# lyndonchan/wsss-analysis

Hardware: AMD Instinct MI355X
Metric: images/sec CAM+CRF pseudo-labels, VOC2012 321x321 (higher is better)
Workload: dtype f16x3; 1 GPU; resnet50 CAM + dense-CRF (M=21, 10 mean-field iters), 321x321, batch 32 images (=64 samples) per GPU, image-sharded; batch_images=32, num_classes=20, parallelism=image-sharded x1, no collective, steps_per_rank=245

## Files before the change

### include/wsscam.h

```cpp
#ifndef WSSCAM_H
#define WSSCAM_H

#include <stddef.h>
#include <stdint.h>

#ifdef __cplusplus
extern "C" {
#endif

#define WSC_VERSION 100

typedef enum wsc_status {
    WSC_OK = 0,
    WSC_ERR_INVALID = -1,
    WSC_ERR_NO_DEVICE = -2,
    WSC_ERR_HIP = -3,
    WSC_ERR_MISSING_KEY = -4,
    WSC_ERR_SHAPE = -5,
    WSC_ERR_NOMEM = -6,
    WSC_ERR_KEY_RANGE = -7,
    WSC_ERR_CAPACITY = -8,
    WSC_ERR_RANGE = -9
} wsc_status;

typedef enum wsc_arch {
    WSC_ARCH_RESNET50_CAM = 0,
    WSC_ARCH_VGG16_CAM = 1,
    WSC_ARCH_M7_CAM = 2,
    WSC_ARCH_RESNET50_IRN = 3,
    WSC_ARCH_VGG16_IRN = 4,
    WSC_ARCH_M7_IRN = 5
} wsc_arch;

typedef enum wsc_precision {
    WSC_PREC_BF16 = 0,
    WSC_PREC_BF16X3 = 1,
    WSC_PREC_F16 = 2,
    WSC_PREC_F16X3 = 3
} wsc_precision;

typedef struct wsc_ctx wsc_ctx;
typedef struct wsc_net wsc_net;
typedef enum {
    WSC_OPT_CRF_GAUSS_ON_CHIP = 0,
    WSC_OPT_CRF_FUSED_BLUR = 1,
    WSC_OPT_CRF_BLUR_ON_CHIP = 2,
    WSC_OPT_CRF_RANK_BALLOT = 3,
    WSC_OPT_CRF_EMBED_FULL = 4,
    WSC_OPT_RW_TILED = 5,
    WSC_OPT_STEM_POOL_FUSED = 6,
    WSC_OPT_CONV_WINDOW = 7,
    WSC_OPT_CAM_HEAD_STREAM = 8,
    WSC_OPT_CRF_MSG_IN_UPDATE = 9,
    WSC_OPT_COUNT = 10
} wsc_option;

typedef struct wsc_crf wsc_crf;
typedef struct wsc_crf_v wsc_crf_v;

typedef struct wsc_tensor_desc {
    const char *name;
    const float *data;
    int32_t ndim;
    int64_t shape[4];
} wsc_tensor_desc;


int wsc_version(void);
const char *wsc_last_error(void);

int wsc_ctx_create(int device, void *stream, wsc_ctx **out);
void wsc_ctx_destroy(wsc_ctx *ctx);
int wsc_ctx_set_option(wsc_ctx *ctx, int option, int value);
int wsc_sync(wsc_ctx *ctx);
int wsc_ctx_range_status(wsc_ctx *ctx, int *flag_out, int clear);
int wsc_ctx_wait(wsc_ctx *ctx, wsc_ctx *other);
int wsc_ctx_mark(wsc_ctx *ctx, int slot);
int wsc_ctx_wait_mark(wsc_ctx *ctx, int slot);
int wsc_ctx_wait_for_mark(wsc_ctx *ctx, wsc_ctx *other, int slot);
int wsc_device_info(wsc_ctx *ctx, char *arch_name, size_t arch_name_len, int *num_cus);

int wsc_malloc(wsc_ctx *ctx, size_t bytes, void **dptr_out);
int wsc_free(wsc_ctx *ctx, void *dptr);
int wsc_memcpy_h2d(wsc_ctx *ctx, void *dst_dev, const void *src_host, size_t bytes);
int wsc_memcpy_d2h(wsc_ctx *ctx, void *dst_host, const void *src_dev, size_t bytes);
int wsc_memset(wsc_ctx *ctx, void *dst_dev, int value, size_t bytes);
int wsc_host_alloc(wsc_ctx *ctx, size_t bytes, void **host_out);
int wsc_host_free(wsc_ctx *ctx, void *host);
int wsc_host_write_segments(const char *path, int n, const void *const *ptrs, const size_t *sizes);
int wsc_memcpy_h2d_async(wsc_ctx *ctx, void *dst_dev, const void *src_pinned_host, size_t bytes);
int wsc_memcpy_d2h_async(wsc_ctx *ctx, void *dst_pinned_host, const void *src_dev, size_t bytes);

int wsc_timer_begin(wsc_ctx *ctx);
int wsc_timer_end(wsc_ctx *ctx, float *ms_out);

int wsc_profile_begin(wsc_ctx *ctx);
int wsc_profile_end(wsc_ctx *ctx, int max_classes, int32_t *calls_out, float *total_ms_out, double *work_out,
                    int *n_classes_out);
const char *wsc_profile_class_name(int cls);


int wsc_net_create(wsc_ctx *ctx, int arch, const wsc_tensor_desc *weights, int n_weights,
                   int num_classes, int precision, wsc_net **out);
void wsc_net_destroy(wsc_net *net);
int wsc_net_cam_size(const wsc_net *net, int S, int *h_out);
int wsc_net_feat_channels(const wsc_net *net, int *f_out);

int wsc_net_forward_cam(wsc_ctx *ctx, const wsc_net *net, const float *x_dev, int B, int S,
                        float *cam_dev, float *score_dev);
int wsc_net_cam_size_hw(const wsc_net *net, int H, int W, int *h_out, int *w_out);
int wsc_net_forward_cam_hw(wsc_ctx *ctx, const wsc_net *net, const float *x_dev, int B, int H, int W, float *cam_dev,
                           float *score_dev);

int wsc_net_forward_features(wsc_ctx *ctx, const wsc_net *net, const float *x_dev ,
                             int N, int S, float *feat_dev);

int wsc_net_forward_edge(wsc_ctx *ctx, const wsc_net *net, const float *x_dev, int B, int S, int feat_h, int feat_w,
                         float *edge_dev, float *dp_dev);

int wsc_rw_propagate(wsc_ctx *ctx, const float *x_dev, const float *edge_dev, int K, int h, int w,
                     const int32_t *dirs_host, const int32_t *path_start_host, const int32_t *path_yx_host, int D,
                     float beta, int n_steps, float *rw_dev);
int wsc_rw_propagate_batch(wsc_ctx *ctx, int n_img, const int32_t *K_host, const int32_t *h_host,
                           const int32_t *w_host, const float *x_dev, const float *edge_dev,
                           const int32_t *dirs_host, const int32_t *path_start_host, const int32_t *path_yx_host,
                           int D, float beta, int n_steps, float *rw_dev);

int wsc_net_forward_gradcam(wsc_ctx *ctx, const wsc_net *net, const float *x_dev, int N, int S, int relu,
                            float *cams_dev, float *score_dev);

#define WSC_CONV_GENERIC 0x100
int wsc_conv2d_nchw(wsc_ctx *ctx, const float *x_dev, int N, int Cin, int H, int W, const float *w_host,
                    int Cout, int kh, int kw, int stride, int pad, const float *scale_host,
                    const float *shift_host, const float *residual_dev, int relu, int precision,
                    float *y_dev);


int wsc_cam_postprocess(wsc_ctx *ctx, const float *cam_dev, int B, int C, int h, int w,
                        const int32_t *size_hw_host , const int32_t *keys_host,
                        const int32_t *key_off_host , const int64_t *strided_off_host ,
                        const int64_t *highres_off_host , float *strided_dev, float *highres_dev);

int wsc_cam_eval_confusion(wsc_ctx *ctx, const float *highres_dev, int B, const int32_t *size_hw_host,
                           const int32_t *keys_host, const int32_t *key_off_host,
                           const int64_t *highres_off_host, float bg_thres, const uint8_t *gt_dev, int n_class,
                           int ignore_label, uint8_t *pred_dev, int64_t *confusion_dev);

int wsc_unary_from_maps(wsc_ctx *ctx, const float *maps_dev, int B, int C, int N, float bg_value,
                        float *unary_dev);

int wsc_cam_eval_confusion_nn(wsc_ctx *ctx, const float *maps_dev, int B, const int32_t *src_hw_host ,
                              const int32_t *out_hw_host , const int32_t *keys_host, const int32_t *key_off_host ,
                              const int64_t *maps_off_host , const uint8_t *gt_dev, int n_class, int ignore_label,
                              uint8_t *pred_dev, int64_t *confusion_dev);

int wsc_label_confusion_nn(wsc_ctx *ctx, const int32_t *labels_dev, int B, const int32_t *src_hw_host ,
                           const int32_t *out_hw_host , const int64_t *labels_off_host , const uint8_t *gt_dev,
                           int n_class, int ignore_label, uint8_t *pred_dev, int64_t *confusion_dev);

int wsc_sem_seg_finish(wsc_ctx *ctx, const float *rw_dev, int B, const int64_t *rw_off_host , const int32_t *khw_host ,
                       const int32_t *up_hw_host , const int32_t *out_hw_host , const int32_t *keys_host,
                       const int32_t *key_off_host , int has_bg, float bg_thres, uint8_t *label_dev);

int wsc_cam_unary(wsc_ctx *ctx, const float *cam_dev, int B, int C, int h, int w, int H0, int W0, float bg_value,
                  float *unary_dev);
int wsc_cam_unary_pm(wsc_ctx *ctx, const float *cam_dev, int B, int C, int h, int w, int H0, int W0, float bg_value,
                     float *unary_pm_dev);

int wsc_cam_sum_scales(wsc_ctx *ctx, const float *cam_dev, int n_images, int n_scales, long long map_elems, float *out_dev);

int wsc_msf_input_u8(wsc_ctx *ctx, const uint8_t *images_dev, int B, const int32_t *size_hw_host,
                     const int64_t *offset_host, int S, const float *mean3_host, const float *std3_host,
                     int pre_div255, int pair, float *x_dev);

int wsc_resize_u8(wsc_ctx *ctx, const uint8_t *images_dev, int B, const int32_t *size_hw_host, const int64_t *offset_host,
                  int OH, int OW, uint8_t *out_dev);

int wsc_bilinear_resize(wsc_ctx *ctx, const float *src_dev, int C, int h, int w, float *dst_dev, int H,
                        int W);


int wsc_label_unary_from_cam(wsc_ctx *ctx, const float *highres_dev, int B, int K, int N, float thres, float gt_prob,
                             float *unary_dev, int32_t *labels_dev);
int wsc_ir_label_combine(wsc_ctx *ctx, const int32_t *fg_pred_dev, const int32_t *bg_pred_dev, const int32_t *keys_host,
                         int B, int M, int N, uint8_t *conf_dev);


int wsc_hsn_gradcam_post(wsc_ctx *ctx, const float *cams_nhwc_dev, int B, int h, int w, int C, int S,
                         const float *gate_dev, float *out_dev, int out_channels, int out_first);
int wsc_hsn_voc_background(wsc_ctx *ctx, const float *Hbg_dev, int B, int Cb, int N, float *y_dev, int Ctot);
int wsc_hsn_class_mass(wsc_ctx *ctx, const float *maps_dev, int n_maps, int N, uint32_t *mass_dev);
int wsc_hsn_background(wsc_ctx *ctx, const uint8_t *rgb_dev, int B, int H, int W, int Ho, int Wo, double *bg_dev);
int wsc_cam_adp_modify(wsc_ctx *ctx, const float *cam_dev, int B, int n_sc, int C, int hw, const double *bg_dev, int mode,
                       const int32_t *use_host, int n_use, const int32_t *adipose_host, int n_adip, const int32_t *exc_host,
                       int n_exc, float *out_dev);
int wsc_hsn_cs_gradcam(wsc_ctx *ctx, const float *H_dev, int B, int C_all, int N, const double *bg_dev,
                       const int32_t *src_of_valid_host, int Cv, int bg_ind, int other_ind,
                       const int32_t *exception_inds_host, int n_exc, const int32_t *adipose_src_host, int n_adip,
                       float *cs_dev, float *y_dev, uint32_t *mass_dev);
int wsc_hsn_gather_unary(wsc_ctx *ctx, const float *maps_dev, const int64_t *chan_off_host, int n_chan, int N,
                         float *unary_dev);


int wsc_crf_create(wsc_ctx *ctx, const uint8_t *rgb_dev, int B, int H, int W, float g_sxy,
                   float bi_sxy, float bi_srgb, wsc_crf **out);
void wsc_crf_destroy(wsc_crf *crf);
int wsc_crf_lattice_sizes(wsc_ctx *ctx, const wsc_crf *crf, int32_t *v_gauss_host,
                          int32_t *v_bilat_host);
int wsc_crf_gaussian_on_chip(const wsc_crf *crf, int M);

int wsc_crf_inference(wsc_ctx *ctx, wsc_crf *crf, const float *unary_dev, int M, float g_compat,
                      float bi_compat, int n_iters, float *q_dev, int32_t *argmax_dev);
int wsc_crf_inference_pm(wsc_ctx *ctx, wsc_crf *crf, const float *unary_pm_dev, int M, float g_compat,
                         float bi_compat, int n_iters, float *q_dev, int32_t *argmax_dev);

int wsc_crf_v_create(wsc_ctx *ctx, const uint8_t *const *rgb_dev, const int32_t *hw_host , int B, float g_sxy,
                     float bi_sxy, float bi_srgb, wsc_crf_v **out);
void wsc_crf_v_destroy(wsc_crf_v *crf);
int wsc_crf_v_num_groups(const wsc_crf_v *crf);
int wsc_crf_v_inference(wsc_ctx *ctx, wsc_crf_v *crf, const float *const *unary_dev, const int32_t *M_host, float g_compat,
                        float bi_compat, int n_iters, float *const *q_dev, int32_t *const *argmax_dev);

#ifdef __cplusplus
}
#endif
#endif
```

### profiles/conv_layer_table.py

```python
import re
import sqlite3
import sys


def resnet50_layers(S):
    def o(h, k, s, p):
        return (h + 2 * p - k) // s + 1

    L = []
    h = o(S, 7, 2, 3)
    L.append(("stem 7x7 s2 3->64", h, 3, 64, 7))
    h = o(h, 3, 2, 1)
    inp = 64
    for li, (planes, blocks, stride) in enumerate(((64, 3, 1), (128, 4, 2), (256, 6, 2), (512, 3, 1)), 1):
        for b in range(blocks):
            s = stride if b == 0 else 1
            ho = o(h, 3, s, 1)
            n = "layer%d.%d." % (li, b)
            L.append((n + "conv1 1x1 %d->%d" % (inp, planes), h, inp, planes, 1))
            L.append((n + "conv2 3x3 %d s%d" % (planes, s), ho, planes, planes, 3))
            if b == 0:
                L.append((n + "conv3+proj 1x1 (%d+%d)->%d" % (planes, inp, planes * 4), ho, planes + inp, planes * 4, 1))
            else:
                L.append((n + "conv3 1x1 %d->%d +res" % (planes, planes * 4), ho, planes, planes * 4, 1))
            inp = planes * 4
            h = ho
    L.append(("CAM head 1x1 2048->20", h, 2048, 20, 1))
    return L


def n_dispatches(M, cin, cout, k, num_cus=256, planes=1):
    if cin % 64 or cout % 256:
        return 1
    nk = k * k * cin // (32 if planes == 2 else 64)
    blocks_sq = ((M + 255) // 256) * (cout // 256)
    if nk < (16 if planes == 2 else 4) or blocks_sq < 192:
        return 1
    rounds, rem = divmod(blocks_sq, num_cus)
    return 2 if rounds >= 1 and 0 < rem and rem * 2 <= num_cus else 1


def main(db, N=64, S=321, planes=1):
    c = sqlite3.connect(db)
    tabs = [r[0] for r in c.execute("select name from sqlite_master where type='table'")]
    kd = [t for t in tabs if "kernel_dispatch" in t][0]
    ks = [t for t in tabs if "kernel_symbol" in t][0]
    rows = c.execute("select s.kernel_name, d.start, d.end, d.grid_size_x / d.workgroup_size_x, d.group_segment_size "
                     "from %s d join %s s on d.kernel_id = s.id order by d.start" % (kd, ks)).fetchall()
    start = [i for i, r in enumerate(rows) if "nchw_to_nhwc4" in r[0]][-1]
    convs = [r for r in rows[start:] if "conv_igemm_kernel" in r[0] or "stem_pool_kernel" in r[0] or "cam_head_kernel" in r[0]]
    layers = resnet50_layers(S)
    if "stem_pool_kernel" in convs[0][0]:
        layers[0] = ("stem 7x7 s2 3->64 + maxpool (fused)",) + layers[0][1:]
    print("%-44s %8s %8s %9s %7s %6s" % ("layer", "us", "TFLOP/s", "act TB/s", "blocks", "LDS KB"))
    tot = 0.0
    pos = 0
    for (name, ho, cin, cout, k) in layers:
        M = N * ho * ho
        nd = n_dispatches(M, cin, cout, k, planes=planes)
        rs = convs[pos:pos + nd]
        pos += nd
        us = sum(r[2] - r[1] for r in rs) / 1000.0
        tot += us
        fl = 2.0 * M * cout * k * k * cin
        by = 2.0 * M * cout * (2 if "+res" in name else 1) + 2.0 * N * (ho * (2 if "s2" in name else 1)) ** 2 * cin
        if "fused" in name:
            by = 8.0 * N * S * S + 2.0 * N * ((ho + 1) // 2) ** 2 * cout
        by *= planes
        print("%-44s %8.1f %8.0f %9.2f %7s %6s" % (name, us, fl / us / 1e6, by / us / 1e6, "+".join(str(r[3]) for r in rs),
                                                    "/".join("%.0f" % (r[4] / 1024.0) for r in rs)))
    print("conv kernels total %.1f us" % tot)


if __name__ == "__main__":
    main(sys.argv[1], *(int(v) for v in sys.argv[2:]))
```

### wsss-analysis_amd/csrc/api.hip

```cpp
#include "common.h"

#include <cerrno>
#include <cstdarg>
#include <fcntl.h>
#include <sys/uio.h>
#include <unistd.h>
#include <vector>
#include <cstdio>
#include <cstring>

static thread_local char g_err[1024] = "";

void wsc_set_error(const char *fmt, ...) {
    va_list ap;
    va_start(ap, fmt);
    vsnprintf(g_err, sizeof(g_err), fmt, ap);
    va_end(ap);
}

int wsc_ctx_workspace(wsc_ctx *ctx, size_t bytes, void **out) {
    if (bytes > ctx->ws_bytes) {
        WSC_HIP(hipStreamSynchronize(ctx->stream));
        if (ctx->ws) WSC_HIP(hipFree(ctx->ws));
        ctx->ws = nullptr;
        ctx->ws_bytes = 0;
        const size_t want = bytes + bytes / 8;
        hipError_t e = hipMalloc(&ctx->ws, want);
        if (e != hipSuccess) {
            wsc_set_error("workspace hipMalloc(%zu bytes) failed: %s", want, hipGetErrorString(e));
            return WSC_ERR_NOMEM;
        }
        ctx->ws_bytes = want;
    }
    *out = ctx->ws;
    return WSC_OK;
}

int wsc_ctx_cached_alloc(wsc_ctx *ctx, size_t bytes, void **out) {
    size_t want = bytes < 256 ? 256 : bytes;
    want = want <= (1u << 20) ? (want + 4095) / 4096 * 4096 : (want + (2u << 20) - 1) / (2u << 20) * (2u << 20);
    auto it = ctx->free_blocks.lower_bound(want);
    if (it != ctx->free_blocks.end() && it->first <= 2 * want + (1u << 20)) {
        *out = it->second;
        ctx->live_blocks[it->second] = it->first;
        ctx->free_blocks.erase(it);
        return WSC_OK;
    }
    void *p = nullptr;
    hipError_t e = hipMalloc(&p, want);
    if (e != hipSuccess) {
        (void)hipStreamSynchronize(ctx->stream);
        for (auto &kv : ctx->free_blocks) (void)hipFree(kv.second);
        ctx->free_blocks.clear();
        e = hipMalloc(&p, want);
    }
    if (e != hipSuccess) {
        wsc_set_error("hipMalloc(%zu bytes) failed: %s", want, hipGetErrorString(e));
        return WSC_ERR_NOMEM;
    }
    ctx->live_blocks[p] = want;
    *out = p;
    return WSC_OK;
}

void wsc_ctx_cached_free(wsc_ctx *ctx, void *p) {
    if (!p) return;
    auto it = ctx->live_blocks.find(p);
    if (it == ctx->live_blocks.end()) return;
    ctx->free_blocks.emplace(it->second, p);
    ctx->live_blocks.erase(it);
}

int wsc_ctx_upload_small(wsc_ctx *ctx, void *dst_dev, const void *src_host, size_t bytes) {
    if (bytes == 0) return WSC_OK;
    wsc_ctx::PinSlot &s = ctx->pin_ring[ctx->pin_next];
    ctx->pin_next = (ctx->pin_next + 1) % wsc_ctx::PIN_SLOTS;
    if (s.busy) {
        WSC_HIP(hipEventSynchronize(s.ev));
        s.busy = false;
    }
    if (!s.ev) WSC_HIP(hipEventCreateWithFlags(&s.ev, hipEventDisableTiming));
    if (bytes > s.bytes) {
        if (s.p) WSC_HIP(hipHostFree(s.p));
        s.p = nullptr;
        s.bytes = 0;
        const size_t want = bytes * 2 < (64u << 10) ? (64u << 10) : bytes * 2;
        WSC_HIP(hipHostMalloc(&s.p, want, hipHostMallocDefault));
        s.bytes = want;
    }
    memcpy(s.p, src_host, bytes);
    WSC_HIP(hipMemcpyAsync(dst_dev, s.p, bytes, hipMemcpyHostToDevice, ctx->stream));
    WSC_HIP(hipEventRecord(s.ev, ctx->stream));
    s.busy = true;
    return WSC_OK;
}

static hipEvent_t prof_event(wsc_ctx *ctx) {
    if (!ctx->prof_pool.empty()) {
        hipEvent_t e = ctx->prof_pool.back();
        ctx->prof_pool.pop_back();
        return e;
    }
    hipEvent_t e = nullptr;
    (void)hipEventCreate(&e);
    return e;
}

WscKernelTimer::WscKernelTimer(wsc_ctx *c, int cls, double work) : ctx(c) {
    if (!ctx->profiling) return;
    WscProfRecord r;
    r.cls = cls;
    r.work = work;
    r.e0 = prof_event(ctx);
    r.e1 = prof_event(ctx);
    (void)hipEventRecord(r.e0, ctx->stream);
    ctx->prof.push_back(r);
    idx = (int)ctx->prof.size() - 1;
}
WscKernelTimer::~WscKernelTimer() {
    if (idx >= 0) (void)hipEventRecord(ctx->prof[idx].e1, ctx->stream);
}

static const char *kClassNames[WSC_K_COUNT] = {
    "conv_igemm_kernel<256-row tiles,glds>", "conv_igemm_kernel<128x128,glds>", "conv_igemm_kernel<128x64,glds>", "conv_igemm_kernel<small-Cin> / stem_pool_kernel",
    "pool/layout/flip-add", "cam_tail+unary", "crf_build(all)", "gauss_msg_kernel", "combine4+blur_lds+blur4+blur3_tile",
    "update_splat_kernel", "crf init/finish"};

int wsc_ctx_range_check(wsc_ctx *ctx) {
    const unsigned f = *(volatile unsigned *)ctx->range_host;
    if (f == 0u) return WSC_OK;
    wsc_set_error("an activation of an IEEE-half conv mode (f16 / f16x3) reached half's ceiling (|v| >= 65504) in a layer with %u "
                  "output channels and was saturated -- the reference's fp32 would have kept it, these maps are not the reference's; "
                  "use WSC_PREC_BF16X3 for this model (wsc_ctx_range_status clears the flag)", f);
    return WSC_ERR_RANGE;
}

extern "C" {

int wsc_profile_begin(wsc_ctx *ctx) {
    WSC_CHECK(ctx, WSC_ERR_INVALID, "wsc_profile_begin: null ctx");
    WSC_HIP(hipStreamSynchronize(ctx->stream));
    for (auto &r : ctx->prof) {
        ctx->prof_pool.push_back(r.e0);
        ctx->prof_pool.push_back(r.e1);
    }
    ctx->prof.clear();
    ctx->profiling = true;
    return WSC_OK;
}

int wsc_profile_end(wsc_ctx *ctx, int max_classes, int32_t *calls_out, float *total_ms_out, double *work_out,
                    int *n_classes_out) {
    WSC_CHECK(ctx && calls_out && total_ms_out && work_out, WSC_ERR_INVALID, "wsc_profile_end: null argument");
    ctx->profiling = false;
    WSC_HIP(hipStreamSynchronize(ctx->stream));
    const int n = max_classes < WSC_K_COUNT ? max_classes : (int)WSC_K_COUNT;
    for (int i = 0; i < n; ++i) {
        calls_out[i] = 0;
        total_ms_out[i] = 0.f;
        work_out[i] = 0.0;
    }
    for (auto &r : ctx->prof) {
        float ms = 0.f;
        WSC_HIP(hipEventElapsedTime(&ms, r.e0, r.e1));
        if (r.cls < n) {
            calls_out[r.cls] += 1;
            total_ms_out[r.cls] += ms;
            work_out[r.cls] += r.work;
        }
        ctx->prof_pool.push_back(r.e0);
        ctx->prof_pool.push_back(r.e1);
    }
    ctx->prof.clear();
    if (n_classes_out) *n_classes_out = n;
    return WSC_OK;
}

const char *wsc_profile_class_name(int cls) { return cls >= 0 && cls < WSC_K_COUNT ? kClassNames[cls] : ""; }

int wsc_version(void) { return WSC_VERSION; }
const char *wsc_last_error(void) { return g_err; }

int wsc_ctx_create(int device, void *stream, wsc_ctx **out) {
    WSC_CHECK(out != nullptr, WSC_ERR_INVALID, "wsc_ctx_create: out is null");
    int count = 0;
    hipError_t e = hipGetDeviceCount(&count);
    if (e != hipSuccess || count <= 0) {
        wsc_set_error("no HIP device available (%s); libwsscam has no CPU fallback",
                      e == hipSuccess ? "device count is 0" : hipGetErrorString(e));
        return WSC_ERR_NO_DEVICE;
    }
    WSC_CHECK(device >= 0 && device < count, WSC_ERR_INVALID, "device %d out of range [0,%d)", device, count);
    WSC_HIP(hipSetDevice(device));
    hipDeviceProp_t prop;
    WSC_HIP(hipGetDeviceProperties(&prop, device));
    if (strncmp(prop.gcnArchName, "gfx950", 6) != 0) {
        wsc_set_error("device %d is %s; libwsscam is built for gfx950 only", device, prop.gcnArchName);
        return WSC_ERR_NO_DEVICE;
    }
    wsc_ctx *ctx = new wsc_ctx();
    ctx->device = device;
    ctx->num_cus = prop.multiProcessorCount;
    ctx->arch = prop.gcnArchName;
    if (stream) {
        ctx->stream = (hipStream_t)stream;
        ctx->own_stream = false;
    } else {
        WSC_HIP(hipStreamCreateWithFlags(&ctx->stream, hipStreamNonBlocking));
        ctx->own_stream = true;
    }
    WSC_HIP(hipMalloc(&ctx->zero_page, 256));
    WSC_HIP(hipMemset(ctx->zero_page, 0, 256));
    WSC_HIP(hipHostMalloc((void **)&ctx->range_host, 64, hipHostMallocMapped));
    memset(ctx->range_host, 0, 64);
    WSC_HIP(hipHostGetDevicePointer((void **)&ctx->range_dev, ctx->range_host, 0));
    WSC_HIP(hipEventCreateWithFlags(&ctx->pinned_ev, hipEventDisableTiming));
    WSC_HIP(hipEventCreateWithFlags(&ctx->join_ev, hipEventDisableTiming));
    WSC_HIP(hipEventCreate(&ctx->ev0));
    WSC_HIP(hipEventCreate(&ctx->ev1));
    *out = ctx;
    return WSC_OK;
}

int wsc_ctx_set_option(wsc_ctx *ctx, int option, int value) {
    WSC_CHECK(ctx != nullptr, WSC_ERR_INVALID, "wsc_ctx_set_option: null context");
    WSC_CHECK(option >= 0 && option < WSC_OPT_COUNT, WSC_ERR_INVALID, "wsc_ctx_set_option: unknown option %d", option);
    ctx->opt[option] = value;
    return WSC_OK;
}

void wsc_ctx_destroy(wsc_ctx *ctx) {
    if (!ctx) return;
    (void)hipSetDevice(ctx->device);
    (void)hipStreamSynchronize(ctx->stream);
    for (auto &a : ctx->attachments) a.second(a.first);
    if (ctx->ws) (void)hipFree(ctx->ws);
    if (ctx->zero_page) (void)hipFree(ctx->zero_page);
    if (ctx->range_host) (void)hipHostFree(ctx->range_host);
    for (auto &kv : ctx->free_blocks) (void)hipFree(kv.second);
    for (auto &kv : ctx->live_blocks) (void)hipFree(kv.first);
    if (ctx->pinned) (void)hipHostFree(ctx->pinned);
    for (wsc_ctx::PinSlot &s : ctx->pin_ring) {
        if (s.p) (void)hipHostFree(s.p);
        if (s.ev) (void)hipEventDestroy(s.ev);
    }
    if (ctx->pinned_ev) (void)hipEventDestroy(ctx->pinned_ev);
    if (ctx->join_ev) (void)hipEventDestroy(ctx->join_ev);
    for (hipEvent_t e : ctx->marks)
        if (e) (void)hipEventDestroy(e);
    if (ctx->fork_ev) (void)hipEventDestroy(ctx->fork_ev);
    if (ctx->aux_done_ev) (void)hipEventDestroy(ctx->aux_done_ev);
    if (ctx->aux_stream) {
        (void)hipStreamSynchronize(ctx->aux_stream);
        (void)hipStreamDestroy(ctx->aux_stream);
    }
    for (auto &r : ctx->prof) { (void)hipEventDestroy(r.e0); (void)hipEventDestroy(r.e1); }
    for (auto e : ctx->prof_pool) (void)hipEventDestroy(e);
    if (ctx->ev0) (void)hipEventDestroy(ctx->ev0);
    if (ctx->ev1) (void)hipEventDestroy(ctx->ev1);
    if (ctx->own_stream) (void)hipStreamDestroy(ctx->stream);
    delete ctx;
}

int wsc_sync(wsc_ctx *ctx) {
    WSC_CHECK(ctx, WSC_ERR_INVALID, "wsc_sync: null ctx");
    WSC_HIP(hipSetDevice(ctx->device));
    WSC_HIP(hipStreamSynchronize(ctx->stream));
    return wsc_ctx_range_check(ctx);
}

int wsc_ctx_range_status(wsc_ctx *ctx, int *flag_out, int clear) {
    WSC_CHECK(ctx, WSC_ERR_INVALID, "wsc_ctx_range_status: null ctx");
    WSC_HIP(hipSetDevice(ctx->device));
    WSC_HIP(hipStreamSynchronize(ctx->stream));
    volatile unsigned *f = ctx->range_host;
    if (flag_out) *flag_out = (int)*f;
    if (clear) *f = 0u;
    return WSC_OK;
}

int wsc_ctx_mark(wsc_ctx *ctx, int slot) {
    WSC_CHECK(ctx && slot >= 0 && slot < 8, WSC_ERR_INVALID, "wsc_ctx_mark: slot %d outside [0, 8)", slot);
    WSC_HIP(hipSetDevice(ctx->device));
    if (!ctx->marks[slot]) WSC_HIP(hipEventCreateWithFlags(&ctx->marks[slot], hipEventDisableTiming));
    WSC_HIP(hipEventRecord(ctx->marks[slot], ctx->stream));
    ctx->mark_set[slot] = true;
    return WSC_OK;
}

int wsc_ctx_wait_mark(wsc_ctx *ctx, int slot) {
    WSC_CHECK(ctx && slot >= 0 && slot < 8, WSC_ERR_INVALID, "wsc_ctx_wait_mark: slot %d outside [0, 8)", slot);
    if (!ctx->mark_set[slot]) return WSC_OK;
    WSC_HIP(hipSetDevice(ctx->device));
    WSC_HIP(hipEventSynchronize(ctx->marks[slot]));
    return wsc_ctx_range_check(ctx);
}

int wsc_ctx_wait_for_mark(wsc_ctx *ctx, wsc_ctx *other, int slot) {
    WSC_CHECK(ctx && other && slot >= 0 && slot < 8, WSC_ERR_INVALID, "wsc_ctx_wait_for_mark: bad argument (slot %d)", slot);
    WSC_CHECK(ctx->device == other->device, WSC_ERR_INVALID, "wsc_ctx_wait_for_mark: contexts are on different devices");
    if (!other->mark_set[slot] || ctx == other) return WSC_OK;
    WSC_HIP(hipSetDevice(ctx->device));
    WSC_HIP(hipStreamWaitEvent(ctx->stream, other->marks[slot], 0));
    return WSC_OK;
}

int wsc_ctx_wait(wsc_ctx *ctx, wsc_ctx *other) {
    WSC_CHECK(ctx && other, WSC_ERR_INVALID, "wsc_ctx_wait: null ctx");
    WSC_CHECK(ctx->device == other->device, WSC_ERR_INVALID, "wsc_ctx_wait: contexts are on different devices");
    if (ctx == other) return WSC_OK;
    WSC_HIP(hipEventRecord(other->join_ev, other->stream));
    WSC_HIP(hipStreamWaitEvent(ctx->stream, other->join_ev, 0));
    return WSC_OK;
}

int wsc_device_info(wsc_ctx *ctx, char *arch_name, size_t arch_name_len, int *num_cus) {
    WSC_CHECK(ctx, WSC_ERR_INVALID, "wsc_device_info: null ctx");
    if (arch_name && arch_name_len > 0) {
        strncpy(arch_name, ctx->arch.c_str(), arch_name_len - 1);
        arch_name[arch_name_len - 1] = 0;
    }
    if (num_cus) *num_cus = ctx->num_cus;
    return WSC_OK;
}

int wsc_malloc(wsc_ctx *ctx, size_t bytes, void **dptr_out) {
    WSC_CHECK(ctx && dptr_out, WSC_ERR_INVALID, "wsc_malloc: null argument");
    WSC_HIP(hipSetDevice(ctx->device));
    hipError_t e = hipMalloc(dptr_out, bytes ? bytes : 1);
    if (e != hipSuccess) {
        wsc_set_error("hipMalloc(%zu) failed: %s", bytes, hipGetErrorString(e));
        return WSC_ERR_NOMEM;
    }
    return WSC_OK;
}

int wsc_free(wsc_ctx *ctx, void *dptr) {
    WSC_CHECK(ctx, WSC_ERR_INVALID, "wsc_free: null ctx");
    if (!dptr) return WSC_OK;
    WSC_HIP(hipStreamSynchronize(ctx->stream));
    WSC_HIP(hipFree(dptr));
    return WSC_OK;
}

int wsc_memcpy_h2d(wsc_ctx *ctx, void *dst_dev, const void *src_host, size_t bytes) {
    WSC_CHECK(ctx && (bytes == 0 || (dst_dev && src_host)), WSC_ERR_INVALID, "wsc_memcpy_h2d: null argument");
    if (bytes == 0) return WSC_OK;
    WSC_HIP(hipMemcpyAsync(dst_dev, src_host, bytes, hipMemcpyHostToDevice, ctx->stream));
    return WSC_OK;
}

int wsc_memcpy_d2h(wsc_ctx *ctx, void *dst_host, const void *src_dev, size_t bytes) {
    WSC_CHECK(ctx && (bytes == 0 || (dst_host && src_dev)), WSC_ERR_INVALID, "wsc_memcpy_d2h: null argument");
    if (bytes == 0) return WSC_OK;
    WSC_HIP(hipStreamSynchronize(ctx->stream));
    WSC_HIP(hipMemcpyAsync(dst_host, src_dev, bytes, hipMemcpyDeviceToHost, ctx->stream));
    WSC_HIP(hipStreamSynchronize(ctx->stream));
    return wsc_ctx_range_check(ctx);
}

int wsc_memset(wsc_ctx *ctx, void *dst_dev, int value, size_t bytes) {
    WSC_CHECK(ctx && (bytes == 0 || dst_dev), WSC_ERR_INVALID, "wsc_memset: null argument");
    if (bytes == 0) return WSC_OK;
    WSC_HIP(hipMemsetAsync(dst_dev, value, bytes, ctx->stream));
    return WSC_OK;
}

int wsc_host_alloc(wsc_ctx *ctx, size_t bytes, void **host_out) {
    WSC_CHECK(ctx && host_out, WSC_ERR_INVALID, "wsc_host_alloc: null argument");
    WSC_HIP(hipSetDevice(ctx->device));
    hipError_t e = hipHostMalloc(host_out, bytes ? bytes : 1, hipHostMallocDefault);
    if (e != hipSuccess) {
        wsc_set_error("hipHostMalloc(%zu) failed: %s", bytes, hipGetErrorString(e));
        return WSC_ERR_NOMEM;
    }
    return WSC_OK;
}

int wsc_host_free(wsc_ctx *ctx, void *host) {
    WSC_CHECK(ctx, WSC_ERR_INVALID, "wsc_host_free: null ctx");
    if (!host) return WSC_OK;
    WSC_HIP(hipStreamSynchronize(ctx->stream));
    WSC_HIP(hipHostFree(host));
    return WSC_OK;
}

int wsc_host_write_segments(const char *path, int n, const void *const *ptrs, const size_t *sizes) {
    WSC_CHECK(path && n >= 0 && (n == 0 || (ptrs && sizes)), WSC_ERR_INVALID, "wsc_host_write_segments: null argument");
    const int fd = open(path, O_WRONLY | O_CREAT | O_TRUNC, 0644);
    if (fd < 0) {
        wsc_set_error("wsc_host_write_segments: cannot open %s: %s", path, strerror(errno));
        return WSC_ERR_INVALID;
    }
    int st = WSC_OK;
    std::vector<struct iovec> iov;
    for (int i = 0; i < n; ++i)
        if (sizes[i] > 0) iov.push_back({const_cast<void *>(ptrs[i]), sizes[i]});
    size_t at = 0;
    while (at < iov.size() && st == WSC_OK) {
        const int cnt = (int)std::min<size_t>(iov.size() - at, 64);
        ssize_t w = writev(fd, iov.data() + at, cnt);
        if (w < 0) {
            if (errno == EINTR) continue;
            wsc_set_error("wsc_host_write_segments: write to %s failed: %s", path, strerror(errno));
            st = WSC_ERR_INVALID;
            break;
        }
        while (w > 0 && at < iov.size()) {
            if ((size_t)w >= iov[at].iov_len) {
                w -= (ssize_t)iov[at].iov_len;
                ++at;
            } else {
                iov[at].iov_base = (char *)iov[at].iov_base + w;
                iov[at].iov_len -= (size_t)w;
                w = 0;
            }
        }
    }
    if (close(fd) != 0 && st == WSC_OK) {
        wsc_set_error("wsc_host_write_segments: close of %s failed: %s", path, strerror(errno));
        st = WSC_ERR_INVALID;
    }
    return st;
}

int wsc_memcpy_h2d_async(wsc_ctx *ctx, void *dst_dev, const void *src_pinned_host, size_t bytes) {
    WSC_CHECK(ctx && (bytes == 0 || (dst_dev && src_pinned_host)), WSC_ERR_INVALID, "wsc_memcpy_h2d_async: null argument");
    if (bytes == 0) return WSC_OK;
    WSC_HIP(hipMemcpyAsync(dst_dev, src_pinned_host, bytes, hipMemcpyHostToDevice, ctx->stream));
// ... 26 lines not shown
```

### wsss-analysis_amd/csrc/common.h

```cpp
#pragma once
#include <hip/hip_runtime.h>
#include <stdint.h>
#include <map>
#include <string>
#include <unordered_map>
#include <vector>

#include "../../include/wsscam.h"

typedef uint16_t bf16_t;

typedef __bf16 bf16x8_t __attribute__((ext_vector_type(8)));
typedef _Float16 f16x8_t __attribute__((ext_vector_type(8)));
typedef float f32x16_t __attribute__((ext_vector_type(16)));
typedef float f32x4_t __attribute__((ext_vector_type(4)));

__host__ __device__ inline bf16_t f32_to_bf16(float f) {
    union { float f; uint32_t u; } v;
    v.f = f;
    uint32_t u = v.u;
    if ((u & 0x7fffffffu) > 0x7f800000u) return (bf16_t)((u >> 16) | 0x40);
    u += 0x7fffu + ((u >> 16) & 1u);
    return (bf16_t)(u >> 16);
}
__host__ __device__ inline float bf16_to_f32(bf16_t h) {
    union { float f; uint32_t u; } v;
    v.u = ((uint32_t)h) << 16;
    return v.f;
}

__host__ __device__ inline uint16_t f32_to_f16(float f) {
#if defined(__HIP_DEVICE_COMPILE__)
    const _Float16 h = (_Float16)fminf(fmaxf(f, -65504.f), 65504.f);
    return __builtin_bit_cast(uint16_t, h);
#else
    union { float f; uint32_t u; } v, magic;
    v.f = f;
    const uint32_t sign = v.u & 0x80000000u;
    v.u ^= sign;
    uint16_t o;
    if (v.u >= ((127u + 16u) << 23)) {
        o = v.u > (255u << 23) ? 0x7e00 : 0x7bff;
    } else if (v.u < (113u << 23)) {
        magic.u = ((127u - 15u) + (23u - 10u) + 1u) << 23;
        v.f += magic.f;
        o = (uint16_t)(v.u - magic.u);
    } else {
        const uint32_t mant_odd = (v.u >> 13) & 1u;
        v.u += ((15u - 127u) << 23) + 0xfffu;
        v.u += mant_odd;
        o = (uint16_t)(v.u >> 13);
        if (o >= 0x7c00) o = 0x7bff;
    }
    return (uint16_t)(o | (sign >> 16));
#endif
}
__host__ __device__ inline float f16_to_f32(uint16_t h) {
#if defined(__HIP_DEVICE_COMPILE__)
    return (float)__builtin_bit_cast(_Float16, h);
#else
    union { float f; uint32_t u; } o, magic;
    magic.u = 113u << 23;
    const uint32_t shifted_exp = 0x7c00u << 13;
    o.u = ((uint32_t)h & 0x7fffu) << 13;
    const uint32_t exp = shifted_exp & o.u;
    o.u += (127u - 15u) << 23;
    if (exp == shifted_exp) o.u += (128u - 16u) << 23;
    else if (exp == 0) { o.u += 1u << 23; o.f -= magic.f; }
    o.u |= ((uint32_t)h & 0x8000u) << 16;
    return o.f;
#endif
}
__host__ __device__ inline uint16_t f32_to_h16(float f, int fmt) { return fmt ? f32_to_f16(f) : f32_to_bf16(f); }
__host__ __device__ inline float h16_to_f32(uint16_t h, int fmt) { return fmt ? f16_to_f32(h) : bf16_to_f32(h); }

void wsc_set_error(const char *fmt, ...);
#define WSC_HIP(expr)                                                                          \
    do {                                                                                       \
        hipError_t _e = (expr);                                                                \
        if (_e != hipSuccess) {                                                                \
            wsc_set_error("%s:%d: %s failed: %s", __FILE__, __LINE__, #expr,                   \
                          hipGetErrorString(_e));                                              \
            return WSC_ERR_HIP;                                                                \
        }                                                                                      \
    } while (0)
#define WSC_CHECK(cond, code, ...)                                                             \
    do {                                                                                       \
        if (!(cond)) {                                                                         \
            wsc_set_error(__VA_ARGS__);                                                        \
            return (code);                                                                     \
        }                                                                                      \
    } while (0)
#define WSC_TRY(expr)                                                                          \
    do {                                                                                       \
        int _s = (expr);                                                                       \
        if (_s != WSC_OK) return _s;                                                           \
    } while (0)

enum WscKernelClass {
    WSC_K_CONV256 = 0,
    WSC_K_CONV128,
    WSC_K_CONV64,
    WSC_K_CONV_SMALLCIN,
    WSC_K_POOL_MISC,
    WSC_K_CAM_TAIL,
    WSC_K_CRF_BUILD,
    WSC_K_GAUSS_MSG,
    WSC_K_BLUR,
    WSC_K_SLICE_UPDATE,
    WSC_K_CRF_MISC,
    WSC_K_COUNT
};
struct WscProfRecord {
    int cls;
    double work;
    hipEvent_t e0, e1;
};

struct wsc_ctx {
    int device = 0;
    hipStream_t stream = nullptr;
    bool own_stream = false;
    int num_cus = 0;
    std::string arch;
    void *ws = nullptr;
    size_t ws_bytes = 0;
    static constexpr int PIN_SLOTS = 8;
    struct PinSlot {
        void *p = nullptr;
        size_t bytes = 0;
        hipEvent_t ev = nullptr;
        bool busy = false;
    };
    PinSlot pin_ring[PIN_SLOTS];
    int pin_next = 0;
    int opt[WSC_OPT_COUNT] = {1, 1, 1, 0, 0, -1, 1, 1, 1, 1};
    void *pinned = nullptr;
    size_t pinned_bytes = 0;
    void *zero_page = nullptr;
    unsigned *range_host = nullptr, *range_dev = nullptr;
    hipEvent_t pinned_ev = nullptr;
    bool pinned_busy = false;
    hipEvent_t ev0 = nullptr, ev1 = nullptr;
    hipEvent_t join_ev = nullptr;
    hipEvent_t marks[8] = {};
    bool mark_set[8] = {};
    hipStream_t aux_stream = nullptr;
    hipEvent_t fork_ev = nullptr, aux_done_ev = nullptr;
    bool profiling = false;
    std::vector<WscProfRecord> prof;
    std::vector<hipEvent_t> prof_pool;
    std::multimap<size_t, void *> free_blocks;
    std::unordered_map<void *, size_t> live_blocks;
    std::vector<std::pair<void *, void (*)(void *)>> attachments;
};
int wsc_ctx_workspace(wsc_ctx *ctx, size_t bytes, void **out);
int wsc_ctx_range_check(wsc_ctx *ctx);
__device__ __forceinline__ unsigned half2_at_ceiling(unsigned hw) { return (hw & 0x7fff7fffu) + 0x04010401u; }
struct WscKernelTimer {
    wsc_ctx *ctx;
    int idx = -1;
    WscKernelTimer(wsc_ctx *c, int cls, double work);
    ~WscKernelTimer();
};
int wsc_ctx_cached_alloc(wsc_ctx *ctx, size_t bytes, void **out);
void wsc_ctx_cached_free(wsc_ctx *ctx, void *p);
struct WscCachedGuard {
    wsc_ctx *ctx;
    void *p;
    WscCachedGuard(wsc_ctx *c, void *q) : ctx(c), p(q) {}
    WscCachedGuard(const WscCachedGuard &) = delete;
    WscCachedGuard &operator=(const WscCachedGuard &) = delete;
    void free_now() {
        if (p) wsc_ctx_cached_free(ctx, p);
        p = nullptr;
    }
    ~WscCachedGuard() { free_now(); }
};
int wsc_ctx_upload_small(wsc_ctx *ctx, void *dst_dev, const void *src_host, size_t bytes);

struct ConvLaunch {
    const bf16_t *x, *x_lo;
    const bf16_t *w;
    const float *s1, *b1;
    const float *s2, *b2;
    const bf16_t *res, *res_lo;
    bf16_t *y, *y_lo;
    float *y_f32;
    int N, H, W, Cin, Ho, Wo, Cout, CoutPad;
    int kh, kw, stride, pad;
    int relu;
    int small_cin;
    int split;
    int fmt;
    int generic;
    int ldy;
    const bf16_t *x2, *x2_lo;
    int H2, W2, C2, stride2;
};
int conv_igemm_launch(wsc_ctx *ctx, const ConvLaunch &p);
int launch_cam_head(wsc_ctx *ctx, const bf16_t *x, const bf16_t *x_lo, int M, int K, const bf16_t *w, int Kw, int CoutPad,
                    const float *s1, const float *b1, int C, int relu, float *y);

int launch_nchw_to_nhwc4(wsc_ctx *ctx, const float *x, int N, int H, int W, bf16_t *y, bf16_t *y_lo, int fmt);
void stem_pool_input_dims(int H, int W, int *Hp, int *Wp);
int launch_stem_pool(wsc_ctx *ctx, const bf16_t *x, const bf16_t *x_lo, int N, int H, int W, const bf16_t *w, int Kw, const float *s1,
                     const float *b1, int relu, bf16_t *y, bf16_t *y_lo);
int launch_gather_strided(wsc_ctx *ctx, const bf16_t *x, const bf16_t *x_lo, int N, int H, int W, int C, int stride, int Ho, int Wo,
                          bf16_t *y, bf16_t *y_lo, int ldy);
int launch_nchw_to_nhwc4_pad(wsc_ctx *ctx, const float *x, int N, int H, int W, int Hp, int Wp, int pad, bf16_t *y, bf16_t *y_lo,
                             int fmt);
int launch_maxpool(wsc_ctx *ctx, const bf16_t *x, const bf16_t *x_lo, int N, int H, int W, int C, int k,
                   int stride, int pad, int Ho, int Wo, bf16_t *y, bf16_t *y_lo, int fmt);
int launch_flip_add(wsc_ctx *ctx, const float *head, int B, int h, int w, int C, int Cs, float *cam);
int launch_gap_linear_sigmoid(wsc_ctx *ctx, const bf16_t *feat, const bf16_t *feat_lo, int B, int hw, int F,
                              const float *Wc, const float *bias, int C, float *score, int fmt,
                              int sample_stride);
int launch_bf16_to_f32(wsc_ctx *ctx, const bf16_t *x, const bf16_t *x_lo, size_t n, float *y, int fmt);
int launch_nchw_to_nhwc(wsc_ctx *ctx, const float *x, int N, int C, int HW, bf16_t *y, bf16_t *y_lo, int fmt);
int launch_nhwc_to_nchw(wsc_ctx *ctx, const bf16_t *x, const bf16_t *x_lo, int N, int C, int HW, float *y, int fmt);

int launch_group_norm_stats(wsc_ctx *ctx, const float *x, int N, int H, int W, int C, int G, float eps, void *partial,
                            void *stats);
size_t group_norm_partial_bytes(int N, int H, int W, int G);
int launch_group_norm_apply(wsc_ctx *ctx, const float *x, const void *stats, const float *gamma, const float *beta,
                            int N, int H, int W, int C, int G, int up, int relu, bf16_t *y, bf16_t *y_lo, int Hd, int Wd,
                            int Ctot, int coff, int fmt);
int launch_edge_finish(wsc_ctx *ctx, const float *e, int He, int We, const float *d, int Hd, int Wd, int B, int fh, int fw,
                       float ms0, float ms1, float *edge, float *dp);
```

### wsss-analysis_amd/csrc/conv_igemm.hip

```cpp
#include "common.h"

#include <cstdlib>
#include <type_traits>

#ifdef WSC_AB_KNOBS
#define WSC_DBG(p, bit) ((p).debug & (bit))
#else
#define WSC_DBG(p, bit) 0
#endif

namespace {

constexpr int BK = 64;

struct ConvKArgs {
    const bf16_t *x, *x_lo, *w;
    const float *s1, *b1, *s2, *b2;
    const bf16_t *res, *res_lo;
    bf16_t *y, *y_lo;
    float *y_f32;
    int H, W, Cin, Ho, Wo, Cout;
    int ldy;
    int kh, kw, stride, pad, relu;
    int M, HoWo;
    int m_base, m_end;
    unsigned div_howo_mul, div_howo_s1, div_howo_s2, div_wo_mul, div_wo_s1, div_wo_s2;
    int cchunks;
    int ntaps;
    int ksteps_base;
    int nk;
    int Kw;
    int Kbase;
    int ntiles_n, nblocks;
    const bf16_t *zero;
    int fast;
    int debug;
    long long lo_delta;
    const bf16_t *x2;
    long long lo_delta2;
    int cc2, H2, W2, C2, stride2;
    int ldx;
    int win_npix;
    int stem_rows;
    int kw_real;
    unsigned *range;
};

__device__ __forceinline__ int lds_off(int row, int slot) {
    return row * 128 + ((slot ^ ((row >> 1) & 7)) << 4);
}

template <int BM, int BN, int MODE, int SPLIT, int ET, bool GLDS, int STAGES, int WMT = 64, int FAST = 0, int WPT = 0>
__global__ __launch_bounds__(BM * 2, (STAGES == 1 && FAST != 0) ? 4 : 2) void conv_igemm_kernel(ConvKArgs p) {
    constexpr bool FEPI = (FAST & 1) != 0, PW = (FAST & 2) != 0;
    constexpr bool WIN = WPT > 0;
    static_assert(!WIN || (SPLIT == 2 && BM == 128 && WMT == 64 && STAGES == 2 && FAST == 1), "LDS window: single-staged split, 128-row tile");
    static_assert(FAST == 0 || (SPLIT != 1 && ET == 1 && ((GLDS && MODE == 0) || FAST == 1)),
                  "FAST paths: f16, one plane or the single-staged split; the pointwise prologue belongs to the LDS-DMA layers");
    static_assert(SPLIT != 2 || (GLDS && MODE == 0 && STAGES == 2), "single-staged split: LDS-DMA layers, two LDS buffers");
    constexpr int CK = SPLIT == 2 ? 32 : 64;
    constexpr int NT = BM * 2;
    constexpr int NW = BM / 32;
    constexpr int WR = BM / WMT;
    constexpr int WC = NW / WR;
    constexpr int WN = BN / WC;
    constexpr int MI = WMT / 32;
    constexpr int NI = WN / 32;
    static_assert(WR * WC == NW && WN % 32 == 0 && (WMT == 64 || WMT == 128), "wave layout");
    constexpr int NB = BN * 8 / NT;
    constexpr int A_BYTES = BM * BK * 2;
    constexpr int B_BYTES = BN * BK * 2;
    constexpr int WIN_BYTES = WPT * 4096;
    constexpr int A_REGION = WIN ? WIN_BYTES : STAGES * A_BYTES;
    constexpr int CT_STRIDE = BN + 4;
    static_assert(GLDS || (BM == 128 && STAGES <= 2), "register staging exists for the 128-row tile only");
    static_assert(STAGES >= 1 && STAGES <= 3, "1 (single K-step layers), 2 or 3 LDS buffers");

    extern __shared__ __attribute__((aligned(16))) char smem[];

    const int t = threadIdx.x;
    const int lane = t & 63;
    const int wv = __builtin_amdgcn_readfirstlane(t >> 6);
    const int wm = wv / WC, wn = wv - wm * WC;

    int tile;
    {
        const int bid = blockIdx.x;
        const int xcd = bid & 7;
        const int q = p.nblocks >> 3, r = p.nblocks & 7;
        tile = (xcd < r ? xcd * (q + 1) : r * (q + 1) + (xcd - r) * q) + (bid >> 3);
    }
    const int mt = tile / p.ntiles_n;
    const int nt = tile - mt * p.ntiles_n;
    const int m0 = p.m_base + mt * BM;
    const int n0 = nt * BN;

    const int slot = t & 7;
    const int lrow = GLDS ? (wv * 32 + (lane >> 3)) : (t >> 3);
    constexpr int RSTEP = GLDS ? 8 : 32;
    int hb[4], wb[4];
    long long base[4];
#pragma unroll
    for (int i = 0; i < 4; ++i) {
        const int m = m0 + lrow + RSTEP * i;
        if (PW) {
            const int mc = m < p.m_end ? m : p.m_end - 1;
            hb[i] = 0;
            wb[i] = 0;
            base[i] = (long long)mc * p.ldx;
        } else if (m < p.m_end) {
            const unsigned t1 = __umulhi(p.div_howo_mul, (unsigned)m);
            const int n = (int)((t1 + (((unsigned)m - t1) >> p.div_howo_s1)) >> p.div_howo_s2);
            const int rem = m - n * p.HoWo;
            const unsigned t2 = __umulhi(p.div_wo_mul, (unsigned)rem);
            const int ho = (int)((t2 + (((unsigned)rem - t2) >> p.div_wo_s1)) >> p.div_wo_s2);
            const int wo = rem - ho * p.Wo;
            hb[i] = ho * p.stride - p.pad;
            wb[i] = wo * p.stride - p.pad;
            base[i] = (((long long)n * p.H + hb[i]) * p.W + wb[i]) * (long long)p.ldx;
        } else {
            hb[i] = -(1 << 28);
            wb[i] = 0;
            base[i] = 0;
        }
    }
    const int brow0 = GLDS ? (wv * (BN / NW) + (lane >> 3)) : (t >> 3);
    const bf16_t *wrow[NB];
#pragma unroll
    for (int i = 0; i < NB; ++i) {
        const int r = brow0 + RSTEP * i;
        const int ks = GLDS ? (slot ^ ((r >> 1) & 7)) : slot;
        wrow[i] = p.w + (long long)(n0 + r) * p.Kw + ks * 8;
    }

    long long aoff[4];
#pragma unroll
    for (int i = 0; i < 4; ++i) {
        const int r = lrow + RSTEP * i;
        const int ks = slot ^ ((r >> 1) & 7);
        if (SPLIT == 2) aoff[i] = base[i] + (ks & 3) * 8 + ((ks & 4) ? p.lo_delta : 0ll);
        else aoff[i] = base[i] + ks * 8;
    }

    typedef unsigned u32x4_t __attribute__((ext_vector_type(4)));
    u32x4_t ra[4], rb[NB];

    auto issue_dma = [&](int kt, int buf) {
        int seg = 0, ktl = kt;
        if (SPLIT) {
            seg = kt / p.ksteps_base;
            ktl = kt - seg * p.ksteps_base;
        }
        const bf16_t *src = (SPLIT && seg == 1) ? p.x_lo : p.x;
        const int cc = ktl / p.ntaps;
        const int tap = ktl - cc * p.ntaps;
        const int khi = tap / p.kw;
        const int kwi = tap - khi * p.kw;
        const long long tap_off = ((long long)khi * p.W + kwi) * p.ldx + cc * 64;
        char *sa = smem + buf * A_BYTES + wv * 4096;
        char *sb = smem + STAGES * A_BYTES + buf * B_BYTES + wv * (NB * 1024);
#pragma unroll
        for (int i = 0; i < 4; ++i) {
            const int r = lrow + RSTEP * i;
            const int ks = slot ^ ((r >> 1) & 7);
            const int hi = hb[i] + khi, wi = wb[i] + kwi;
            const bool ok = PW || ((unsigned)hi < (unsigned)p.H && (unsigned)wi < (unsigned)p.W);
            const bf16_t *g = ok ? src + base[i] + tap_off + ks * 8 : p.zero;
            __builtin_amdgcn_global_load_lds((const __attribute__((address_space(1))) void *)g,
                                             (__attribute__((address_space(3))) void *)(sa + i * 1024), 16, 0, 0);
        }
        const int wk = ((SPLIT && seg == 2) ? p.Kbase : 0) + ktl * 64;
#pragma unroll
        for (int i = 0; i < NB; ++i)
            __builtin_amdgcn_global_load_lds((const __attribute__((address_space(1))) void *)(wrow[i] + wk),
                                             (__attribute__((address_space(3))) void *)(sb + i * 1024), 16, 0, 0);
    };

    auto load_tile = [&](int kt) __attribute__((always_inline)) {
        int seg = 0, ktl = kt;
        if (SPLIT) {
            seg = kt / p.ksteps_base;
            ktl = kt - seg * p.ksteps_base;
        }
        const bf16_t *src = (SPLIT && seg == 1) ? p.x_lo : p.x;
        if (MODE == 0) {
            const int cc = ktl / p.ntaps;
            const int tap = ktl - cc * p.ntaps;
            const int khi = tap / p.kw;
            const int kwi = tap - khi * p.kw;
            const long long tap_off = ((long long)khi * p.W + kwi) * p.ldx + cc * 64 + slot * 8;
#pragma unroll
            for (int i = 0; i < 4; ++i) {
                const int hi = hb[i] + khi, wi = wb[i] + kwi;
                const bool ok = (unsigned)hi < (unsigned)p.H && (unsigned)wi < (unsigned)p.W;
                ra[i] = ok ? *reinterpret_cast<const u32x4_t *>(src + base[i] + tap_off) : u32x4_t{0u, 0u, 0u, 0u};
            }
        } else {
            const int g = ktl * 8 + slot;
            const int khi = g >> MODE;
            const int px = (g & ((1 << MODE) - 1)) * 2;
#pragma unroll
            for (int i = 0; i < 4; ++i) {
                const int hi = hb[i] + khi, wi = wb[i] + px;
                const bool okh = khi < p.kh && (unsigned)hi < (unsigned)p.H;
                const uint2 *q = reinterpret_cast<const uint2 *>(src + base[i] + ((long long)khi * p.W + px) * 4);
                uint2 v0 = make_uint2(0, 0), v1 = make_uint2(0, 0);
                if (okh && (unsigned)wi < (unsigned)p.W) v0 = q[0];
                if (okh && (unsigned)(wi + 1) < (unsigned)p.W) v1 = q[1];
                ra[i] = u32x4_t{v0.x, v0.y, v1.x, v1.y};
            }
        }
        const int wk = ((SPLIT && seg == 2) ? p.Kbase : 0) + ktl * 64;
#pragma unroll
        for (int i = 0; i < NB; ++i) rb[i] = *reinterpret_cast<const u32x4_t *>(wrow[i] + wk);
    };

    auto store_lds = [&](int buf) __attribute__((always_inline)) {
        char *sa = smem + buf * A_BYTES;
        char *sb = smem + STAGES * A_BYTES + buf * B_BYTES;
#pragma unroll
        for (int i = 0; i < 4; ++i) *reinterpret_cast<u32x4_t *>(sa + lds_off(lrow + 32 * i, slot)) = ra[i];
#pragma unroll
        for (int i = 0; i < NB; ++i) *reinterpret_cast<u32x4_t *>(sb + lds_off(lrow + 32 * i, slot)) = rb[i];
    };

    f32x16_t acc[MI][NI];
#pragma unroll
    for (int mi = 0; mi < MI; ++mi)
#pragma unroll
        for (int ni = 0; ni < NI; ++ni)
#pragma unroll
            for (int r = 0; r < 16; ++r) acc[mi][ni][r] = 0.f;

    const int l31 = lane & 31;
    const int kgrp = lane >> 5;

    auto mfma = [&](const u32x4_t &a, const u32x4_t &b, f32x16_t &c) {
        if (WSC_DBG(p, 4)) return;
        if (ET == 0)
            c = __builtin_amdgcn_mfma_f32_32x32x16_bf16(__builtin_bit_cast(bf16x8_t, a), __builtin_bit_cast(bf16x8_t, b),
                                                        c, 0, 0, 0);
        else
            c = __builtin_amdgcn_mfma_f32_32x32x16_f16(__builtin_bit_cast(f16x8_t, a), __builtin_bit_cast(f16x8_t, b),
                                                       c, 0, 0, 0);
    };
    auto mfma0 = [&](const u32x4_t &a, const u32x4_t &b) -> f32x16_t {
        const f32x16_t z = {0.f, 0.f, 0.f, 0.f, 0.f, 0.f, 0.f, 0.f, 0.f, 0.f, 0.f, 0.f, 0.f, 0.f, 0.f, 0.f};
        if (ET == 0)
            return __builtin_amdgcn_mfma_f32_32x32x16_bf16(__builtin_bit_cast(bf16x8_t, a), __builtin_bit_cast(bf16x8_t, b), z, 0, 0, 0);
        return __builtin_amdgcn_mfma_f32_32x32x16_f16(__builtin_bit_cast(f16x8_t, a), __builtin_bit_cast(f16x8_t, b), z, 0, 0, 0);
    };
    const unsigned lds0 = (unsigned)(uintptr_t)(__attribute__((address_space(3))) char *)smem;

    auto compute = [&](int buf) {
        if (GLDS) {
            const unsigned sa = lds0 + buf * A_BYTES, sb = lds0 + STAGES * A_BYTES + buf * B_BYTES;
            u32x4_t fa[2][MI], fb[2][NI];
            auto rd = [&](int set, int ks) {
                const int sl = ks * 2 + kgrp;
#pragma unroll
                for (int mi = 0; mi < MI; ++mi)
                    asm volatile("ds_read_b128 %0, %1" : "=v"(fa[set][mi]) : "v"(sa + lds_off(wm * WMT + mi * 32 + l31, sl)) : "memory");
#pragma unroll
                for (int ni = 0; ni < NI; ++ni)
                    asm volatile("ds_read_b128 %0, %1" : "=v"(fb[set][ni]) : "v"(sb + lds_off(wn * WN + ni * 32 + l31, sl)) : "memory");
            };
            rd(0, 0);
#pragma unroll
            for (int ks = 0; ks < 4; ++ks) {
                const int set = ks & 1;
                if (ks < 3) {
                    rd(set ^ 1, ks + 1);
                    asm volatile("s_waitcnt lgkmcnt(%0)" ::"n"(MI + NI) : "memory");
                } else {
                    asm volatile("s_waitcnt lgkmcnt(0)" ::: "memory");
                }
                __builtin_amdgcn_sched_barrier(0);
#pragma unroll
                for (int mi = 0; mi < MI; ++mi)
#pragma unroll
                    for (int ni = 0; ni < NI; ++ni) mfma(fa[set][mi], fb[set][ni], acc[mi][ni]);
            }
            return;
        }
        const char *sa = smem + buf * A_BYTES;
        const char *sb = smem + STAGES * A_BYTES + buf * B_BYTES;
#pragma unroll
        for (int ks = 0; ks < 4; ++ks) {
            const int sl = ks * 2 + kgrp;
            u32x4_t af[MI], bfr[NI];
#pragma unroll
            for (int mi = 0; mi < MI; ++mi)
                af[mi] = *reinterpret_cast<const u32x4_t *>(sa + lds_off(wm * WMT + mi * 32 + l31, sl));
#pragma unroll
            for (int ni = 0; ni < NI; ++ni)
                bfr[ni] = *reinterpret_cast<const u32x4_t *>(sb + lds_off(wn * WN + ni * 32 + l31, sl));
#pragma unroll
            for (int mi = 0; mi < MI; ++mi)
#pragma unroll
                for (int ni = 0; ni < NI; ++ni) mfma(af[mi], bfr[ni], acc[mi][ni]);
        }
    };

    const int nk = STAGES == 1 ? 1 : p.nk;
    if (GLDS && MODE == 0 && STAGES == 3) {
        constexpr int PER = 4 + NB;
        issue_dma(0, 0);
        if (nk > 1) {
            issue_dma(1, 1);
            asm volatile("s_waitcnt vmcnt(%0)" ::"n"(PER) : "memory");
        } else {
            asm volatile("s_waitcnt vmcnt(0)" ::: "memory");
        }
        __builtin_amdgcn_s_barrier();
        int cur = 0;
        for (int kt = 0; kt < nk; ++kt) {
            const bool ahead = kt + 2 < nk;
            if (ahead && !WSC_DBG(p, 1)) issue_dma(kt + 2, cur == 0 ? 2 : cur - 1);
            if (!WSC_DBG(p, 2)) compute(cur);
            if (ahead) asm volatile("s_waitcnt vmcnt(%0)" ::"n"(PER) : "memory");
            else asm volatile("s_waitcnt vmcnt(0)" ::: "memory");
            __builtin_amdgcn_s_barrier();
            cur = cur == 2 ? 0 : cur + 1;
        }
    } else if (GLDS && MODE == 0) {
        int n_seg = 0, n_khi = 0, n_kwi = 0, n_cc = 0, n_ktl = 0;
        const bf16_t *n_src = p.x;
        long long n_tap = 0;
        int n_wk = 0;
        auto prep = [&]() {
            n_src = (SPLIT == 1 && n_seg == 1) ? p.x_lo : p.x;
            n_tap = ((long long)n_khi * p.W + n_kwi) * p.ldx + n_cc * CK;
            if (SPLIT != 1 && p.x2 != nullptr && n_cc >= p.cc2) {
                n_src = p.x2;
                n_tap = (n_cc - p.cc2) * CK;
            }
            n_wk = ((SPLIT == 1 && n_seg == 2) ? p.Kbase : 0) + n_ktl * 64;
        };
        auto second_source = [&]() {
#pragma unroll
            for (int i = 0; i < 4; ++i) {
                const int m = m0 + lrow + RSTEP * i;
                const unsigned mc = (unsigned)(m < p.m_end ? m : p.m_end - 1);
                const unsigned t1 = __umulhi(p.div_howo_mul, mc);
                const int n = (int)((t1 + ((mc - t1) >> p.div_howo_s1)) >> p.div_howo_s2);
                const int rem = (int)mc - n * p.HoWo;
                const unsigned t2 = __umulhi(p.div_wo_mul, (unsigned)rem);
                const int ho = (int)((t2 + (((unsigned)rem - t2) >> p.div_wo_s1)) >> p.div_wo_s2);
                const int wo = rem - ho * p.Wo;
                const long long b2 = (((long long)n * p.H2 + ho * p.stride2) * p.W2 + wo * p.stride2) * (long long)p.C2;
                const int r = lrow + RSTEP * i;
                const int ks = slot ^ ((r >> 1) & 7);
                if (SPLIT == 2) aoff[i] = b2 + (ks & 3) * 8 + ((ks & 4) ? p.lo_delta2 : 0ll);
                else aoff[i] = b2 + ks * 8;
            }
        };
        auto advance = [&]() {
            ++n_ktl;
// ... 106 lines not shown
            constexpr int cur = decltype(cur_c)::value;
            const unsigned(&oA)[4] = offA, (&oB)[4] = offB;
            const bool more = kt + 1 < nk && !WSC_DBG(p, 1);
            if (more) {
                prep();
                if (SPLIT != 2) {
#pragma unroll
                    for (int i = 0; i < 4; ++i) issue_a(i, cur ^ 1);
#pragma unroll
                    for (int i = 0; i < NB; ++i) issue_b(i, cur ^ 1);
                }
            }
            if constexpr (SPLIT == 2) {
                u32x4_t fah[2][MI], fal[2][MI], fbh[2][NI], fbl[2][NI];
                constexpr int NAP = WIN ? 0 : 4;
                constexpr int EVERY = (6 * MI * NI) / (NAP + NB);
                static_assert(EVERY >= 1, "a K-step has room for every DMA piece");
                auto piece = [&](int j) {
                    if (!more || j % EVERY != 0) return;
                    const int q = j / EVERY;
                    if (q < NAP) {
                        if (!(WSC_DBG(p, 32) && (n_khi | n_kwi) != 0)) issue_a(q, cur ^ 1);
                    } else if (q < NAP + NB) issue_b(q - NAP, cur ^ 1);
                    __builtin_amdgcn_sched_barrier(0);
                };
                unsigned aw[MI][4];
                if constexpr (WIN) {
                    if ((c_khi | c_kwi) == 0 && c_cc + 1 < p.cchunks) win_load(c_cc + 1);
                    const int toff = c_khi * p.W + c_kwi;
                    const unsigned tbit = 1u << (c_khi * 3 + c_kwi);
#pragma unroll
                    for (int mi = 0; mi < MI; ++mi) {
                        const int pos = (tapmask[mi] & tbit) ? WIN_ZERO : qm[mi] + toff;
                        const unsigned b0 = lds0 + (unsigned)pos * 128u, sw = (unsigned)(pos >> 1) & 7u;
#pragma unroll
                        for (int pr = 0; pr < 4; ++pr) aw[mi][pr] = b0 + ((((unsigned)(pr * 2 + kgrp)) ^ sw) << 4);
                    }
                }
                auto rd = [&](int set, int sl) {
#pragma unroll
                    for (int mi = 0; mi < MI; ++mi) {
                        if constexpr (WIN) {
                            asm volatile("ds_read_b128 %0, %1" : "=v"(fah[set][mi]) : "v"(aw[mi][sl]) : "memory");
                            asm volatile("ds_read_b128 %0, %1" : "=v"(fal[set][mi]) : "v"(aw[mi][2 + sl]) : "memory");
                        } else {
                            asm volatile("ds_read_b128 %0, %1 offset:%2" : "=v"(fah[set][mi]) : "v"(oA[sl]), "n"(cur * A_BYTES + mi * 4096) : "memory");
                            asm volatile("ds_read_b128 %0, %1 offset:%2" : "=v"(fal[set][mi]) : "v"(oA[2 + sl]), "n"(cur * A_BYTES + mi * 4096) : "memory");
                        }
                    }
#pragma unroll
                    for (int ni = 0; ni < NI; ++ni) {
                        asm volatile("ds_read_b128 %0, %1 offset:%2" : "=v"(fbh[set][ni]) : "v"(oB[sl]), "n"(cur * B_BYTES + ni * 4096) : "memory");
                        asm volatile("ds_read_b128 %0, %1 offset:%2" : "=v"(fbl[set][ni]) : "v"(oB[2 + sl]), "n"(cur * B_BYTES + ni * 4096) : "memory");
                    }
                };
                rd(0, 0);
#pragma unroll
                for (int sl = 0; sl < 2; ++sl) {
                    if (sl == 0) {
                        rd(1, 1);
                        asm volatile("s_waitcnt lgkmcnt(%0)" ::"n"(2 * (MI + NI)) : "memory");
                    } else {
                        asm volatile("s_waitcnt lgkmcnt(0)" ::: "memory");
                    }
                    __builtin_amdgcn_sched_barrier(0);
#pragma unroll
                    for (int mi = 0; mi < MI; ++mi)
#pragma unroll
                        for (int ni = 0; ni < NI; ++ni) {
                            mfma(fal[sl][mi], fbh[sl][ni], acc[mi][ni]);
                            piece((sl * 3 + 0) * MI * NI + mi * NI + ni);
                        }
#pragma unroll
                    for (int mi = 0; mi < MI; ++mi)
#pragma unroll
                        for (int ni = 0; ni < NI; ++ni) {
                            mfma(fah[sl][mi], fbl[sl][ni], acc[mi][ni]);
                            piece((sl * 3 + 1) * MI * NI + mi * NI + ni);
                        }
#pragma unroll
                    for (int mi = 0; mi < MI; ++mi)
#pragma unroll
                        for (int ni = 0; ni < NI; ++ni) {
                            mfma(fah[sl][mi], fbh[sl][ni], acc[mi][ni]);
                            piece((sl * 3 + 2) * MI * NI + mi * NI + ni);
                        }
                }
            } else if (STAGES == 1 || !WSC_DBG(p, 2)) {
                u32x4_t fa[2][MI], fb[2][NI];

                auto rd = [&](int set, int ks) {
#pragma unroll
                    for (int mi = 0; mi < MI; ++mi)
                        asm volatile("ds_read_b128 %0, %1 offset:%2" : "=v"(fa[set][mi]) : "v"(oA[ks]), "n"(cur * A_BYTES + mi * 4096) : "memory");
#pragma unroll
                    for (int ni = 0; ni < NI; ++ni)
                        asm volatile("ds_read_b128 %0, %1 offset:%2" : "=v"(fb[set][ni]) : "v"(oB[ks]), "n"(cur * B_BYTES + ni * 4096) : "memory");
                };
                rd(0, 0);
#pragma unroll
                for (int ks = 0; ks < 4; ++ks) {
                    const int set = ks & 1;
                    if (ks < 3) {
                        rd(set ^ 1, ks + 1);
                        asm volatile("s_waitcnt lgkmcnt(%0)" ::"n"(MI + NI) : "memory");
                    } else {
                        asm volatile("s_waitcnt lgkmcnt(0)" ::: "memory");
                    }
                    __builtin_amdgcn_sched_barrier(0);
#pragma unroll
                    for (int mi = 0; mi < MI; ++mi)
#pragma unroll
                        for (int ni = 0; ni < NI; ++ni) {
                            if (STAGES == 1 && ks == 0) acc[mi][ni] = mfma0(fa[set][mi], fb[set][ni]);
                            else mfma(fa[set][mi], fb[set][ni], acc[mi][ni]);
                        }
                }
            }
            if (more) advance();
            __syncthreads();
            if constexpr (WIN) {
                if (++c_kwi == p.kw) {
                    c_kwi = 0;
                    if (++c_khi == p.kh) {
                        c_khi = 0;
                        ++c_cc;
                        if (more) {
                            win_store();
                            __syncthreads();
                        }
                    }
                }
            }
        };
        static_assert(A_BYTES + (MI - 1) * 4096 < 65536 && B_BYTES + (NI - 1) * 4096 < 65536, "ds_read immediate offset range");
        if constexpr (ROLL) {
            u32x4_t fah[MI], fal[MI], fbh[NI], fbl[NI];
            auto slice = [&](auto buf_c, auto pair_c, bool more, bool dma, int dbuf) __attribute__((always_inline)) {
                constexpr int nbuf = decltype(buf_c)::value, npair = decltype(pair_c)::value;
                const unsigned(&oA)[4] = offA, (&oB)[4] = offB;
                auto piece = [&](int j) {
                    if (!dma || j % 3 != 0) return;
                    const int q = j / 3;
                    if (q < 4) issue_a(q, dbuf);
                    else if (q < 4 + NB) issue_b(q - 4, dbuf);
                    __builtin_amdgcn_sched_barrier(0);
                };
                static_assert(3 * MI * NI >= 3 * (4 + NB), "a slice has room for every DMA piece");
                auto rdA = [&](u32x4_t(&f)[MI], int pair) {
                    if (WSC_DBG(p, 16)) return;
#pragma unroll
                    for (int mi = 0; mi < MI; ++mi)
                        asm volatile("ds_read_b128 %0, %1 offset:%2" : "=v"(f[mi]) : "v"(oA[pair]), "n"(nbuf * A_BYTES + mi * 4096) : "memory");
                };
                auto rdB = [&](u32x4_t(&f)[NI], int pair) {
                    if (WSC_DBG(p, 16)) return;
#pragma unroll
                    for (int ni = 0; ni < NI; ++ni)
                        asm volatile("ds_read_b128 %0, %1 offset:%2" : "=v"(f[ni]) : "v"(oB[pair]), "n"(nbuf * B_BYTES + ni * 4096) : "memory");
                };
                asm volatile("s_waitcnt lgkmcnt(%0)" ::"n"(MI) : "memory");
                __builtin_amdgcn_sched_barrier(0);
#pragma unroll
                for (int mi = 0; mi < MI; ++mi)
#pragma unroll
                    for (int ni = 0; ni < NI; ++ni) {
                        mfma(fal[mi], fbh[ni], acc[mi][ni]);
                        piece(mi * NI + ni);
                    }
                __builtin_amdgcn_sched_barrier(0);
                if (more) {
                    rdA(fal, 2 + npair);
                    asm volatile("s_waitcnt lgkmcnt(%0)" ::"n"(MI) : "memory");
                } else {
                    asm volatile("s_waitcnt lgkmcnt(0)" ::: "memory");
                }
                __builtin_amdgcn_sched_barrier(0);
#pragma unroll
                for (int mi = 0; mi < MI; ++mi)
#pragma unroll
                    for (int ni = 0; ni < NI; ++ni) {
                        mfma(fah[mi], fbl[ni], acc[mi][ni]);
                        piece(MI * NI + mi * NI + ni);
                    }
                __builtin_amdgcn_sched_barrier(0);
                if (more) rdB(fbl, 2 + npair);
#pragma unroll
                for (int mi = 0; mi < MI; ++mi)
#pragma unroll
                    for (int ni = 0; ni < NI; ++ni) {
                        mfma(fah[mi], fbh[ni], acc[mi][ni]);
                        piece(2 * MI * NI + mi * NI + ni);
                    }
                __builtin_amdgcn_sched_barrier(0);
                if (more) {
                    rdB(fbh, npair);
                    rdA(fah, npair);
                }
            };
            {
                const unsigned(&oA)[4] = offA, (&oB)[4] = offB;
#pragma unroll
                for (int mi = 0; mi < MI; ++mi) asm volatile("ds_read_b128 %0, %1 offset:%2" : "=v"(fal[mi]) : "v"(oA[2]), "n"(mi * 4096) : "memory");
#pragma unroll
                for (int ni = 0; ni < NI; ++ni) asm volatile("ds_read_b128 %0, %1 offset:%2" : "=v"(fbl[ni]) : "v"(oB[2]), "n"(ni * 4096) : "memory");
#pragma unroll
                for (int ni = 0; ni < NI; ++ni) asm volatile("ds_read_b128 %0, %1 offset:%2" : "=v"(fbh[ni]) : "v"(oB[0]), "n"(ni * 4096) : "memory");
#pragma unroll
                for (int mi = 0; mi < MI; ++mi) asm volatile("ds_read_b128 %0, %1 offset:%2" : "=v"(fah[mi]) : "v"(oA[0]), "n"(mi * 4096) : "memory");
            }
            auto rstep = [&](auto cur_c, int kt) __attribute__((always_inline)) {
                constexpr int cur = decltype(cur_c)::value;
                slice(std::integral_constant<int, cur>{}, std::integral_constant<int, 1>{}, true, false, 0);
                if (WSC_DBG(p, 8)) asm volatile("s_waitcnt vmcnt(0) lgkmcnt(0)" ::: "memory");
                else
                __syncthreads();
                const bool refill = kt + 2 < nk && !WSC_DBG(p, 1);
                if (refill) prep();
                slice(std::integral_constant<int, cur ^ 1>{}, std::integral_constant<int, 0>{}, kt + 1 < nk, refill, cur);
                if (refill) advance();
            };
            for (int kt = 0; kt < nk; kt += 2) {
                rstep(std::integral_constant<int, 0>{}, kt);
                if (kt + 1 < nk) rstep(std::integral_constant<int, 1>{}, kt + 1);
            }
            __syncthreads();
        } else
        for (int kt = 0; kt < nk; kt += 2) {
            kstep(std::integral_constant<int, 0>{}, kt);
            if (kt + 1 < nk) kstep(std::integral_constant<int, 1>{}, kt + 1);
        }
    } else {
        load_tile(0);
        store_lds(0);
        __syncthreads();
        for (int kt = 0; kt < nk; ++kt) {
            const int cur = kt & 1;
            const bool more = kt + 1 < nk;
            if (more) load_tile(kt + 1);
            compute(cur);
            if (more) store_lds(cur ^ 1);
            __syncthreads();
        }
    }

    constexpr int TPR = BN / 8;
    constexpr int RPP = NT / TPR;
    constexpr int NPASS = BM / RPP;
    const int c8 = t % TPR;
    const int r0 = t / TPR;
    const int c = n0 + c8 * 8;
    const bool cok = c < p.Cout;
    const bool full = c + 8 <= p.Cout;
    const bool has_res = p.res != nullptr && full;
    constexpr bool PRE_ALL = WMT == 64 && !(STAGES == 1 && FEPI);
    constexpr int NHALF_R = STAGES == 1 ? BM / 64 : (WMT == 128 ? BM / 128 : 1);
    constexpr int NRES = PRE_ALL ? NPASS : NPASS / NHALF_R;
    uint4 rres[NRES], rres_lo[NRES];
    auto fetch_res = [&](int first_pass) {
#pragma unroll
        for (int i = 0; i < NRES; ++i) {
            const int m = m0 + (first_pass + i) * RPP + r0;
            rres[i] = make_uint4(0, 0, 0, 0);
            rres_lo[i] = make_uint4(0, 0, 0, 0);
            if (FEPI) {
                if (has_res) {
                    const int mc = m < p.m_end ? m : p.m_end - 1;
                    rres[i] = *reinterpret_cast<const uint4 *>(p.res + ((unsigned)mc * (unsigned)p.Cout + (unsigned)c));
                    if (SPLIT) rres_lo[i] = *reinterpret_cast<const uint4 *>(p.res_lo + ((unsigned)mc * (unsigned)p.Cout + (unsigned)c));
                }
            } else if (has_res && m < p.m_end) {
                const long long o = (long long)m * p.Cout + c;
                rres[i] = *reinterpret_cast<const uint4 *>(p.res + o);
                if (SPLIT) rres_lo[i] = *reinterpret_cast<const uint4 *>(p.res_lo + o);
            }
        }
    };
    if (PRE_ALL) fetch_res(0);
    const bool fpost = FEPI && p.s2 != nullptr;
    const float sat_lo = (p.relu && !fpost) ? 0.f : -65504.f;
    float s1[8], b1[8], s2[FEPI ? 1 : 8], b2[FEPI ? 1 : 8];
    const bool post = !FEPI && p.s2 != nullptr;
    if (FEPI) {
        const f32x4_t sa = *reinterpret_cast<const f32x4_t *>(p.s1 + c), sb = *reinterpret_cast<const f32x4_t *>(p.s1 + c + 4);
        const f32x4_t ba = *reinterpret_cast<const f32x4_t *>(p.b1 + c), bb = *reinterpret_cast<const f32x4_t *>(p.b1 + c + 4);
#pragma unroll
        for (int j = 0; j < 4; ++j) {
            s1[j] = sa[j];
            s1[4 + j] = sb[j];
            b1[j] = ba[j];
            b1[4 + j] = bb[j];
        }
    } else {
#pragma unroll
        for (int j = 0; j < 8; ++j) {
            s1[j] = cok ? p.s1[c + j] : 0.f;
            b1[j] = cok ? p.b1[c + j] : 0.f;
            s2[j] = (cok && post) ? p.s2[c + j] : 1.f;
            b2[j] = (cok && post) ? p.b2[c + j] : 0.f;
        }
    }

    float *ct = reinterpret_cast<float *>(smem);
    constexpr int NHALF = STAGES == 1 ? BM / 64 : (WMT == 128 ? BM / 128 : 1);
    constexpr int GR = BM / NHALF;
    constexpr int PPH = NPASS / NHALF;
    static_assert(NPASS % NHALF == 0 && PPH * RPP == GR && GR % WMT == 0, "epilogue pass layout");
    const int grp = (wm * WMT) / GR, roff = wm * WMT - grp * GR;
    unsigned ovf = 0u;
#pragma unroll
    for (int half = 0; half < NHALF; ++half) {
        if (half > 0) __syncthreads();
        if (!PRE_ALL) fetch_res(half * PPH);
        if (grp == half) {
#pragma unroll
            for (int mi = 0; mi < MI; ++mi)
#pragma unroll
                for (int ni = 0; ni < NI; ++ni)
#pragma unroll
                    for (int r = 0; r < 16; ++r) {
                        const int row = roff + mi * 32 + (r & 3) + 8 * (r >> 2) + 4 * kgrp;
                        const int col = wn * WN + ni * 32 + l31;
                        ct[row * CT_STRIDE + col] = acc[mi][ni][r];
                    }
        }
        __syncthreads();
        if (!cok) continue;
#pragma unroll
        for (int pp = 0; pp < PPH; ++pp) {
            const int pass = half * PPH + pp;
            const int lrow_e = pp * RPP + r0;
            const int m = m0 + half * GR + lrow_e;
            if (FEPI) {
                float v[8];
                const f32x4_t q0 = *reinterpret_cast<const f32x4_t *>(ct + lrow_e * CT_STRIDE + c8 * 8);
                const f32x4_t q1 = *reinterpret_cast<const f32x4_t *>(ct + lrow_e * CT_STRIDE + c8 * 8 + 4);
#pragma unroll
                for (int j = 0; j < 4; ++j) {
                    v[j] = q0[j] * s1[j] + b1[j];
                    v[4 + j] = q1[j] * s1[4 + j] + b1[4 + j];
                }
                if (has_res) {
                    const int ri = PRE_ALL ? pass : pp;
                    const uint32_t rw[4] = {rres[ri].x, rres[ri].y, rres[ri].z, rres[ri].w};
#pragma unroll
                    for (int j = 0; j < 4; ++j) {
                        v[2 * j] += f16_to_f32((bf16_t)(rw[j] & 0xffffu));
                        v[2 * j + 1] += f16_to_f32((bf16_t)(rw[j] >> 16));
                    }
                    if (SPLIT) {
                        const uint32_t lw[4] = {rres_lo[ri].x, rres_lo[ri].y, rres_lo[ri].z, rres_lo[ri].w};
#pragma unroll
                        for (int j = 0; j < 4; ++j) {
                            v[2 * j] += f16_to_f32((bf16_t)(lw[j] & 0xffffu));
                            v[2 * j + 1] += f16_to_f32((bf16_t)(lw[j] >> 16));
                        }
                    }
                }
                if (fpost) {
                    const f32x4_t s2a = *reinterpret_cast<const f32x4_t *>(p.s2 + c), s2b = *reinterpret_cast<const f32x4_t *>(p.s2 + c + 4);
                    const f32x4_t b2a = *reinterpret_cast<const f32x4_t *>(p.b2 + c), b2b = *reinterpret_cast<const f32x4_t *>(p.b2 + c + 4);
                    const float rl = p.relu ? 0.f : -3.0e38f;
#pragma unroll
                    for (int j = 0; j < 4; ++j) {
                        v[j] = __builtin_amdgcn_fmed3f(v[j], rl, 3.0e38f) * s2a[j] + b2a[j];
                        v[4 + j] = __builtin_amdgcn_fmed3f(v[4 + j], rl, 3.0e38f) * s2b[j] + b2b[j];
                    }
                }
                uint32_t hw[4], lw[SPLIT ? 4 : 1];
#pragma unroll
                for (int j = 0; j < 4; ++j) {
                    const float c0 = __builtin_amdgcn_fmed3f(v[2 * j], sat_lo, 65504.f), c1 = __builtin_amdgcn_fmed3f(v[2 * j + 1], sat_lo, 65504.f);
                    const _Float16 h0 = (_Float16)c0;
                    const _Float16 h1 = (_Float16)c1;
                    hw[j] = (uint32_t)__builtin_bit_cast(uint16_t, h0) | ((uint32_t)__builtin_bit_cast(uint16_t, h1) << 16);
                    if (SPLIT) {
                        const _Float16 l0 = (_Float16)(c0 - (float)h0), l1 = (_Float16)(c1 - (float)h1);
                        lw[j] = (uint32_t)__builtin_bit_cast(uint16_t, l0) | ((uint32_t)__builtin_bit_cast(uint16_t, l1) << 16);
                    }
                }
                if (m < p.m_end) {
                    ovf |= half2_at_ceiling(hw[0]) | half2_at_ceiling(hw[1]) | half2_at_ceiling(hw[2]) | half2_at_ceiling(hw[3]);
                    *reinterpret_cast<uint4 *>(p.y + ((unsigned)m * (unsigned)p.ldy + (unsigned)c)) = make_uint4(hw[0], hw[1], hw[2], hw[3]);
                    if (SPLIT) *reinterpret_cast<uint4 *>(p.y_lo + ((unsigned)m * (unsigned)p.ldy + (unsigned)c)) = make_uint4(lw[0], lw[1], lw[2], lw[3]);
                }
                continue;
            }
            if (m < p.m_end) {
                float v[8];
                const f32x4_t q0 = *reinterpret_cast<const f32x4_t *>(ct + lrow_e * CT_STRIDE + c8 * 8);
                const f32x4_t q1 = *reinterpret_cast<const f32x4_t *>(ct + lrow_e * CT_STRIDE + c8 * 8 + 4);
#pragma unroll
                for (int j = 0; j < 4; ++j) {
                    v[j] = q0[j];
                    v[4 + j] = q1[j];
                }
#pragma unroll
                for (int j = 0; j < 8; ++j) v[j] = v[j] * s1[j] + b1[j];
                const long long o = (long long)m * p.Cout + c;
                if (has_res) {
                    const int ri = PRE_ALL ? pass : pp;
                    const uint32_t rw[4] = {rres[ri].x, rres[ri].y, rres[ri].z, rres[ri].w};
#pragma unroll
                    for (int j = 0; j < 4; ++j) {
                        v[2 * j] += h16_to_f32((bf16_t)(rw[j] & 0xffffu), ET);
                        v[2 * j + 1] += h16_to_f32((bf16_t)(rw[j] >> 16), ET);
                    }
                    if (SPLIT) {
                        const uint32_t lw[4] = {rres_lo[ri].x, rres_lo[ri].y, rres_lo[ri].z, rres_lo[ri].w};
#pragma unroll
                        for (int j = 0; j < 4; ++j) {
                            v[2 * j] += h16_to_f32((bf16_t)(lw[j] & 0xffffu), ET);
                            v[2 * j + 1] += h16_to_f32((bf16_t)(lw[j] >> 16), ET);
                        }
                    }
                }
                if (p.relu) {
#pragma unroll
                    for (int j = 0; j < 8; ++j) v[j] = fmaxf(v[j], 0.f);
                }
                if (post) {
#pragma unroll
                    for (int j = 0; j < 8; ++j) v[j] = v[j] * s2[j] + b2[j];
                }
                if (p.y_f32 != nullptr) {
                    if (full && (p.Cout & 3) == 0) {
                        f32x4_t o0 = {v[0], v[1], v[2], v[3]}, o1 = {v[4], v[5], v[6], v[7]};
                        *reinterpret_cast<f32x4_t *>(p.y_f32 + o) = o0;
                        *reinterpret_cast<f32x4_t *>(p.y_f32 + o + 4) = o1;
                    } else {
                        for (int j = 0; j < 8 && c + j < p.Cout; ++j) p.y_f32[o + j] = v[j];
                    }
                }
                if (p.y != nullptr && full) {
                    uint32_t hw[4], lw[4];
#pragma unroll
                    for (int j = 0; j < 4; ++j) {
                        const bf16_t h0 = f32_to_h16(v[2 * j], ET), h1 = f32_to_h16(v[2 * j + 1], ET);
                        hw[j] = (uint32_t)h0 | ((uint32_t)h1 << 16);
                        if (SPLIT) {
                            const float c0 = ET ? fminf(fmaxf(v[2 * j], -65504.f), 65504.f) : v[2 * j];
                            const float c1 = ET ? fminf(fmaxf(v[2 * j + 1], -65504.f), 65504.f) : v[2 * j + 1];
                            const bf16_t l0 = f32_to_h16(c0 - h16_to_f32(h0, ET), ET);
                            const bf16_t l1 = f32_to_h16(c1 - h16_to_f32(h1, ET), ET);
                            lw[j] = (uint32_t)l0 | ((uint32_t)l1 << 16);
                        }
                    }
                    if (ET) ovf |= half2_at_ceiling(hw[0]) | half2_at_ceiling(hw[1]) | half2_at_ceiling(hw[2]) | half2_at_ceiling(hw[3]);
                    const long long oy = (long long)m * p.ldy + c;
                    *reinterpret_cast<uint4 *>(p.y + oy) = make_uint4(hw[0], hw[1], hw[2], hw[3]);
                    if (SPLIT) *reinterpret_cast<uint4 *>(p.y_lo + oy) = make_uint4(lw[0], lw[1], lw[2], lw[3]);
                }
            }
        }
    }
    if (ET && (ovf & 0x80008000u)) *p.range = (unsigned)p.Cout;
}

template <int BM, int BN, int MODE, int SPLIT, int ET, int STAGES, int WMT = 64, int FAST = 0, int WPT = 0>
int launch_stages(wsc_ctx *ctx, const ConvKArgs &a) {
    constexpr bool GLDS = MODE == 0;
    constexpr int A_BYTES = BM * BK * 2, B_BYTES = BN * BK * 2;
    constexpr int PIPE = WPT > 0 ? WPT * 4096 + STAGES * B_BYTES : STAGES * (A_BYTES + B_BYTES);
    constexpr int EPI = (STAGES == 1 ? 64 : (WMT == 128 ? 128 : BM)) * (BN + 4) * 4;
    constexpr int LDS = PIPE > EPI ? PIPE : EPI;
    static_assert(LDS <= 160 * 1024, "LDS budget of a CU");
    static bool attr_set[64] = {};
    auto kern = conv_igemm_kernel<BM, BN, MODE, SPLIT, ET, GLDS, STAGES, WMT, FAST, WPT>;
    const int dev = ctx->device >= 0 && ctx->device < 64 ? ctx->device : 0;
    int lds_req = LDS;
#ifdef WSC_AB_KNOBS
    static const int lds_pad = [] { const char *e = getenv("WSC_CONV_LDS_PAD"); return e ? atoi(e) : 0; }();
    if (STAGES == 2 && lds_pad > lds_req && lds_pad <= 160 * 1024) lds_req = lds_pad;
#endif
    if (!attr_set[dev] || ctx->device != dev) {
        WSC_HIP(hipFuncSetAttribute(reinterpret_cast<const void *>(kern),
                                    hipFuncAttributeMaxDynamicSharedMemorySize, lds_req > LDS ? 160 * 1024 : LDS));
        attr_set[dev] = true;
    }
    const double flops = 2.0 * (a.m_end - a.m_base) * a.Cout *
                         ((MODE == 0 && !a.stem_rows) ? (double)a.kh * a.kw * a.Cin : (double)a.kh * (a.stem_rows ? a.kw_real : a.kw) * 3);
    WscKernelTimer timer(ctx, (MODE != 0 || a.stem_rows) ? WSC_K_CONV_SMALLCIN : (BM == 256 ? WSC_K_CONV256 : (BN == 128 ? WSC_K_CONV128 : WSC_K_CONV64)), flops);
    hipLaunchKernelGGL(kern, dim3(a.nblocks), dim3(BM * 2), lds_req, ctx->stream, a);
    WSC_HIP(hipGetLastError());
    return WSC_OK;
}

template <int WPT, int BN = 128>
int launch_window(wsc_ctx *ctx, const ConvKArgs &a) {
    return launch_stages<128, BN, 0, 2, 1, 2, 64, 1, WPT>(ctx, a);
}

template <int BM, int BN, int MODE, int SPLIT, int ET, int FAST = 0>
int launch_variant(wsc_ctx *ctx, const ConvKArgs &a) {
    if constexpr (BM == 256 && BN == 256) {
        return launch_stages<BM, BN, MODE, SPLIT, ET, 2, 128, FAST>(ctx, a);
    } else if constexpr (BM == 256) {
        return launch_stages<BM, BN, MODE, SPLIT, ET, 3, 64, FAST>(ctx, a);
    } else if constexpr (MODE == 0) {
        if constexpr (SPLIT != 2)
            if (a.nk == 1) return launch_stages<BM, BN, MODE, SPLIT, ET, 1, 64, FAST>(ctx, a);
        return launch_stages<BM, BN, MODE, SPLIT, ET, 2, 64, FAST>(ctx, a);
    } else {
        if (a.nk == 1) return launch_stages<BM, BN, MODE, SPLIT, ET, 1, 64, FAST>(ctx, a);
        return launch_stages<BM, BN, MODE, SPLIT, ET, 2, 64, FAST>(ctx, a);
    }
}

template <int BM, int BN, int SPLIT = 0>
int launch_fast(wsc_ctx *ctx, const ConvKArgs &a, int fast) {
    if (fast == 3) return launch_variant<BM, BN, 0, SPLIT, 1, 3>(ctx, a);
    return launch_variant<BM, BN, 0, SPLIT, 1, 1>(ctx, a);
}

template <int BN>
int launch_bn(wsc_ctx *ctx, const ConvKArgs &a, int small_cin, int split, int fmt) {
    if (split == 2) {
        if (small_cin == 0 && a.fast == 3) return launch_variant<128, BN, 0, 2, 1, 3>(ctx, a);
        if (small_cin == 0 && a.fast) return launch_variant<128, BN, 0, 2, 1, 1>(ctx, a);
        if (small_cin == 0) return launch_variant<128, BN, 0, 2, 1>(ctx, a);
        if (small_cin == 1) return launch_variant<128, BN, 1, 1, 1>(ctx, a);
        return launch_variant<128, BN, 2, 1, 1>(ctx, a);
    }
    if (split) {
        if (small_cin == 0) return launch_variant<128, BN, 0, true, 0>(ctx, a);
        if (small_cin == 1) return launch_variant<128, BN, 1, true, 0>(ctx, a);
        return launch_variant<128, BN, 2, true, 0>(ctx, a);
    }
    if (fmt) {
        if (small_cin == 0 && a.fast) return launch_fast<128, BN>(ctx, a, a.fast);
        if (small_cin == 1 && a.fast) return launch_variant<128, BN, 1, false, 1, 1>(ctx, a);
        if (small_cin == 2 && a.fast) return launch_variant<128, BN, 2, false, 1, 1>(ctx, a);
        if (small_cin == 0) return launch_variant<128, BN, 0, false, 1>(ctx, a);
        if (small_cin == 1) return launch_variant<128, BN, 1, false, 1>(ctx, a);
        return launch_variant<128, BN, 2, false, 1>(ctx, a);
    }
    if (small_cin == 0) return launch_variant<128, BN, 0, false, 0>(ctx, a);
    if (small_cin == 1) return launch_variant<128, BN, 1, false, 0>(ctx, a);
    return launch_variant<128, BN, 2, false, 0>(ctx, a);
}

int launch_big(wsc_ctx *ctx, const ConvKArgs &a, int split, int fmt) {
    if (split) return launch_variant<256, 128, 0, true, 0>(ctx, a);
    if (fmt && a.fast) return launch_fast<256, 128>(ctx, a, a.fast);
    if (fmt) return launch_variant<256, 128, 0, false, 1>(ctx, a);
    return launch_variant<256, 128, 0, false, 0>(ctx, a);
}
int launch_square(wsc_ctx *ctx, const ConvKArgs &a, int split, int fmt) {
    if (split == 2) return a.fast ? launch_fast<256, 256, 2>(ctx, a, a.fast) : launch_variant<256, 256, 0, 2, 1>(ctx, a);
    if (split) return launch_variant<256, 256, 0, true, 0>(ctx, a);
    if (fmt && a.fast) return launch_fast<256, 256>(ctx, a, a.fast);
    if (fmt) return launch_variant<256, 256, 0, false, 1>(ctx, a);
    return launch_variant<256, 256, 0, false, 0>(ctx, a);
}

}

int conv_igemm_launch(wsc_ctx *ctx, const ConvLaunch &p) {
    ConvKArgs a;
    a.x = p.x; a.x_lo = p.x_lo; a.w = p.w;
    a.s1 = p.s1; a.b1 = p.b1; a.s2 = p.s2; a.b2 = p.b2;
    a.res = p.res; a.res_lo = p.res_lo;
    a.y = p.y; a.y_lo = p.y_lo; a.y_f32 = p.y_f32;
    a.H = p.H; a.W = p.W; a.Cin = p.Cin; a.Ho = p.Ho; a.Wo = p.Wo; a.Cout = p.Cout;
    a.ldy = p.ldy > 0 ? p.ldy : p.Cout;
    a.win_npix = 0;
    a.ldx = p.Cin; a.x2 = nullptr; a.lo_delta2 = 0; a.cc2 = 0; a.H2 = a.W2 = a.C2 = 0; a.stride2 = 1;
    a.kh = p.kh; a.kw = p.kw; a.stride = p.stride; a.pad = p.pad; a.relu = p.relu;
    a.M = p.N * p.Ho * p.Wo;
    a.m_base = 0;
    a.m_end = a.M;
    a.HoWo = p.Ho * p.Wo;
    auto fastdiv = [](unsigned d, unsigned &mul, unsigned &s1, unsigned &s2) {
        unsigned l = 0;
        while ((1ull << l) < d) ++l;
        mul = (unsigned)(((1ull << 32) * ((1ull << l) - d)) / d + 1);
        s1 = l < 1 ? l : 1;
        s2 = l > 0 ? l - 1 : 0;
    };
    fastdiv((unsigned)(a.HoWo > 0 ? a.HoWo : 1), a.div_howo_mul, a.div_howo_s1, a.div_howo_s2);
    fastdiv((unsigned)(p.Wo > 0 ? p.Wo : 1), a.div_wo_mul, a.div_wo_s1, a.div_wo_s2);
    WSC_CHECK(p.split >= 0 && p.split <= 2 && !(p.split == 1 && p.fmt) && !(p.split == 2 && !p.fmt), WSC_ERR_INVALID,
              "conv: split mode %d with operand format %d (bf16x3 = split 1 on bf16 planes, f16x3 = split 2 on half planes)", p.split, p.fmt);
    const bool stem_rows = p.small_cin == 3;
    if (stem_rows)
        WSC_CHECK(p.split == 2 && p.Cin == 4 && p.pad == 0 && p.kw <= 7 && (p.stride & 1) == 0, WSC_ERR_INVALID,
                  "conv: the padded-stem form needs split 2, a 4-channel padded input, kw <= 7 and an even stride");
    const int small_cin_eff = stem_rows ? 0 : p.small_cin;
    a.stem_rows = stem_rows ? 1 : 0;
    a.kw_real = p.kw;
    const bool single_staged = p.split == 2 && small_cin_eff == 0;
    if (stem_rows) {
        a.kw = 1;
        a.cchunks = 1;
        a.ntaps = p.kh;
        a.ksteps_base = p.kh;
    } else if (p.small_cin == 0) {
        WSC_CHECK(p.Cin % 64 == 0, WSC_ERR_INVALID, "conv: Cin=%d not a multiple of 64", p.Cin);
        a.cchunks = p.Cin / (single_staged ? 32 : 64);
        a.ntaps = p.kh * p.kw;
        a.ksteps_base = p.kh * p.kw * a.cchunks;
    } else {
        WSC_CHECK(p.Cin == 4, WSC_ERR_INVALID, "conv: small-Cin mode needs a 4-channel activation");
        a.cchunks = 1;
        a.ntaps = p.kh * p.kw;
        a.ksteps_base = ((p.kh << p.small_cin) + 7) / 8;
    }
    a.Kbase = a.ksteps_base * 64;
    a.Kw = a.Kbase * ((p.split && !single_staged) ? 2 : 1);
    a.nk = a.ksteps_base * ((p.split && !single_staged) ? 3 : 1);
    a.lo_delta = single_staged ? (long long)(p.x_lo - p.x) : 0;
    if (p.x2 != nullptr) {
        const int K1 = p.Cin - p.C2;
        WSC_CHECK(p.split != 1 && small_cin_eff == 0 && p.kh == 1 && p.kw == 1 && p.stride == 1 && p.pad == 0 && K1 > 0 &&
                  K1 % 64 == 0 && p.C2 % 64 == 0 && p.stride2 >= 1 && (p.Ho - 1) * p.stride2 < p.H2 && (p.Wo - 1) * p.stride2 < p.W2 &&
                  (!single_staged || p.x2_lo != nullptr),
                  WSC_ERR_INVALID, "conv: a second input needs a 1x1 / stride 1 layer, channel counts in multiples of 64 and no bf16x3");
        a.x2 = p.x2;
        a.lo_delta2 = single_staged ? (long long)(p.x2_lo - p.x2) : 0;
        a.cc2 = K1 / (single_staged ? 32 : 64);
        a.H2 = p.H2; a.W2 = p.W2; a.C2 = p.C2; a.stride2 = p.stride2;
        a.ldx = K1;
    }
    const int BN = p.CoutPad % 128 == 0 ? 128 : 64;
    WSC_CHECK(p.CoutPad % 64 == 0, WSC_ERR_INVALID, "conv: CoutPad=%d not a multiple of 64", p.CoutPad);
    a.ntiles_n = p.CoutPad / BN;
    a.zero = (const bf16_t *)ctx->zero_page;
    a.range = ctx->range_dev;
#ifdef WSC_AB_KNOBS
    static const int debug = [] { const char *e = getenv("WSC_CONV_DEBUG"); return e ? atoi(e) : 0; }();
    a.debug = debug;
#else
    a.debug = 0;
#endif
    const int nofast = p.generic;
    a.fast = 0;
    if (!nofast && p.fmt && (p.split == 0 || single_staged) && p.y != nullptr && p.y_f32 == nullptr &&
        p.Cout == p.CoutPad && (long long)a.M * a.ldy < (1ll << 31)) {
        a.fast = 1;
        if (small_cin_eff == 0 && p.kh == 1 && p.kw == 1 && p.pad == 0 && p.stride == 1) a.fast = 3;
    }
    if (a.M == 0) return WSC_OK;
#ifdef WSC_AB_KNOBS
    static const int force = [] { const char *e = getenv("WSC_CONV_TILE"); return e ? atoi(e) : 0; }();
#else
    constexpr int force = 0;
#endif
    const long long blocks256 = ((a.M + 255) / 256) * (long long)a.ntiles_n;
    bool big = false;
    if (force == -1) big = small_cin_eff == 0 && BN == 128 && a.Kbase >= 512 && blocks256 >= 200;
    if (force == 256) big = small_cin_eff == 0 && BN == 128;
    const long long blocks_sq = ((a.M + 255) / 256) * (long long)(p.CoutPad / 256);
    bool square = small_cin_eff == 0 && p.CoutPad % 256 == 0 && a.nk >= 4 && blocks_sq >= 192;
    if (force == 512) square = small_cin_eff == 0 && p.CoutPad % 256 == 0;
    if (force != 0 && force != 512) square = false;
    if (p.split == 2) big = false;
    if (p.x2 != nullptr) big = false;
    if (p.split == 2 && !a.fast) square = false;
    if (p.split == 2 && force == 0 && a.nk < 16) square = false;
    if (square) {
        const int ntn = p.CoutPad / 256;
        const long long rounds = blocks_sq / ctx->num_cus, rem = blocks_sq - rounds * ctx->num_cus;
#ifdef WSC_AB_KNOBS
        static const int nosplit = [] { const char *e = getenv("WSC_CONV_NOSPLIT"); return e ? atoi(e) : 0; }();
#else
        constexpr int nosplit = 0;
#endif
        if (!nosplit && rounds >= 1 && rem > 0 && rem * 2 <= ctx->num_cus && ctx->num_cus > 0) {
            const int big_rows = (int)((rounds * ctx->num_cus) / ntn);
            ConvKArgs b = a;
            b.ntiles_n = ntn;
            b.m_end = big_rows * 256;
            b.nblocks = big_rows * ntn;
            WSC_TRY(launch_square(ctx, b, p.split, p.fmt));
            a.m_base = big_rows * 256;
            a.nblocks = ((a.M - a.m_base + 127) / 128) * a.ntiles_n;
            return launch_bn<128>(ctx, a, small_cin_eff, p.split, p.fmt);
        }
        a.ntiles_n = ntn;
        a.nblocks = (int)blocks_sq;
        return launch_square(ctx, a, p.split, p.fmt);
    }
    const int BMsel = big ? 256 : 128;
    a.nblocks = ((a.M + BMsel - 1) / BMsel) * a.ntiles_n;
    if (!big && single_staged && a.fast == 1 && p.kh == 3 && p.kw == 3 && p.stride == 1 && p.pad == 1 && p.x2 == nullptr &&
        p.Ho == p.H && p.Wo == p.W && ctx->opt[WSC_OPT_CONV_WINDOW] != 0) {
        const long long need = 127 + 2ll * p.W + 3 + 1;
        const long long npix = (long long)p.N * p.H * p.W;
        if (need <= 320 && npix < (1ll << 30) && a.lo_delta >= 0 && npix * p.Cin + a.lo_delta < (1ll << 33) && (a.lo_delta & 7) == 0) {
            a.win_npix = (int)npix;
            if (BN == 128) return need <= 256 ? launch_window<8>(ctx, a) : launch_window<10>(ctx, a);
            return need <= 256 ? launch_window<8, 64>(ctx, a) : launch_window<10, 64>(ctx, a);
        }
    }
    if (big) return launch_big(ctx, a, p.split, p.fmt);
    if (BN == 128) return launch_bn<128>(ctx, a, small_cin_eff, p.split, p.fmt);
    return launch_bn<64>(ctx, a, small_cin_eff, p.split, p.fmt);
}
```

### wsss-analysis_amd/csrc/net.hip

```cpp
#include "common.h"

#include <algorithm>
#include <cmath>
#include <cstring>
#include <unordered_map>

namespace {

struct HostTensor {
    const float *data;
    int ndim;
    int64_t shape[4];
    int64_t numel() const {
        int64_t n = 1;
        for (int i = 0; i < ndim; ++i) n *= shape[i];
        return n;
    }
};
typedef std::unordered_map<std::string, HostTensor> Dict;

struct ConvW {
    bf16_t *w = nullptr;
    float *s1 = nullptr, *b1 = nullptr, *s2 = nullptr, *b2 = nullptr;
    int Cin = 0, Cout = 0, CoutPad = 0, kh = 1, kw = 1, stride = 1, pad = 0, relu = 0, small_cin = 0;
};

struct IrnHead {
    ConvW conv;
    int groups = 1, up = 1;
    float *gamma = nullptr, *beta = nullptr;
    int src = 0;
    int dst = 0, coff = 0;
};
struct IrnCat {
    int channels, stage, stride;
};

enum OpType { OP_CONV = 0, OP_POOL = 1, OP_GATHER = 2 };
struct Op {
    int type;
    int conv;
    int in, out, res;
    int pk, ps, pp;
    int pitch = 0;
    int coff = 0;
    int in2 = -1;
};

}

struct wsc_net {
    wsc_ctx *ctx = nullptr;
    int arch = 0, C = 0, split = 0, fmt = 0, F = 0;
    std::vector<ConvW> convs;
    std::vector<Op> ops;
    int final_buf = 0;
    ConvW head;
    float *cls_w = nullptr, *cls_b = nullptr;
    int Ccls = 0;
    int cls_max = 0;
    std::vector<int> taps;
    std::vector<IrnHead> heads;
    std::vector<IrnCat> cats;
    ConvW edge6, dp7b;
    float mean_shift[2] = {0.f, 0.f};
    std::vector<void *> allocs;
};

namespace {

int upload(wsc_net *net, const void *host, size_t bytes, void **out) {
    void *d = nullptr;
    WSC_HIP(hipMalloc(&d, bytes));
    net->allocs.push_back(d);
    WSC_HIP(hipMemcpy(d, host, bytes, hipMemcpyHostToDevice));
    *out = d;
    return WSC_OK;
}

int get(const Dict &d, const std::string &k, int ndim, const HostTensor **out) {
    auto it = d.find(k);
    WSC_CHECK(it != d.end(), WSC_ERR_MISSING_KEY, "state_dict: missing key '%s'", k.c_str());
    WSC_CHECK(it->second.ndim == ndim, WSC_ERR_SHAPE, "state_dict: '%s' has ndim %d, expected %d", k.c_str(),
              it->second.ndim, ndim);
    WSC_CHECK(it->second.data != nullptr, WSC_ERR_INVALID, "state_dict: '%s' has a null data pointer", k.c_str());
    *out = &it->second;
    return WSC_OK;
}
bool has(const Dict &d, const std::string &k) { return d.find(k) != d.end(); }

int fold_bn(const Dict &d, const std::string &bn, int C, double eps_default, std::vector<float> &s,
            std::vector<float> &b) {
    const HostTensor *g, *be, *mu, *var;
    WSC_TRY(get(d, bn + ".weight", 1, &g));
    WSC_TRY(get(d, bn + ".bias", 1, &be));
    WSC_TRY(get(d, bn + ".running_mean", 1, &mu));
    WSC_TRY(get(d, bn + ".running_var", 1, &var));
    WSC_CHECK(g->shape[0] == C && be->shape[0] == C && mu->shape[0] == C && var->shape[0] == C, WSC_ERR_SHAPE,
              "state_dict: batch-norm '%s' is not %d channels", bn.c_str(), C);
    double eps = eps_default;
    auto it = d.find(bn + ".eps");
    if (it != d.end() && it->second.data) eps = it->second.data[0];
    s.resize(C);
    b.resize(C);
    for (int c = 0; c < C; ++c) {
        const double sc = (double)g->data[c] / std::sqrt((double)var->data[c] + eps);
        s[c] = (float)sc;
        b[c] = (float)((double)be->data[c] - (double)mu->data[c] * sc);
    }
    return WSC_OK;
}

int make_conv(wsc_net *net, const HostTensor *w, int stride, int pad, int relu, int small_cin,
              const std::vector<float> &s1, const std::vector<float> &b1, const std::vector<float> *s2,
              const std::vector<float> *b2, ConvW *out) {
    const int Cout = (int)w->shape[0], Cin = (int)w->shape[1], kh = (int)w->shape[2], kw = (int)w->shape[3];
    ConvW c;
    c.Cout = Cout;
    c.CoutPad = Cout <= 64 ? 64 : ((Cout + 127) / 128) * 128;
    c.kh = kh; c.kw = kw; c.stride = stride; c.pad = pad; c.relu = relu; c.small_cin = small_cin;
    int Kbase;
    if (small_cin == 0) {
        WSC_CHECK(Cin % 64 == 0, WSC_ERR_SHAPE, "conv with Cin=%d is not supported (need a multiple of 64)", Cin);
        c.Cin = Cin;
        Kbase = kh * kw * Cin;
    } else if (small_cin == 3) {
        WSC_CHECK(Cin <= 4 && kw <= 7 && net->split == 2, WSC_ERR_SHAPE, "padded-stem conv needs Cin <= 4, kw <= 7, f16x3");
        c.Cin = 4;
        Kbase = kh * 32;
    } else {
        WSC_CHECK(Cin <= 4, WSC_ERR_SHAPE, "small-Cin conv needs Cin <= 4, got %d", Cin);
        WSC_CHECK(kw <= (2 << small_cin), WSC_ERR_SHAPE, "small-Cin conv: kw=%d too wide", kw);
        c.Cin = 4;
        Kbase = (((kh << small_cin) + 7) / 8) * 64;
    }
    const int planes = net->split ? 2 : 1;
    const int Kw = Kbase * planes;
    const bool interleaved = net->split == 2 && (small_cin == 0 || small_cin == 3);
    std::vector<bf16_t> wp((size_t)c.CoutPad * Kw, 0);
    std::vector<float> s1v(s1);
    std::vector<float> wscale(Cout, 1.f);
    if (net->fmt == 1) {
        const size_t per = (size_t)Cin * kh * kw;
        for (int co = 0; co < Cout; ++co) {
            float mx = 0.f;
            for (size_t i = 0; i < per; ++i) mx = std::max(mx, std::fabs(w->data[(size_t)co * per + i]));
            if (!(mx > 0.f) || !std::isfinite(mx)) continue;
            int e;
            std::frexp(mx, &e);
            const int sh = std::max(std::min(13 - e, 100), -100);
            wscale[co] = std::ldexp(1.f, sh);
            s1v[co] = s1[co] * std::ldexp(1.f, -sh);
        }
    }
    for (int co = 0; co < Cout; ++co) {
        bf16_t *row = wp.data() + (size_t)co * Kw;
        const float wsc = wscale[co];
        auto put = [&](int k, float v) {
            v *= wsc;
            const bf16_t h = f32_to_h16(v, net->fmt);
            const int lo_at = interleaved ? 32 : Kbase;
            row[k] = h;
            if (net->split) row[lo_at + k] = f32_to_h16(v - h16_to_f32(h, net->fmt), net->fmt);
        };
        for (int ci = 0; ci < Cin; ++ci)
            for (int r = 0; r < kh; ++r)
                for (int s = 0; s < kw; ++s) {
                    const float v = w->data[(((size_t)co * Cin + ci) * kh + r) * kw + s];
                    if (small_cin == 3) {
                        put(r * 64 + s * 4 + ci, v);
                    } else if (interleaved) {
                        put((((ci >> 5) * kh + r) * kw + s) * 64 + (ci & 31), v);
                    } else if (small_cin == 0) {
                        put((((ci >> 6) * kh + r) * kw + s) * 64 + (ci & 63), v);
                    } else {
                        put((r << small_cin) * 8 + s * 4 + ci, v);
                    }
                }
    }
    WSC_TRY(upload(net, wp.data(), wp.size() * sizeof(bf16_t), (void **)&c.w));
    auto up_vec = [&](const std::vector<float> &v, float **dst) -> int {
        std::vector<float> p(c.CoutPad, 0.f);
        for (int i = 0; i < Cout; ++i) p[i] = v[i];
        return upload(net, p.data(), p.size() * sizeof(float), (void **)dst);
    };
    WSC_TRY(up_vec(s1v, &c.s1));
    WSC_TRY(up_vec(b1, &c.b1));
    if (s2) {
        WSC_TRY(up_vec(*s2, &c.s2));
        WSC_TRY(up_vec(*b2, &c.b2));
    }
    *out = c;
    return WSC_OK;
}

int add_conv_op(wsc_net *net, const ConvW &c, int in, int out, int res) {
    net->convs.push_back(c);
    Op op;
    op.type = OP_CONV; op.conv = (int)net->convs.size() - 1; op.in = in; op.out = out; op.res = res;
    op.pk = op.ps = op.pp = 0;
    net->ops.push_back(op);
    return WSC_OK;
}
void add_pool_op(wsc_net *net, int k, int s, int p, int in, int out) {
    Op op;
    op.type = OP_POOL; op.conv = -1; op.in = in; op.out = out; op.res = -1; op.pk = k; op.ps = s; op.pp = p;
    net->ops.push_back(op);
}

int resnet_conv(wsc_net *net, const Dict &d, const std::string &conv, const std::string &bn, int stride, int pad,
                int relu, int small_cin, int in, int out, int res) {
    const HostTensor *w;
    WSC_TRY(get(d, conv + ".weight", 4, &w));
    std::vector<float> s, b;
    WSC_TRY(fold_bn(d, bn, (int)w->shape[0], 1e-5, s, b));
    ConvW c;
    WSC_TRY(make_conv(net, w, stride, pad, relu, small_cin, s, b, nullptr, nullptr, &c));
    return add_conv_op(net, c, in, out, res);
}

int build_resnet50_backbone(wsc_net *net, const Dict &d) {
    WSC_TRY(resnet_conv(net, d, "resnet50.conv1", "resnet50.bn1", 2, 3, 1,  net->split == 2 ? 3 : 2, -1, 0, -1));
    add_pool_op(net, 3, 2, 1, 0, 1);
    net->taps.push_back((int)net->ops.size() - 1);
    int cur = 1;
    bool fuse_shortcut = true;
#ifdef WSC_AB_KNOBS
    if (const char *e = getenv("WSC_NET_SHORTCUT_FUSED")) fuse_shortcut = atoi(e) != 0;
#endif
    const int planes[4] = {64, 128, 256, 512};
    const int blocks[4] = {3, 4, 6, 3};
    const int strides[4] = {1, 2, 2, 1};
    for (int L = 0; L < 4; ++L) {
        (void)planes;
        for (int bi = 0; bi < blocks[L]; ++bi) {
            const std::string pre = "resnet50.layer" + std::to_string(L + 1) + "." + std::to_string(bi);
            const int s = bi == 0 ? strides[L] : 1;
            int f[3], nf = 0;
            for (int i = 0; i < 4 && nf < 3; ++i)
                if (i != cur) f[nf++] = i;
            WSC_TRY(resnet_conv(net, d, pre + ".conv1", pre + ".bn1", 1, 0, 1, 0, cur, f[0], -1));
            bool fuse_here = false;
            if (has(d, pre + ".downsample.0.weight") && has(d, pre + ".conv3.weight") && fuse_shortcut) {
                const HostTensor *w3, *wd;
                WSC_TRY(get(d, pre + ".conv3.weight", 4, &w3));
                WSC_TRY(get(d, pre + ".downsample.0.weight", 4, &wd));
                fuse_here = wd->shape[0] == w3->shape[0] && w3->shape[2] == 1 && w3->shape[3] == 1 && wd->shape[2] == 1 &&
                            wd->shape[3] == 1 && w3->shape[1] % 8 == 0 && wd->shape[1] % 8 == 0 &&
                            (w3->shape[1] + wd->shape[1]) % 64 == 0;
            }
            if (fuse_here) {
                const HostTensor *w3, *wd;
                WSC_TRY(get(d, pre + ".conv3.weight", 4, &w3));
                WSC_TRY(get(d, pre + ".downsample.0.weight", 4, &wd));
                const int Co = (int)w3->shape[0], K1 = (int)w3->shape[1], K2 = (int)wd->shape[1];
                std::vector<float> s3, b3, sd, bd;
                WSC_TRY(fold_bn(d, pre + ".bn3", Co, 1e-5, s3, b3));
                WSC_TRY(fold_bn(d, pre + ".downsample.1", Co, 1e-5, sd, bd));
                std::vector<float> wc((size_t)Co * (K1 + K2)), sig(Co), sh(Co);
                for (int co = 0; co < Co; ++co) {
                    float g = std::max(std::fabs(s3[co]), std::fabs(sd[co]));
                    if (!(g > 0.f)) g = 1.f;
                    sig[co] = g;
                    sh[co] = b3[co] + bd[co];
                    for (int k = 0; k < K1; ++k) wc[(size_t)co * (K1 + K2) + k] = w3->data[(size_t)co * K1 + k] * (s3[co] / g);
                    for (int k = 0; k < K2; ++k) wc[(size_t)co * (K1 + K2) + K1 + k] = wd->data[(size_t)co * K2 + k] * (sd[co] / g);
                }
                HostTensor wt;
                wt.data = wc.data(); wt.ndim = 4; wt.shape[0] = Co; wt.shape[1] = K1 + K2; wt.shape[2] = 1; wt.shape[3] = 1;
                WSC_TRY(resnet_conv(net, d, pre + ".conv2", pre + ".bn2", s, 1, 1, 0, f[0], f[1], -1));
                ConvW c;
                WSC_TRY(make_conv(net, &wt, 1, 0, 1, 0, sig, sh, nullptr, nullptr, &c));
                if (net->split != 1) {
                    WSC_TRY(add_conv_op(net, c, f[1], f[0], -1));
                    net->ops.back().in2 = cur;
                    net->ops.back().ps = s;
                } else {
                    net->ops.back().pitch = K1 + K2;
                    net->ops.back().coff = 0;
                    Op g;
                    g.type = OP_GATHER; g.conv = -1; g.in = cur; g.out = f[1]; g.res = -1; g.pk = 1; g.ps = s; g.pp = 0;
                    g.pitch = K1 + K2; g.coff = K1;
                    net->ops.push_back(g);
                    WSC_TRY(add_conv_op(net, c, f[1], f[0], -1));
                }
                cur = f[0];
                continue;
            }
            WSC_TRY(resnet_conv(net, d, pre + ".conv2", pre + ".bn2", s, 1, 1, 0, f[0], f[1], -1));
            int res = cur;
            if (has(d, pre + ".downsample.0.weight")) {
                WSC_TRY(resnet_conv(net, d, pre + ".downsample.0", pre + ".downsample.1", s, 0, 0, 0, cur, f[2], -1));
                res = f[2];
            }
            WSC_TRY(resnet_conv(net, d, pre + ".conv3", pre + ".bn3", 1, 0, 1, 0, f[1], f[0], res));
            cur = f[0];
        }
        net->taps.push_back((int)net->ops.size() - 1);
    }
    net->final_buf = cur;
    return WSC_OK;
}

int build_resnet50(wsc_net *net, const Dict &d) {
    WSC_TRY(build_resnet50_backbone(net, d));
    const HostTensor *cw;
    WSC_TRY(get(d, "classifier.weight", 4, &cw));
    WSC_CHECK(cw->shape[0] == net->C && cw->shape[2] == 1 && cw->shape[3] == 1, WSC_ERR_SHAPE,
              "classifier.weight must be [%d][F][1][1]", net->C);
    net->F = (int)cw->shape[1];
    std::vector<float> one(net->C, 1.f), zero(net->C, 0.f);
    WSC_TRY(make_conv(net, cw, 1, 0, 0, 0, one, zero, nullptr, nullptr, &net->head));
    return WSC_OK;
}

int build_plain_stack(wsc_net *net, const Dict &d, const std::string &root,
                      const std::vector<std::pair<std::string, std::vector<int>>> &cfg, int *cur_io,
                      int *feat_channels, std::vector<int> *layer_taps = nullptr) {
    int cur = *cur_io;
    int in_ch = 3;
    bool first = true;
    for (const auto &layer : cfg) {
        int idx = 0;
        for (int v : layer.second) {
            if (v == -1) {
                const int out = (cur + 1) & 1;
                add_pool_op(net, 2, 2, 0, cur, out);
                cur = out;
                idx += 1;
            } else if (v == -2) {
                idx += 1;
            } else {
                const std::string key = root + "." + layer.first + "." + std::to_string(idx);
                const HostTensor *w, *bias;
                WSC_TRY(get(d, key + ".weight", 4, &w));
                WSC_TRY(get(d, key + ".bias", 1, &bias));
                WSC_CHECK(w->shape[0] == v && w->shape[1] == in_ch && w->shape[2] == 3 && w->shape[3] == 3,
                          WSC_ERR_SHAPE, "'%s.weight' must be [%d][%d][3][3]", key.c_str(), v, in_ch);
                std::vector<float> one(v, 1.f), bb(bias->data, bias->data + v);
                const std::string bn = root + "." + layer.first + "." + std::to_string(idx + 2);
                ConvW c;
                if (has(d, bn + ".running_mean")) {
                    std::vector<float> s2, b2;
                    WSC_TRY(fold_bn(d, bn, v, 1e-3, s2, b2));
                    WSC_TRY(make_conv(net, w, 1, 1, 1, first ? 1 : 0, one, bb, &s2, &b2, &c));
                    idx += 3;
                } else {
                    WSC_TRY(make_conv(net, w, 1, 1, 1, first ? 1 : 0, one, bb, nullptr, nullptr, &c));
                    idx += 2;
                }
                const int in = first ? -1 : cur;
                const int out = first ? 0 : ((cur + 1) & 1);
                WSC_TRY(add_conv_op(net, c, in, out, -1));
                cur = out;
                in_ch = v;
                first = false;
            }
        }
        if (layer_taps) layer_taps->push_back((int)net->ops.size() - 1);
    }
    *cur_io = cur;
    *feat_channels = in_ch;
    return WSC_OK;
}

int gradcam_bias(const Dict &d, int C, std::vector<float> &bias) {
    bias.assign(C, 0.f);
    if (!has(d, "gradcam_bias")) return WSC_OK;
    const HostTensor *gb;
    WSC_TRY(get(d, "gradcam_bias", 1, &gb));
    WSC_CHECK(gb->shape[0] == C, WSC_ERR_SHAPE, "gradcam_bias must be [%d]", C);
    for (int c = 0; c < C; ++c) bias[c] = gb->data[c];
    return WSC_OK;
}

int build_vgg16(wsc_net *net, const Dict &d) {
    const std::vector<std::pair<std::string, std::vector<int>>> cfg = {
        {"layer1", {64, 64, -1}},
        {"layer2", {128, 128, -1}},
        {"layer3", {256, 256, 256, -1}},
        {"layer4", {512, 512, 512, 512, 512, 512}},
        {"layer5", {1024, -2, 1024, -2}}};
    int cur = 0;
    WSC_TRY(build_plain_stack(net, d, "vgg16", cfg, &cur, &net->F));
    net->final_buf = cur;
    const HostTensor *lw;
    WSC_TRY(get(d, "vgg16.classifier.0.weight", 2, &lw));
    WSC_CHECK(lw->shape[0] >= net->C && lw->shape[1] == net->F, WSC_ERR_SHAPE,
              "vgg16.classifier.0.weight must be [>=%d][%d]", net->C, net->F);
    HostTensor hw = *lw;
    hw.ndim = 4; hw.shape[0] = net->C; hw.shape[2] = 1; hw.shape[3] = 1;
    std::vector<float> one(net->C, 1.f), zero(net->C, 0.f);
    std::vector<float> wt;
    if (has(d, "gradcam_weights")) {
        const HostTensor *gw;
        WSC_TRY(get(d, "gradcam_weights", 2, &gw));
        WSC_CHECK(gw->shape[0] == net->F && gw->shape[1] == net->C, WSC_ERR_SHAPE,
                  "gradcam_weights must be [%d][%d]", net->F, net->C);
        wt.resize((size_t)net->C * net->F);
        for (int f = 0; f < net->F; ++f)
            for (int c = 0; c < net->C; ++c) wt[(size_t)c * net->F + f] = gw->data[(size_t)f * net->C + c];
        hw.data = wt.data();
        WSC_TRY(gradcam_bias(d, net->C, zero));
    }
    WSC_TRY(make_conv(net, &hw, 1, 0, 0, 0, one, zero, nullptr, nullptr, &net->head));
    net->Ccls = net->C;
    net->cls_max = 0;
    WSC_TRY(upload(net, lw->data, (size_t)net->C * net->F * sizeof(float), (void **)&net->cls_w));
    if (has(d, "vgg16.classifier.0.bias")) {
        const HostTensor *lb;
        WSC_TRY(get(d, "vgg16.classifier.0.bias", 1, &lb));
        WSC_TRY(upload(net, lb->data, (size_t)net->C * sizeof(float), (void **)&net->cls_b));
    }
    return WSC_OK;
}

int build_m7(wsc_net *net, const Dict &d) {
    const std::vector<std::pair<std::string, std::vector<int>>> cfg = {
        {"layer1", {64, 64, -1}}, {"layer2", {128, 128, -1}}, {"layer3_p1", {256, 256, 256}}};
    int cur = 0;
    WSC_TRY(build_plain_stack(net, d, "m7", cfg, &cur, &net->F));
    net->final_buf = cur;
    const HostTensor *gw;
    WSC_TRY(get(d, "gradcam_weights", 2, &gw));
    WSC_CHECK(gw->shape[0] == net->F && gw->shape[1] == net->C, WSC_ERR_SHAPE, "gradcam_weights must be [%d][%d]",
              net->F, net->C);
    std::vector<float> wt((size_t)net->C * net->F);
    for (int f = 0; f < net->F; ++f)
        for (int c = 0; c < net->C; ++c) wt[(size_t)c * net->F + f] = gw->data[(size_t)f * net->C + c];
    HostTensor hw;
    hw.data = wt.data(); hw.ndim = 4; hw.shape[0] = net->C; hw.shape[1] = net->F; hw.shape[2] = 1; hw.shape[3] = 1;
    std::vector<float> one(net->C, 1.f), zero(net->C, 0.f);
    WSC_TRY(gradcam_bias(d, net->C, zero));
    WSC_TRY(make_conv(net, &hw, 1, 0, 0, 0, one, zero, nullptr, nullptr, &net->head));
    const HostTensor *lw;
    WSC_TRY(get(d, "m7.classifier.0.weight", 2, &lw));
    WSC_CHECK(lw->shape[0] >= net->C && lw->shape[1] == net->F, WSC_ERR_SHAPE,
              "m7.classifier.0.weight must be [>=%d][%d]", net->C, net->F);
    net->Ccls = net->C;
    net->cls_max = 1;
    WSC_TRY(upload(net, lw->data, (size_t)net->C * net->F * sizeof(float), (void **)&net->cls_w));
    if (has(d, "m7.classifier.0.bias")) {
        const HostTensor *lb;
        WSC_TRY(get(d, "m7.classifier.0.bias", 1, &lb));
        WSC_TRY(upload(net, lb->data, (size_t)net->C * sizeof(float), (void **)&net->cls_b));
    }
    return WSC_OK;
}

struct HeadSpec {
    const char *name;
    int src, stride, cout, groups, up, dst, coff;
};

int add_irn_head(wsc_net *net, const Dict &d, const HeadSpec &hs, int cin_pad) {
    const HostTensor *w, *g, *b;
    const std::string nm = hs.name;
    WSC_TRY(get(d, nm + ".0.weight", 4, &w));
    WSC_TRY(get(d, nm + ".1.weight", 1, &g));
    WSC_TRY(get(d, nm + ".1.bias", 1, &b));
    WSC_CHECK(w->shape[0] == hs.cout && w->shape[2] == 1 && w->shape[3] == 1 && g->shape[0] == hs.cout &&
                  b->shape[0] == hs.cout,
              WSC_ERR_SHAPE, "'%s': expected a 1x1 conv with %d outputs + GroupNorm", hs.name, hs.cout);
    (void)cin_pad;
    IrnHead h;
    std::vector<float> one(hs.cout, 1.f), zero(hs.cout, 0.f);
    WSC_TRY(make_conv(net, w, hs.stride, 0, 0, 0, one, zero, nullptr, nullptr, &h.conv));
    h.groups = hs.groups; h.up = hs.up; h.src = hs.src; h.dst = hs.dst; h.coff = hs.coff;
    WSC_TRY(upload(net, g->data, sizeof(float) * hs.cout, (void **)&h.gamma));
    WSC_TRY(upload(net, b->data, sizeof(float) * hs.cout, (void **)&h.beta));
    net->heads.push_back(h);
    return WSC_OK;
}

int build_irn_heads(wsc_net *net, const Dict &d, const std::vector<HeadSpec> &specs, const std::vector<IrnCat> &cats,
                    const std::string &edge_final, int edge_in, const std::string &dp_final) {
    net->cats = cats;
    for (const HeadSpec &hs : specs) WSC_TRY(add_irn_head(net, d, hs, 0));
    const HostTensor *w6, *b6, *w7;
    WSC_TRY(get(d, edge_final + ".weight", 4, &w6));
    WSC_TRY(get(d, edge_final + ".bias", 1, &b6));
    WSC_CHECK(w6->shape[0] == 1 && w6->shape[1] == edge_in, WSC_ERR_SHAPE, "%s.weight must be [1][%d][1][1]",
              edge_final.c_str(), edge_in);
    const int cin_pad = cats[0].channels;
    std::vector<float> w6p(cin_pad, 0.f);
    for (int i = 0; i < edge_in; ++i) w6p[i] = w6->data[i];
    HostTensor t6;
    t6.data = w6p.data(); t6.ndim = 4; t6.shape[0] = 1; t6.shape[1] = cin_pad; t6.shape[2] = 1; t6.shape[3] = 1;
    std::vector<float> one1(1, 1.f), bias1(1, b6->data[0]);
    WSC_TRY(make_conv(net, &t6, 1, 0, 0, 0, one1, bias1, nullptr, nullptr, &net->edge6));
    WSC_TRY(get(d, dp_final + ".weight", 4, &w7));
    WSC_CHECK(w7->shape[0] == 2 && w7->shape[1] == cats.back().channels, WSC_ERR_SHAPE, "%s.weight must be [2][%d][1][1]",
              dp_final.c_str(), cats.back().channels);
    std::vector<float> one2(2, 1.f), zero2(2, 0.f);
    WSC_TRY(make_conv(net, w7, 1, 0, 0, 0, one2, zero2, nullptr, nullptr, &net->dp7b));
    if (has(d, "mean_shift.running_mean")) {
        const HostTensor *ms;
        WSC_TRY(get(d, "mean_shift.running_mean", 1, &ms));
        WSC_CHECK(ms->shape[0] == 2, WSC_ERR_SHAPE, "mean_shift.running_mean must have 2 entries");
        net->mean_shift[0] = ms->data[0];
        net->mean_shift[1] = ms->data[1];
    }
    return WSC_OK;
}

const std::vector<IrnCat> IRN_CATS5 = {{192, 2, 1}, {768, 3, 1}, {448, 2, 1}, {256, 2, 1}};

int build_resnet50_irn(wsc_net *net, const Dict &d) {
    WSC_TRY(build_resnet50_backbone(net, d));
    const std::vector<HeadSpec> specs = {
        {"fc_edge1", 1, 1, 32, 4, 1, 0, 0},   {"fc_edge2", 2, 1, 32, 4, 1, 0, 32},  {"fc_edge3", 3, 1, 32, 4, 2, 0, 64},
        {"fc_edge4", 4, 1, 32, 4, 4, 0, 96},  {"fc_edge5", 5, 1, 32, 4, 4, 0, 128}, {"fc_dp1", 1, 1, 64, 8, 1, 2, 0},
        {"fc_dp2", 2, 1, 128, 16, 1, 2, 64},  {"fc_dp3", 3, 1, 256, 16, 1, 1, 0},   {"fc_dp4", 4, 1, 256, 16, 2, 1, 256},
        {"fc_dp5", 5, 1, 256, 16, 2, 1, 512}, {"fc_dp6", -2, 1, 256, 16, 2, 2, 192}, {"fc_dp7", -3, 1, 256, 16, 1, 3, 0}};
    return build_irn_heads(net, d, specs, IRN_CATS5, "fc_edge6", 160, "fc_dp7.3");
}

int build_vgg16_irn(wsc_net *net, const Dict &d) {
    const std::vector<std::pair<std::string, std::vector<int>>> cfg = {
        {"layer1", {64, 64, -1}},
        {"layer2", {128, 128, -1}},
        {"layer3", {256, 256, 256, -1}},
        {"layer4", {512, 512, 512, 512, 512, 512}},
        {"layer5", {1024, -2, 1024, -2}}};
    int cur = 0;
    WSC_TRY(build_plain_stack(net, d, "vgg16", cfg, &cur, &net->F, &net->taps));
    net->final_buf = cur;
    const std::vector<HeadSpec> specs = {
        {"fc_edge1", 1, 2, 32, 4, 1, 0, 0},   {"fc_edge2", 2, 1, 32, 4, 1, 0, 32},  {"fc_edge3", 3, 1, 32, 4, 2, 0, 64},
        {"fc_edge4", 4, 1, 32, 4, 2, 0, 96},  {"fc_edge5", 5, 1, 32, 4, 2, 0, 128}, {"fc_dp1", 1, 2, 64, 8, 1, 2, 0},
        {"fc_dp2", 2, 1, 128, 16, 1, 2, 64},  {"fc_dp3", 3, 1, 256, 16, 1, 1, 0},   {"fc_dp4", 4, 1, 256, 16, 1, 1, 256},
        {"fc_dp5", 5, 1, 256, 16, 1, 1, 512}, {"fc_dp6", -2, 1, 256, 16, 2, 2, 192}, {"fc_dp7", -3, 1, 256, 16, 1, 3, 0}};
    return build_irn_heads(net, d, specs, IRN_CATS5, "fc_edge6", 160, "fc_dp7.3");
}

int build_m7_irn(wsc_net *net, const Dict &d) {
    const std::vector<std::pair<std::string, std::vector<int>>> cfg = {
        {"layer1", {64, 64, -1}}, {"layer2", {128, 128, -1}}, {"layer3_p1", {256, 256, 256}}, {"layer3_p2", {-1, -2}}};
    int cur = 0;
    std::vector<int> layer_taps;
    WSC_TRY(build_plain_stack(net, d, "m7", cfg, &cur, &net->F, &layer_taps));
    net->final_buf = cur;
    net->taps = {layer_taps[0], layer_taps[1], layer_taps[3]};
    const std::vector<IrnCat> cats = {{128, 1, 1}, {256, 3, 1}, {448, 2, 1}, {256, 2, 1}};
    const std::vector<HeadSpec> specs = {
        {"fc_edge1", 1, 1, 32, 4, 1, 0, 0},  {"fc_edge2", 2, 1, 32, 4, 2, 0, 32},  {"fc_edge3", 3, 1, 32, 4, 4, 0, 64},
        {"fc_dp1", 1, 2, 64, 8, 1, 2, 0},    {"fc_dp2", 2, 1, 128, 16, 1, 2, 64},  {"fc_dp3", 3, 1, 256, 16, 1, 1, 0},
        {"fc_dp4", -2, 1, 256, 16, 2, 2, 192}, {"fc_dp5", -3, 1, 256, 16, 1, 3, 0}};
    return build_irn_heads(net, d, specs, cats, "fc_edge4", 96, "fc_dp5.3");
}

inline size_t align_up(size_t v, size_t a) { return (v + a - 1) / a * a; }

struct Plan {
    std::vector<int> H, W, C;
    size_t max_act = 0;
    int hf = 0, wf = 0;
};

int plan_dims(const wsc_net *net, int N, int SH, int SW, Plan *pl);
int plan_dims(const wsc_net *net, int N, int S, Plan *pl) { return plan_dims(net, N, S, S, pl); }
int plan_dims(const wsc_net *net, int N, int SH, int SW, Plan *pl) {
    int bh[4] = {0, 0, 0, 0}, bw[4] = {0, 0, 0, 0}, bc[4] = {0, 0, 0, 0};
    pl->max_act = 0;
    for (const Op &op : net->ops) {
        int H = op.in < 0 ? SH : bh[op.in], W = op.in < 0 ? SW : bw[op.in], C = op.in < 0 ? 4 : bc[op.in];
        int Ho, Wo, Co;
        if (op.type == OP_CONV) {
            const ConvW &c = net->convs[op.conv];
            Ho = (H + 2 * c.pad - c.kh) / c.stride + 1;
            Wo = (W + 2 * c.pad - c.kw) / c.stride + 1;
            Co = op.pitch ? op.pitch : c.Cout;
            if (op.in2 >= 0) {
                WSC_CHECK(c.kh == 1 && c.kw == 1 && c.stride == 1 && (H - 1) * op.ps < bh[op.in2] && (W - 1) * op.ps < bw[op.in2],
                          WSC_ERR_INVALID, "internal: second input of a %d x %d layer does not cover its %d x %d output", c.kh, c.kw, H, W);
                C += bc[op.in2];
            }
            WSC_CHECK(C == c.Cin, WSC_ERR_INVALID, "internal: channel mismatch %d vs %d", C, c.Cin);
        } else if (op.type == OP_GATHER) {
            Ho = (H - 1) / op.ps + 1;
            Wo = (W - 1) / op.ps + 1;
            Co = op.pitch;
            WSC_CHECK(Ho == bh[op.out] && Wo == bw[op.out] && bc[op.out] == op.pitch && op.coff + C <= op.pitch, WSC_ERR_INVALID,
                      "internal: gather into a %d x %d x %d tensor does not fit", bh[op.out], bw[op.out], bc[op.out]);
        } else {
            Ho = (H + 2 * op.pp - op.pk) / op.ps + 1;
            Wo = (W + 2 * op.pp - op.pk) / op.ps + 1;
            Co = C;
        }
        WSC_CHECK(Ho > 0 && Wo > 0, WSC_ERR_INVALID, "input size %d x %d too small for this network", SH, SW);
        bh[op.out] = Ho; bw[op.out] = Wo; bc[op.out] = Co;
        pl->H.push_back(Ho); pl->W.push_back(Wo); pl->C.push_back(Co);
        const size_t e = (size_t)N * Ho * Wo * Co;
        if (e > pl->max_act) pl->max_act = e;
    }
    pl->hf = bh[net->final_buf];
    pl->wf = bw[net->final_buf];
    return WSC_OK;
}

size_t tap_plane_bytes(const wsc_net *net, const Plan &pl, int N, int k) {
    const int op = net->taps[k];
    return align_up((size_t)N * pl.H[op] * pl.W[op] * pl.C[op] * sizeof(bf16_t), 256);
}

int run_backbone(wsc_ctx *ctx, const wsc_net *net, const float *x_dev, int N, int S, size_t extra_bytes,
                 const bf16_t **feat, const bf16_t **feat_lo, int *hf, int *wf, void **extra, bool copy_taps = false, int SW = 0) {
    if (SW <= 0) SW = S;
    Plan pl;
    WSC_TRY(plan_dims(net, N, S, SW, &pl));
    const int planes = net->split ? 2 : 1;
    int in_h = S, in_w = SW, in_pad = 0;
    bool fused_stem = false;
    if (!net->ops.empty() && net->ops[0].type == OP_CONV && net->ops[0].in < 0 && net->convs[net->ops[0].conv].small_cin == 3) {
        const ConvW &c0 = net->convs[net->ops[0].conv];
        in_h = (pl.H[0] - 1) * c0.stride + c0.kh;
        in_w = (pl.W[0] - 1) * c0.stride + 8;
        in_pad = c0.pad;
        bool tapped = false;
        for (int tp : net->taps) tapped = tapped || tp == 0;
        fused_stem = ctx->opt[WSC_OPT_STEM_POOL_FUSED] && net->ops.size() > 1 && net->ops[1].type == OP_POOL &&
                     net->ops[1].in == net->ops[0].out && net->ops[1].pk == 3 && net->ops[1].ps == 2 && net->ops[1].pp == 1 &&
                     c0.kh == 7 && c0.kw == 7 && c0.stride == 2 && c0.pad == 3 && c0.Cout == 64 && c0.s2 == nullptr &&
                     net->ops[0].res < 0 && net->fmt == 1 && !tapped;
        if (fused_stem) {
            stem_pool_input_dims(S, SW, &in_h, &in_w);
            in_pad = 5;
        }
    }
    const size_t in_bytes = align_up((size_t)N * in_h * in_w * 4 * sizeof(bf16_t), 256);
    const size_t act_bytes = align_up(pl.max_act * sizeof(bf16_t), 256);
    const size_t total = in_bytes * planes + act_bytes * 4 * planes + align_up(extra_bytes, 256);
    void *ws;
    WSC_TRY(wsc_ctx_workspace(ctx, total, &ws));
    char *p = (char *)ws;
    bf16_t *xin = (bf16_t *)p; p += in_bytes;
    bf16_t *xin_lo = nullptr;
    if (net->split) { xin_lo = (bf16_t *)p; p += in_bytes; }
    bf16_t *buf[4], *buf_lo[4] = {nullptr, nullptr, nullptr, nullptr};
    for (int i = 0; i < 4; ++i) {
        buf[i] = (bf16_t *)p; p += act_bytes;
        if (net->split) { buf_lo[i] = (bf16_t *)p; p += act_bytes; }
    }
    *extra = (void *)p;

    if (in_pad > 0) WSC_TRY(launch_nchw_to_nhwc4_pad(ctx, x_dev, N, S, SW, in_h, in_w, in_pad, xin, xin_lo, net->fmt));
    else WSC_TRY(launch_nchw_to_nhwc4(ctx, x_dev, N, S, SW, xin, xin_lo, net->fmt));
    int bh[4] = {0, 0, 0, 0}, bw[4] = {0, 0, 0, 0}, bc[4] = {0, 0, 0, 0};
    for (size_t i = 0; i < net->ops.size(); ++i) {
        const Op &op = net->ops[i];
        const int H = op.in < 0 ? S : bh[op.in], W = op.in < 0 ? SW : bw[op.in], C = op.in < 0 ? 4 : bc[op.in];
        const bf16_t *src = op.in < 0 ? xin : buf[op.in];
        const bf16_t *src_lo = op.in < 0 ? xin_lo : buf_lo[op.in];
        if (fused_stem && i == 0) continue;
        if (fused_stem && i == 1) {
            const ConvW &c0 = net->convs[net->ops[0].conv];
            WSC_TRY(launch_stem_pool(ctx, xin, xin_lo, N, S, SW, c0.w, c0.kh * 64, c0.s1, c0.b1, c0.relu, buf[op.out], buf_lo[op.out]));
        } else if (op.type == OP_CONV) {
            const ConvW &c = net->convs[op.conv];
            ConvLaunch L;
            memset(&L, 0, sizeof(L));
            L.x = src; L.x_lo = src_lo; L.w = c.w;
            L.s1 = c.s1; L.b1 = c.b1; L.s2 = c.s2; L.b2 = c.b2;
            L.res = op.res >= 0 ? buf[op.res] : nullptr;
            L.res_lo = op.res >= 0 ? buf_lo[op.res] : nullptr;
            L.y = buf[op.out]; L.y_lo = buf_lo[op.out]; L.y_f32 = nullptr;
            if (op.in2 >= 0) {
                L.x2 = buf[op.in2]; L.x2_lo = buf_lo[op.in2];
                L.H2 = bh[op.in2]; L.W2 = bw[op.in2]; L.C2 = bc[op.in2]; L.stride2 = op.ps;
            }
            L.ldy = op.pitch;
            if (op.pitch) {
                L.y += op.coff;
                if (L.y_lo) L.y_lo += op.coff;
            }
            L.N = N; L.H = H; L.W = W; L.Cin = c.Cin; L.Ho = pl.H[i]; L.Wo = pl.W[i];
            L.Cout = c.Cout; L.CoutPad = c.CoutPad;
            L.kh = c.kh; L.kw = c.kw; L.stride = c.stride; L.pad = c.pad; L.relu = c.relu;
            L.small_cin = c.small_cin; L.split = net->split; L.fmt = net->fmt;
            if (c.small_cin == 3 && op.in < 0) {
                L.H = in_h; L.W = in_w; L.pad = 0;
            }
            WSC_TRY(conv_igemm_launch(ctx, L));
        } else if (op.type == OP_GATHER) {
            WSC_TRY(launch_gather_strided(ctx, src, src_lo, N, H, W, C, op.ps, pl.H[i], pl.W[i], buf[op.out] + op.coff,
                                          buf_lo[op.out] ? buf_lo[op.out] + op.coff : nullptr, op.pitch));
        } else {
            WSC_TRY(launch_maxpool(ctx, src, src_lo, N, H, W, C, op.pk, op.ps, op.pp, pl.H[i], pl.W[i], buf[op.out],
                                   buf_lo[op.out], net->fmt));
        }
        bh[op.out] = pl.H[i]; bw[op.out] = pl.W[i]; bc[op.out] = pl.C[i];
        if (copy_taps)
            for (size_t k = 0; k < net->taps.size(); ++k)
                if (net->taps[k] == (int)i) {
                    char *dst = (char *)*extra;
                    for (size_t j = 0; j < k; ++j) dst += tap_plane_bytes(net, pl, N, (int)j) * planes;
                    const size_t nb = (size_t)N * pl.H[i] * pl.W[i] * pl.C[i] * sizeof(bf16_t);
                    WSC_HIP(hipMemcpyAsync(dst, buf[op.out], nb, hipMemcpyDeviceToDevice, ctx->stream));
                    if (net->split)
                        WSC_HIP(hipMemcpyAsync(dst + tap_plane_bytes(net, pl, N, (int)k), buf_lo[op.out], nb,
                                               hipMemcpyDeviceToDevice, ctx->stream));
                }
    }
    *feat = buf[net->final_buf];
    *feat_lo = buf_lo[net->final_buf];
    *hf = pl.hf;
    *wf = pl.wf;
    return WSC_OK;
}

}

extern "C" {

int wsc_net_create(wsc_ctx *ctx, int arch, const wsc_tensor_desc *weights, int n_weights, int num_classes,
                   int precision, wsc_net **out) {
    WSC_CHECK(ctx && weights && out && n_weights > 0, WSC_ERR_INVALID, "wsc_net_create: null argument");
    WSC_CHECK(num_classes > 0 && num_classes <= 64, WSC_ERR_INVALID, "num_classes=%d outside [1,64]", num_classes);
    WSC_CHECK(precision == WSC_PREC_BF16 || precision == WSC_PREC_BF16X3 || precision == WSC_PREC_F16 ||
                  precision == WSC_PREC_F16X3,
              WSC_ERR_INVALID, "unknown precision %d", precision);
    WSC_HIP(hipSetDevice(ctx->device));
    Dict d;
    for (int i = 0; i < n_weights; ++i) {
        WSC_CHECK(weights[i].name != nullptr, WSC_ERR_INVALID, "weights[%d].name is null", i);
        WSC_CHECK(weights[i].ndim >= 0 && weights[i].ndim <= 4, WSC_ERR_SHAPE, "'%s': ndim %d unsupported",
                  weights[i].name, weights[i].ndim);
        HostTensor t;
        t.data = weights[i].data;
        t.ndim = weights[i].ndim;
        for (int k = 0; k < 4; ++k) t.shape[k] = k < t.ndim ? weights[i].shape[k] : 1;
        if (t.ndim == 0) { t.ndim = 1; t.shape[0] = 1; }
        d[weights[i].name] = t;
    }
    wsc_net *net = new wsc_net();
    net->ctx = ctx;
    net->arch = arch;
    net->C = num_classes;
    net->split = precision == WSC_PREC_BF16X3 ? 1 : (precision == WSC_PREC_F16X3 ? 2 : 0);
    net->fmt = (precision == WSC_PREC_F16 || precision == WSC_PREC_F16X3) ? 1 : 0;
    int st;
    switch (arch) {
    case WSC_ARCH_RESNET50_CAM: st = build_resnet50(net, d); break;
    case WSC_ARCH_VGG16_CAM: st = build_vgg16(net, d); break;
    case WSC_ARCH_M7_CAM: st = build_m7(net, d); break;
    case WSC_ARCH_RESNET50_IRN: st = build_resnet50_irn(net, d); break;
    case WSC_ARCH_VGG16_IRN: st = build_vgg16_irn(net, d); break;
    case WSC_ARCH_M7_IRN: st = build_m7_irn(net, d); break;
    default:
        wsc_set_error("unknown arch %d", arch);
        st = WSC_ERR_INVALID;
    }
    if (st != WSC_OK) {
        wsc_net_destroy(net);
        return st;
    }
    *out = net;
    return WSC_OK;
}

void wsc_net_destroy(wsc_net *net) {
    if (!net) return;
    for (void *p : net->allocs) (void)hipFree(p);
    delete net;
}

int wsc_net_cam_size(const wsc_net *net, int S, int *h_out) {
    WSC_CHECK(net && h_out, WSC_ERR_INVALID, "wsc_net_cam_size: null argument");
    Plan pl;
    WSC_TRY(plan_dims(net, 1, S, &pl));
    *h_out = pl.hf;
    return WSC_OK;
}

int wsc_net_feat_channels(const wsc_net *net, int *f_out) {
    WSC_CHECK(net && f_out, WSC_ERR_INVALID, "wsc_net_feat_channels: null argument");
    *f_out = net->F;
    return WSC_OK;
}

int wsc_net_cam_size_hw(const wsc_net *net, int H, int W, int *h_out, int *w_out) {
    WSC_CHECK(net && h_out && w_out, WSC_ERR_INVALID, "wsc_net_cam_size_hw: null argument");
    Plan pl;
    WSC_TRY(plan_dims(net, 1, H, W, &pl));
    *h_out = pl.hf;
    *w_out = pl.wf;
    return WSC_OK;
}

static int run_head(wsc_ctx *ctx, const wsc_net *net, const ConvLaunch &L) {
    if (L.fmt == 1 && L.split != 1 && L.Cout <= 32 && L.CoutPad >= 32 && L.Cin % 256 == 0 && L.y_f32 != nullptr &&
        ctx->opt[WSC_OPT_CAM_HEAD_STREAM] != 0) {
        const int st = launch_cam_head(ctx, L.x, L.split == 2 ? L.x_lo : nullptr, L.N * L.Ho * L.Wo, L.Cin, L.w,
                                       L.Cin * (L.split == 2 ? 2 : 1), L.CoutPad, L.s1, L.b1, L.Cout, L.relu, L.y_f32);
        if (st != WSC_ERR_INVALID) return st;
    }
    (void)net;
    return conv_igemm_launch(ctx, L);
}

int wsc_net_forward_cam(wsc_ctx *ctx, const wsc_net *net, const float *x_dev, int B, int S, float *cam_dev,
                        float *score_dev) {
    return wsc_net_forward_cam_hw(ctx, net, x_dev, B, S, S, cam_dev, score_dev);
}

int wsc_net_forward_cam_hw(wsc_ctx *ctx, const wsc_net *net, const float *x_dev, int B, int S, int SW, float *cam_dev,
                           float *score_dev) {
    WSC_CHECK(ctx && net && x_dev && cam_dev, WSC_ERR_INVALID, "wsc_net_forward_cam: null argument");
    WSC_CHECK(B > 0 && S > 0 && SW > 0, WSC_ERR_INVALID, "wsc_net_forward_cam: B=%d input %d x %d", B, S, SW);
    WSC_CHECK(score_dev == nullptr || net->cls_w != nullptr, WSC_ERR_INVALID,
              "this architecture has no classifier branch (score_dev must be NULL)");
    WSC_HIP(hipSetDevice(ctx->device));
    const int N = 2 * B;
    Plan pl;
    WSC_TRY(plan_dims(net, N, S, SW, &pl));
    const size_t head_bytes = (size_t)N * pl.hf * pl.wf * net->C * sizeof(float);
    const bf16_t *feat, *feat_lo;
    int hf, wf;
    void *extra;
    WSC_TRY(run_backbone(ctx, net, x_dev, N, S, head_bytes, &feat, &feat_lo, &hf, &wf, &extra, false, SW));
    float *head_out = (float *)extra;
    ConvLaunch L;
    memset(&L, 0, sizeof(L));
    const ConvW &c = net->head;
    L.x = feat; L.x_lo = feat_lo; L.w = c.w; L.s1 = c.s1; L.b1 = c.b1;
    L.y_f32 = head_out;
    L.N = N; L.H = hf; L.W = wf; L.Cin = c.Cin; L.Ho = hf; L.Wo = wf; L.Cout = c.Cout; L.CoutPad = c.CoutPad;
    L.kh = 1; L.kw = 1; L.stride = 1; L.pad = 0; L.relu = 0; L.small_cin = 0; L.split = net->split; L.fmt = net->fmt;
    WSC_TRY(run_head(ctx, net, L));
    WSC_TRY(launch_flip_add(ctx, head_out, B, hf, wf, net->C, net->C, cam_dev));
    if (score_dev != nullptr)
        WSC_TRY(launch_gap_linear_sigmoid(ctx, feat, feat_lo, B, net->cls_max ? -(hf * wf) : hf * wf, net->F,
                                          net->cls_w, net->cls_b, net->Ccls, score_dev, net->fmt, 2));
    return WSC_OK;
}

int wsc_net_forward_gradcam(wsc_ctx *ctx, const wsc_net *net, const float *x_dev, int N, int S, int relu,
                            float *cams_dev, float *score_dev) {
    WSC_CHECK(ctx && net && x_dev && cams_dev, WSC_ERR_INVALID, "wsc_net_forward_gradcam: null argument");
    WSC_CHECK(N > 0 && S > 0, WSC_ERR_INVALID, "wsc_net_forward_gradcam: N=%d S=%d", N, S);
    WSC_CHECK(score_dev == nullptr || net->cls_w != nullptr, WSC_ERR_INVALID,
              "this architecture has no classifier branch (score_dev must be NULL)");
    WSC_HIP(hipSetDevice(ctx->device));
    const bf16_t *feat, *feat_lo;
    int hf, wf;
    void *extra;
    WSC_TRY(run_backbone(ctx, net, x_dev, N, S, 0, &feat, &feat_lo, &hf, &wf, &extra));
    ConvLaunch L;
    memset(&L, 0, sizeof(L));
    const ConvW &c = net->head;
    L.x = feat; L.x_lo = feat_lo; L.w = c.w; L.s1 = c.s1; L.b1 = c.b1;
    L.y_f32 = cams_dev;
    L.N = N; L.H = hf; L.W = wf; L.Cin = c.Cin; L.Ho = hf; L.Wo = wf; L.Cout = c.Cout; L.CoutPad = c.CoutPad;
    L.kh = 1; L.kw = 1; L.stride = 1; L.pad = 0; L.relu = relu ? 1 : 0; L.small_cin = 0; L.split = net->split;
    L.fmt = net->fmt;
    WSC_TRY(run_head(ctx, net, L));
    if (score_dev != nullptr)
        WSC_TRY(launch_gap_linear_sigmoid(ctx, feat, feat_lo, N, net->cls_max ? -(hf * wf) : hf * wf, net->F,
                                          net->cls_w, net->cls_b, net->Ccls, score_dev, net->fmt, 1));
    return WSC_OK;
}

int wsc_net_forward_features(wsc_ctx *ctx, const wsc_net *net, const float *x_dev, int N, int S, float *feat_dev) {
    WSC_CHECK(ctx && net && x_dev && feat_dev, WSC_ERR_INVALID, "wsc_net_forward_features: null argument");
    WSC_CHECK(N > 0 && S > 0, WSC_ERR_INVALID, "wsc_net_forward_features: N=%d S=%d", N, S);
    WSC_HIP(hipSetDevice(ctx->device));
    const bf16_t *feat, *feat_lo;
    int hf, wf;
    void *extra;
    WSC_TRY(run_backbone(ctx, net, x_dev, N, S, 0, &feat, &feat_lo, &hf, &wf, &extra));
    return launch_bf16_to_f32(ctx, feat, feat_lo, (size_t)N * hf * wf * net->F, feat_dev, net->fmt);
}

int wsc_net_forward_edge(wsc_ctx *ctx, const wsc_net *net, const float *x_dev, int B, int S, int feat_h, int feat_w,
                         float *edge_dev, float *dp_dev) {
    WSC_CHECK(ctx && net && x_dev && edge_dev && dp_dev, WSC_ERR_INVALID, "wsc_net_forward_edge: null argument");
    WSC_CHECK(!net->heads.empty() && net->cats.size() >= 2, WSC_ERR_INVALID,
              "wsc_net_forward_edge: the network is not an IRNet EdgeDisplacement net");
    WSC_CHECK(B > 0 && S > 0 && feat_h > 0 && feat_w > 0, WSC_ERR_INVALID, "wsc_net_forward_edge: B=%d S=%d", B, S);
    WSC_HIP(hipSetDevice(ctx->device));
    const int N = 2 * B;
    const int planes = net->split ? 2 : 1;
    Plan pl;
    WSC_TRY(plan_dims(net, N, S, &pl));
    const int NS = (int)net->taps.size(), NC = (int)net->cats.size();
    std::vector<int> Hs(NS), Ws(NS), Cs(NS);
    std::vector<size_t> tap_off(NS);
    size_t off = 0;
    for (int k = 0; k < NS; ++k) {
        const int op = net->taps[k];
        Hs[k] = pl.H[op]; Ws[k] = pl.W[op]; Cs[k] = pl.C[op];
        tap_off[k] = off;
        off += tap_plane_bytes(net, pl, N, k) * planes;
    }
    auto outdim = [](int v, int stride) { return (v - 1) / stride + 1; };
    std::vector<int> cat_c(NC), cat_h(NC), cat_w(NC);
    std::vector<size_t> cat_off(NC), cat_bytes(NC);
    for (int i = 0; i < NC; ++i) {
        const IrnCat &c = net->cats[i];
        cat_c[i] = c.channels;
        cat_h[i] = outdim(Hs[c.stage - 1], c.stride);
        cat_w[i] = outdim(Ws[c.stage - 1], c.stride);
        cat_bytes[i] = align_up((size_t)N * cat_h[i] * cat_w[i] * cat_c[i] * sizeof(bf16_t), 256);
        cat_off[i] = off;
        off += cat_bytes[i] * planes;
    }
    const int He = cat_h[0], We = cat_w[0], Hd = cat_h[NC - 1], Wd = cat_w[NC - 1];
    WSC_CHECK(feat_h <= He && feat_w <= We && feat_h <= Hd && feat_w <= Wd, WSC_ERR_INVALID,
              "feature size %dx%d exceeds the head resolution %dx%d / %dx%d", feat_h, feat_w, He, We, Hd, Wd);
    size_t ftmp_elems = 0, part_bytes = 0;
    int max_groups = 1;
    for (const IrnHead &h : net->heads) {
        const int sh = h.src > 0 ? Hs[h.src - 1] : cat_h[-h.src - 1];
        const int sw = h.src > 0 ? Ws[h.src - 1] : cat_w[-h.src - 1];
        const int ho = outdim(sh, h.conv.stride), wo = outdim(sw, h.conv.stride);
        ftmp_elems = std::max(ftmp_elems, (size_t)N * ho * wo * h.conv.Cout);
        part_bytes = std::max(part_bytes, group_norm_partial_bytes(N, ho, wo, h.groups));
        max_groups = std::max(max_groups, h.groups);
    }
    const size_t ftmp_off = off; off += align_up(ftmp_elems * sizeof(float), 256);
    const size_t part_off = off; off += align_up(part_bytes, 256);
    const size_t stat_off = off; off += align_up(sizeof(float) * 2 * N * max_groups, 256);
    const size_t e_off = off; off += align_up(sizeof(float) * (size_t)N * He * We, 256);
    const size_t d_off = off; off += align_up(sizeof(float) * (size_t)N * Hd * Wd * 2, 256);

    const bf16_t *feat, *feat_lo;
    int hf, wf;
    void *extra;
    WSC_TRY(run_backbone(ctx, net, x_dev, N, S, off, &feat, &feat_lo, &hf, &wf, &extra, true));
    char *base = (char *)extra;
    WSC_HIP(hipMemsetAsync(base + cat_off[0], 0, cat_bytes[0] * planes, ctx->stream));

    auto plane = [&](size_t o, size_t bytes, int which) -> bf16_t * {
        return which == 0 ? (bf16_t *)(base + o) : (net->split ? (bf16_t *)(base + o + bytes) : nullptr);
    };
    auto run_conv = [&](const ConvW &c, const bf16_t *x, const bf16_t *x_lo, int H, int W, float *y_f32) -> int {
        ConvLaunch L;
        memset(&L, 0, sizeof(L));
        L.x = x; L.x_lo = x_lo; L.w = c.w;
        L.s1 = c.s1; L.b1 = c.b1; L.s2 = nullptr; L.b2 = nullptr;
        L.y = nullptr; L.y_lo = nullptr; L.y_f32 = y_f32;
        L.N = N; L.H = H; L.W = W; L.Cin = c.Cin; L.Ho = outdim(H, c.stride); L.Wo = outdim(W, c.stride);
        L.Cout = c.Cout; L.CoutPad = c.CoutPad;
        L.kh = 1; L.kw = 1; L.stride = c.stride; L.pad = 0; L.relu = 0;
        L.small_cin = 0; L.split = net->split; L.fmt = net->fmt;
        return conv_igemm_launch(ctx, L);
    };
    float *ftmp = (float *)(base + ftmp_off);
    for (const IrnHead &h : net->heads) {
        const bf16_t *x, *x_lo;
        int sh, sw, sc;
        if (h.src > 0) {
            const int k = h.src - 1;
            const size_t pb = tap_plane_bytes(net, pl, N, k);
            x = plane(tap_off[k], pb, 0); x_lo = plane(tap_off[k], pb, 1);
            sh = Hs[k]; sw = Ws[k]; sc = Cs[k];
        } else {
            const int ci = -h.src - 1;
            x = plane(cat_off[ci], cat_bytes[ci], 0); x_lo = plane(cat_off[ci], cat_bytes[ci], 1);
            sh = cat_h[ci]; sw = cat_w[ci]; sc = cat_c[ci];
        }
        WSC_CHECK(sc == h.conv.Cin, WSC_ERR_SHAPE, "IRNet head: %d input channels, the weights expect %d", sc, h.conv.Cin);
        WSC_TRY(run_conv(h.conv, x, x_lo, sh, sw, ftmp));
        const int ho = outdim(sh, h.conv.stride), wo = outdim(sw, h.conv.stride);
        WSC_TRY(launch_group_norm_stats(ctx, ftmp, N, ho, wo, h.conv.Cout, h.groups, 1e-5f, base + part_off,
                                        base + stat_off));
        const int di = h.dst;
        WSC_TRY(launch_group_norm_apply(ctx, ftmp, base + stat_off, h.gamma, h.beta, N, ho, wo, h.conv.Cout, h.groups,
                                        h.up, 1, plane(cat_off[di], cat_bytes[di], 0), plane(cat_off[di], cat_bytes[di], 1),
                                        cat_h[di], cat_w[di], cat_c[di], h.coff, net->fmt));
    }
    float *e_out = (float *)(base + e_off), *d_out = (float *)(base + d_off);
    WSC_TRY(run_conv(net->edge6, plane(cat_off[0], cat_bytes[0], 0), plane(cat_off[0], cat_bytes[0], 1), He, We, e_out));
    WSC_TRY(run_conv(net->dp7b, plane(cat_off[NC - 1], cat_bytes[NC - 1], 0), plane(cat_off[NC - 1], cat_bytes[NC - 1], 1),
                     Hd, Wd, d_out));
    WSC_TRY(launch_edge_finish(ctx, e_out, He, We, d_out, Hd, Wd, B, feat_h, feat_w, net->mean_shift[0],
                               net->mean_shift[1], edge_dev, dp_dev));
    return WSC_OK;
}

int wsc_conv2d_nchw(wsc_ctx *ctx, const float *x_dev, int N, int Cin, int H, int W, const float *w_host, int Cout,
                    int kh, int kw, int stride, int pad, const float *scale_host, const float *shift_host,
                    const float *residual_dev, int relu, int precision, float *y_dev) {
    WSC_CHECK(ctx && x_dev && w_host && y_dev, WSC_ERR_INVALID, "wsc_conv2d_nchw: null argument");
    WSC_CHECK(Cout % 8 == 0, WSC_ERR_INVALID, "wsc_conv2d_nchw: Cout=%d must be a multiple of 8", Cout);
    WSC_HIP(hipSetDevice(ctx->device));
    wsc_net tmp;
    tmp.ctx = ctx;
    const int generic = (precision & WSC_CONV_GENERIC) ? 1 : 0;
    precision &= ~WSC_CONV_GENERIC;
    WSC_CHECK(precision >= WSC_PREC_BF16 && precision <= WSC_PREC_F16X3, WSC_ERR_INVALID, "unknown precision %d", precision);
    tmp.split = precision == WSC_PREC_BF16X3 ? 1 : (precision == WSC_PREC_F16X3 ? 2 : 0);
    tmp.fmt = (precision == WSC_PREC_F16 || precision == WSC_PREC_F16X3) ? 1 : 0;
    HostTensor wt;
    wt.data = w_host; wt.ndim = 4; wt.shape[0] = Cout; wt.shape[1] = Cin; wt.shape[2] = kh; wt.shape[3] = kw;
    std::vector<float> s1(Cout, 1.f), b1(Cout, 0.f);
    if (scale_host) s1.assign(scale_host, scale_host + Cout);
    if (shift_host) b1.assign(shift_host, shift_host + Cout);
    int small = 0;
    if (Cin <= 4) small = kw <= 4 ? 1 : 2;
    if (small == 2 && tmp.split == 2 && (stride & 1) == 0 && kw <= 7) small = 3;
    ConvW c;
    int st = make_conv(&tmp, &wt, stride, pad, relu, small, s1, b1, nullptr, nullptr, &c);
    auto cleanup = [&]() {
        (void)hipStreamSynchronize(ctx->stream);
// ... 40 lines not shown
```

### wsss-analysis_amd/wsscam/_lib.py

```python
import ctypes
import os
import re
import threading

import numpy as np

_HERE = os.path.dirname(os.path.abspath(__file__))
LIB_PATH = os.path.join(_HERE, "libwsscam.so")
HEADER_PATH = os.path.normpath(os.path.join(_HERE, "..", "..", "include", "wsscam.h"))

WSC_OK = 0
WSC_ERR_INVALID = -1
WSC_ERR_NO_DEVICE = -2
WSC_ERR_HIP = -3
WSC_ERR_MISSING_KEY = -4
WSC_ERR_SHAPE = -5
WSC_ERR_NOMEM = -6
WSC_ERR_KEY_RANGE = -7
WSC_ERR_CAPACITY = -8
WSC_ERR_RANGE = -9

ARCH_RESNET50_CAM = 0
ARCH_VGG16_CAM = 1
ARCH_M7_CAM = 2
ARCH_RESNET50_IRN = 3
ARCH_VGG16_IRN = 4
ARCH_M7_IRN = 5

PREC_BF16 = 0
PREC_BF16X3 = 1
PREC_F16 = 2
PREC_F16X3 = 3
OPT_CRF_GAUSS_ON_CHIP, OPT_CRF_FUSED_BLUR, OPT_CRF_BLUR_ON_CHIP, OPT_CRF_RANK_BALLOT, OPT_CRF_EMBED_FULL, OPT_RW_TILED, \
    OPT_STEM_POOL_FUSED, OPT_CONV_WINDOW, OPT_CAM_HEAD_STREAM, OPT_CRF_MSG_IN_UPDATE = range(10)
OPT_DEFAULTS = {OPT_CRF_GAUSS_ON_CHIP: 1, OPT_CRF_FUSED_BLUR: 1, OPT_CRF_BLUR_ON_CHIP: 1, OPT_CRF_RANK_BALLOT: 0,
                OPT_CRF_EMBED_FULL: 0, OPT_RW_TILED: -1, OPT_STEM_POOL_FUSED: 1, OPT_CONV_WINDOW: 1, OPT_CAM_HEAD_STREAM: 1,
                OPT_CRF_MSG_IN_UPDATE: 1}
CONV_GENERIC = 0x100


class WscError(RuntimeError):
    def __init__(self, status, message):
        super().__init__("libwsscam error %d: %s" % (status, message))
        self.status = status


class TensorDesc(ctypes.Structure):
    _fields_ = [
        ("name", ctypes.c_char_p),
        ("data", ctypes.POINTER(ctypes.c_float)),
        ("ndim", ctypes.c_int32),
        ("shape", ctypes.c_int64 * 4),
    ]


_lib = None

_vp = ctypes.c_void_p
_i = ctypes.c_int
_f = ctypes.c_float
_sz = ctypes.c_size_t

_SIGNATURES = {
    "wsc_version": (_i, []),
    "wsc_last_error": (ctypes.c_char_p, []),
    "wsc_ctx_create": (_i, [_i, _vp, ctypes.POINTER(_vp)]),
    "wsc_ctx_destroy": (None, [_vp]),
    "wsc_sync": (_i, [_vp]),
    "wsc_ctx_range_status": (_i, [_vp, ctypes.POINTER(_i), _i]),
    "wsc_ctx_wait": (_i, [_vp, _vp]),
    "wsc_ctx_mark": (_i, [_vp, _i]),
    "wsc_ctx_wait_mark": (_i, [_vp, _i]),
    "wsc_ctx_wait_for_mark": (_i, [_vp, _vp, _i]),
    "wsc_device_info": (_i, [_vp, ctypes.c_char_p, _sz, ctypes.POINTER(_i)]),
    "wsc_malloc": (_i, [_vp, _sz, ctypes.POINTER(_vp)]),
    "wsc_free": (_i, [_vp, _vp]),
    "wsc_memcpy_h2d": (_i, [_vp, _vp, _vp, _sz]),
    "wsc_memcpy_d2h": (_i, [_vp, _vp, _vp, _sz]),
    "wsc_memset": (_i, [_vp, _vp, _i, _sz]),
    "wsc_ctx_set_option": (_i, [_vp, _i, _i]),
    "wsc_host_alloc": (_i, [_vp, _sz, ctypes.POINTER(_vp)]),
    "wsc_host_free": (_i, [_vp, _vp]),
    "wsc_host_write_segments": (_i, [ctypes.c_char_p, _i, ctypes.POINTER(_vp), ctypes.POINTER(_sz)]),
    "wsc_memcpy_h2d_async": (_i, [_vp, _vp, _vp, _sz]),
    "wsc_memcpy_d2h_async": (_i, [_vp, _vp, _vp, _sz]),
    "wsc_profile_begin": (_i, [_vp]),
    "wsc_profile_end": (_i, [_vp, _i, _vp, _vp, _vp, ctypes.POINTER(_i)]),
    "wsc_profile_class_name": (ctypes.c_char_p, [_i]),
    "wsc_timer_begin": (_i, [_vp]),
    "wsc_timer_end": (_i, [_vp, ctypes.POINTER(_f)]),
    "wsc_net_create": (_i, [_vp, _i, ctypes.POINTER(TensorDesc), _i, _i, _i, ctypes.POINTER(_vp)]),
    "wsc_net_destroy": (None, [_vp]),
    "wsc_net_cam_size": (_i, [_vp, _i, ctypes.POINTER(_i)]),
    "wsc_net_feat_channels": (_i, [_vp, ctypes.POINTER(_i)]),
    "wsc_net_forward_cam": (_i, [_vp, _vp, _vp, _i, _i, _vp, _vp]),
    "wsc_net_forward_gradcam": (_i, [_vp, _vp, _vp, _i, _i, _i, _vp, _vp]),
    "wsc_net_forward_features": (_i, [_vp, _vp, _vp, _i, _i, _vp]),
    "wsc_net_cam_size_hw": (_i, [_vp, _i, _i, ctypes.POINTER(_i), ctypes.POINTER(_i)]),
    "wsc_net_forward_cam_hw": (_i, [_vp, _vp, _vp, _i, _i, _i, _vp, _vp]),
    "wsc_net_forward_edge": (_i, [_vp, _vp, _vp, _i, _i, _i, _i, _vp, _vp]),
    "wsc_rw_propagate": (_i, [_vp, _vp, _vp, _i, _i, _i, _vp, _vp, _vp, _i, _f, _i, _vp]),
    "wsc_rw_propagate_batch": (_i, [_vp, _i, _vp, _vp, _vp, _vp, _vp, _vp, _vp, _vp, _i, _f, _i, _vp]),
    "wsc_conv2d_nchw": (_i, [_vp, _vp, _i, _i, _i, _i, _vp, _i, _i, _i, _i, _i, _vp, _vp, _vp, _i, _i, _vp]),
    "wsc_cam_postprocess": (_i, [_vp, _vp, _i, _i, _i, _i, _vp, _vp, _vp, _vp, _vp, _vp, _vp]),
    "wsc_cam_eval_confusion": (_i, [_vp, _vp, _i, _vp, _vp, _vp, _vp, _f, _vp, _i, _i, _vp, _vp]),
    "wsc_unary_from_maps": (_i, [_vp, _vp, _i, _i, _i, _f, _vp]),
    "wsc_cam_unary": (_i, [_vp, _vp, _i, _i, _i, _i, _i, _i, _f, _vp]),
    "wsc_cam_unary_pm": (_i, [_vp, _vp, _i, _i, _i, _i, _i, _i, _f, _vp]),
    "wsc_cam_sum_scales": (_i, [_vp, _vp, _i, _i, ctypes.c_longlong, _vp]),
    "wsc_cam_eval_confusion_nn": (_i, [_vp, _vp, _i, _vp, _vp, _vp, _vp, _vp, _vp, _i, _i, _vp, _vp]),
    "wsc_label_confusion_nn": (_i, [_vp, _vp, _i, _vp, _vp, _vp, _vp, _i, _i, _vp, _vp]),
    "wsc_sem_seg_finish": (_i, [_vp, _vp, _i, _vp, _vp, _vp, _vp, _vp, _vp, _i, _f, _vp]),
    "wsc_bilinear_resize": (_i, [_vp, _vp, _i, _i, _i, _vp, _i, _i]),
    "wsc_msf_input_u8": (_i, [_vp, _vp, _i, _vp, _vp, _i, _vp, _vp, _i, _i, _vp]),
    "wsc_resize_u8": (_i, [_vp, _vp, _i, _vp, _vp, _i, _i, _vp]),
    "wsc_label_unary_from_cam": (_i, [_vp, _vp, _i, _i, _i, _f, _f, _vp, _vp]),
    "wsc_ir_label_combine": (_i, [_vp, _vp, _vp, _vp, _i, _i, _i, _vp]),
    "wsc_hsn_gradcam_post": (_i, [_vp, _vp, _i, _i, _i, _i, _i, _vp, _vp, _i, _i]),
    "wsc_hsn_voc_background": (_i, [_vp, _vp, _i, _i, _i, _vp, _i]),
    "wsc_hsn_class_mass": (_i, [_vp, _vp, _i, _i, _vp]),
    "wsc_hsn_background": (_i, [_vp, _vp, _i, _i, _i, _i, _i, _vp]),
    "wsc_cam_adp_modify": (_i, [_vp, _vp, _i, _i, _i, _i, _vp, _i, _vp, _i, _vp, _i, _vp, _i, _vp]),
    "wsc_hsn_cs_gradcam": (_i, [_vp, _vp, _i, _i, _i, _vp, _vp, _i, _i, _i, _vp, _i, _vp, _i, _vp, _vp, _vp]),
    "wsc_hsn_gather_unary": (_i, [_vp, _vp, _vp, _i, _i, _vp]),
    "wsc_crf_create": (_i, [_vp, _vp, _i, _i, _i, _f, _f, _f, ctypes.POINTER(_vp)]),
    "wsc_crf_destroy": (None, [_vp]),
    "wsc_crf_lattice_sizes": (_i, [_vp, _vp, _vp, _vp]),
    "wsc_crf_gaussian_on_chip": (_i, [_vp, _i]),
    "wsc_crf_inference": (_i, [_vp, _vp, _vp, _i, _f, _f, _i, _vp, _vp]),
    "wsc_crf_inference_pm": (_i, [_vp, _vp, _vp, _i, _f, _f, _i, _vp, _vp]),
    "wsc_crf_v_create": (_i, [_vp, _vp, _vp, _i, _f, _f, _f, ctypes.POINTER(_vp)]),
    "wsc_crf_v_destroy": (None, [_vp]),
    "wsc_crf_v_num_groups": (_i, [_vp]),
    "wsc_crf_v_inference": (_i, [_vp, _vp, _vp, _vp, _f, _f, _i, _vp, _vp]),
}


def header_symbols():
    with open(HEADER_PATH) as fh:
        text = fh.read()
    text = re.sub(r"/\*.*?\*/", "", text, flags=re.S)
    return sorted(set(re.findall(r"\b(wsc_[a-z0-9_]+)\s*\(", text)))


def load():
    global _lib
    if _lib is not None:
        return _lib
    if not os.path.exists(LIB_PATH):
        raise WscError(WSC_ERR_NO_DEVICE,
                       "libwsscam.so not built at %s -- run `python __graft_entry__.py` (there is no "
                       "CPU fallback for the product path)" % LIB_PATH)
    lib = ctypes.CDLL(LIB_PATH)
    for name, (res, args) in _SIGNATURES.items():
        fn = getattr(lib, name)
        fn.restype = res
        fn.argtypes = args
    _lib = lib
    return lib


def check_exports():
    lib = load()
    declared = header_symbols()
    missing = [s for s in declared if not hasattr(lib, s)]
    unbound = [s for s in declared if s not in _SIGNATURES]
    if missing or unbound:
        raise WscError(WSC_ERR_INVALID, "missing exports %s / unbound %s" % (missing, unbound))
    return declared


def check(status):
    if status != WSC_OK:
        raise WscError(status, load().wsc_last_error().decode("utf-8", "replace"))


def _ptr(x):
    if x is None:
        return None
    if isinstance(x, DeviceBuffer):
        return x.ptr
    if isinstance(x, np.ndarray):
        assert x.flags["C_CONTIGUOUS"]
        return x.ctypes.data
    if isinstance(x, int):
        return x
    if hasattr(x, "data_ptr"):
        return x.data_ptr()
    raise TypeError("cannot take a pointer of %r" % type(x))


class StackChain:

    SLOT = 7

    def __init__(self):
        self._lock = threading.Lock()
        self._last = None

    def run(self, ctx, enqueue):
        with self._lock:
            prev = self._last
            if prev is not None and prev is not ctx:
                ctx.wait_for_mark(prev, self.SLOT)
            try:
                return enqueue()
            finally:
                ctx.mark(self.SLOT)
                self._last = ctx


class Context:

    def __init__(self, device=0, stream=None):
        lib = load()
        h = _vp()
        check(lib.wsc_ctx_create(int(device), stream, ctypes.byref(h)))
        self.h = h
        self.device = device
        self._lib = lib
        self._options = {}

    def close(self):
        if getattr(self, "h", None):
            pool = self.__dict__.pop("_pool", None)
            if pool:
                for lst in pool.values():
                    for buf in lst:
                        self._lib.wsc_free(self.h, buf.ptr)
                        buf.ptr = None
            self._lib.wsc_ctx_destroy(self.h)
            self.h = None

    def __del__(self):
        try:
            self.close()
        except Exception:
            pass

    def sync(self):
        check(self._lib.wsc_sync(self.h))

    def range_status(self, clear=False):
        f = _i(0)
        check(self._lib.wsc_ctx_range_status(self.h, ctypes.byref(f), 1 if clear else 0))
        return int(f.value)

    def mark(self, slot):
        check(self._lib.wsc_ctx_mark(self.h, int(slot)))

    def wait_mark(self, slot):
        check(self._lib.wsc_ctx_wait_mark(self.h, int(slot)))

    def wait_for_mark(self, other, slot):
        check(self._lib.wsc_ctx_wait_for_mark(self.h, other.h, int(slot)))

    def wait_for(self, other):
        check(self._lib.wsc_ctx_wait(self.h, other.h))

    def device_info(self):
        buf = ctypes.create_string_buffer(128)
        n = _i()
        check(self._lib.wsc_device_info(self.h, buf, 128, ctypes.byref(n)))
        return buf.value.decode(), n.value

    def alloc(self, nbytes, pooled=False):
        nbytes = int(nbytes)
        if pooled:
            size = 1 << max(16, (max(nbytes, 1) - 1).bit_length())
            pool = self.__dict__.setdefault("_pool", {})
            lst = pool.get(size)
            if lst:
                buf = lst.pop()
                buf.nbytes = nbytes
                return buf
            buf = DeviceBuffer(self, size)
            buf.nbytes, buf._pool_size = nbytes, size
            return buf
        return DeviceBuffer(self, nbytes)

    def to_device(self, arr, pooled=False):
        arr = np.ascontiguousarray(arr)
        buf = self.alloc(arr.nbytes, pooled=pooled)
        check(self._lib.wsc_memcpy_h2d(self.h, buf.ptr, arr.ctypes.data, arr.nbytes))
        self.sync()
        return buf

    def to_host(self, buf, shape, dtype, offset_bytes=0):
        out = np.empty(shape, dtype=dtype)
        check(self._lib.wsc_memcpy_d2h(self.h, out.ctypes.data, _ptr(buf) + offset_bytes, out.nbytes))
        return out

    def host_alloc(self, nbytes):
        return PinnedBuffer(self, int(nbytes))

    def h2d_async(self, dst_dev, pinned, nbytes, dst_offset=0, src_offset=0):
        check(self._lib.wsc_memcpy_h2d_async(self.h, _ptr(dst_dev) + dst_offset, pinned.ptr + src_offset, int(nbytes)))

    def d2h_async(self, pinned, src_dev, nbytes, dst_offset=0, src_offset=0):
        check(self._lib.wsc_memcpy_d2h_async(self.h, pinned.ptr + dst_offset, _ptr(src_dev) + src_offset, int(nbytes)))

    def set_option(self, option, value):
        check(self._lib.wsc_ctx_set_option(self.h, int(option), int(value)))
        self._options[int(option)] = int(value)

    def get_option(self, option):
        return self._options.get(int(option), OPT_DEFAULTS[int(option)])

    def option(self, option, value):
        import contextlib

        @contextlib.contextmanager
        def _cm():
            before = self.get_option(option)
            self.set_option(option, value)
            try:
                yield self
            finally:
                self.set_option(option, before)

        return _cm()

    def profile_begin(self):
        check(self._lib.wsc_profile_begin(self.h))

    def profile_end(self):
        n = 16
        calls = np.zeros(n, np.int32)
        ms = np.zeros(n, np.float32)
        work = np.zeros(n, np.float64)
        k = _i()
        check(self._lib.wsc_profile_end(self.h, n, calls.ctypes.data, ms.ctypes.data, work.ctypes.data, ctypes.byref(k)))
        return {self._lib.wsc_profile_class_name(i).decode(): (int(calls[i]), float(ms[i]), float(work[i]))
                for i in range(k.value) if calls[i] > 0}

    def timer_begin(self):
        check(self._lib.wsc_timer_begin(self.h))

    def timer_end(self):
        ms = _f()
# ... 463 lines not shown
```

Measured before the change: 2653 images/s.

## Fuse bottleneck conv2 3x3 with conv3 1x1 and residual in one kernel

Adds a TAIL variant of the windowed 3x3 conv kernel. Its f16 hi/lo output tile stays in LDS, and the following 1x1 conv3 with BN, residual add and ReLU runs in the same block. This removes the global write and read of the conv2 intermediate and one kernel launch per bottleneck block. In exchange it needs more LDS per block, which may lower occupancy, and the conv3 part is serialized inside each block. It is on by default, and the buffer assignment for downsample blocks is changed so the pairing check can pass.

```diff
diff --git a/include/wsscam.h b/include/wsscam.h
--- a/include/wsscam.h
+++ b/include/wsscam.h
@@ -52,7 +52,8 @@
     WSC_OPT_CONV_WINDOW = 7,
     WSC_OPT_CAM_HEAD_STREAM = 8,
     WSC_OPT_CRF_MSG_IN_UPDATE = 9,
-    WSC_OPT_COUNT = 10
+    WSC_OPT_CONV_BLOCK_TAIL = 10,
+    WSC_OPT_COUNT = 11
 } wsc_option;
 
 typedef struct wsc_crf wsc_crf;
diff --git a/profiles/conv_layer_table.py b/profiles/conv_layer_table.py
--- a/profiles/conv_layer_table.py
+++ b/profiles/conv_layer_table.py
@@ -40,6 +40,14 @@
     return 2 if rounds >= 1 and 0 < rem and rem * 2 <= num_cus else 1
 
 
+def is_tail(kernel_name):
+    m = re.search(r"conv_igemm_kernel<([^>]*)>", kernel_name)
+    if not m:
+        return False
+    args = [a.strip() for a in m.group(1).split(",")]
+    return len(args) == 11 and args[-1] == "1"
+
+
 def main(db, N=64, S=321, planes=1):
     c = sqlite3.connect(db)
     tabs = [r[0] for r in c.execute("select name from sqlite_master where type='table'")]
@@ -55,8 +63,23 @@
     print("%-44s %8s %8s %9s %7s %6s" % ("layer", "us", "TFLOP/s", "act TB/s", "blocks", "LDS KB"))
     tot = 0.0
     pos = 0
-    for (name, ho, cin, cout, k) in layers:
+    li = 0
+    while li < len(layers):
+        name, ho, cin, cout, k = layers[li]
+        li += 1
         M = N * ho * ho
+        if pos < len(convs) and is_tail(convs[pos][0]):
+            _, _, cin3, cout3, _ = layers[li]
+            li += 1
+            rs = convs[pos:pos + 1]
+            pos += 1
+            us = (rs[0][2] - rs[0][1]) / 1000.0
+            tot += us
+            fl = 2.0 * M * cout * k * k * cin + 2.0 * M * cout3 * cin3
+            by = (2.0 * M * cin + 2.0 * 2 * M * cout3) * planes
+            print("%-44s %8.1f %8.0f %9.2f %7s %6s" % (name.split(" ")[0] + "+conv3 (tail)", us, fl / us / 1e6, by / us / 1e6,
+                                                        str(rs[0][3]), "%.0f" % (rs[0][4] / 1024.0)))
+            continue
         nd = n_dispatches(M, cin, cout, k, planes=planes)
         rs = convs[pos:pos + nd]
         pos += nd
diff --git a/wsss-analysis_amd/csrc/api.hip b/wsss-analysis_amd/csrc/api.hip
--- a/wsss-analysis_amd/csrc/api.hip
+++ b/wsss-analysis_amd/csrc/api.hip
@@ -124,7 +124,7 @@
 static const char *kClassNames[WSC_K_COUNT] = {
     "conv_igemm_kernel<256-row tiles,glds>", "conv_igemm_kernel<128x128,glds>", "conv_igemm_kernel<128x64,glds>", "conv_igemm_kernel<small-Cin> / stem_pool_kernel",
     "pool/layout/flip-add", "cam_tail+unary", "crf_build(all)", "gauss_msg_kernel", "combine4+blur_lds+blur4+blur3_tile",
-    "update_splat_kernel", "crf init/finish"};
+    "update_splat_kernel", "crf init/finish", "conv_igemm_kernel<bottleneck tail>"};
 
 int wsc_ctx_range_check(wsc_ctx *ctx) {
     const unsigned f = *(volatile unsigned *)ctx->range_host;
diff --git a/wsss-analysis_amd/csrc/common.h b/wsss-analysis_amd/csrc/common.h
--- a/wsss-analysis_amd/csrc/common.h
+++ b/wsss-analysis_amd/csrc/common.h
@@ -109,6 +109,7 @@
     WSC_K_BLUR,
     WSC_K_SLICE_UPDATE,
     WSC_K_CRF_MISC,
+    WSC_K_CONV_TAIL,
     WSC_K_COUNT
 };
 struct WscProfRecord {
@@ -134,7 +135,7 @@
     };
     PinSlot pin_ring[PIN_SLOTS];
     int pin_next = 0;
-    int opt[WSC_OPT_COUNT] = {1, 1, 1, 0, 0, -1, 1, 1, 1, 1};
+    int opt[WSC_OPT_COUNT] = {1, 1, 1, 0, 0, -1, 1, 1, 1, 1, 1};
     void *pinned = nullptr;
     size_t pinned_bytes = 0;
     void *zero_page = nullptr;
@@ -199,6 +200,7 @@
     int H2, W2, C2, stride2;
 };
 int conv_igemm_launch(wsc_ctx *ctx, const ConvLaunch &p);
+int conv_block_tail_launch(wsc_ctx *ctx, const ConvLaunch &c2, const ConvLaunch &c3);
 int launch_cam_head(wsc_ctx *ctx, const bf16_t *x, const bf16_t *x_lo, int M, int K, const bf16_t *w, int Kw, int CoutPad,
                     const float *s1, const float *b1, int C, int relu, float *y);
 
diff --git a/wsss-analysis_amd/csrc/conv_igemm.hip b/wsss-analysis_amd/csrc/conv_igemm.hip
--- a/wsss-analysis_amd/csrc/conv_igemm.hip
+++ b/wsss-analysis_amd/csrc/conv_igemm.hip
@@ -1,6 +1,7 @@
 #include "common.h"
 
 #include <cstdlib>
+#include <cstring>
 #include <type_traits>
 
 #ifdef WSC_AB_KNOBS
@@ -44,16 +45,175 @@
     int stem_rows;
     int kw_real;
     unsigned *range;
+    const bf16_t *w3, *res3, *res3_lo;
+    bf16_t *y3, *y3_lo;
+    const float *s3, *b3;
+    int Cout3, Kw3, relu3;
 };
 
 __device__ __forceinline__ int lds_off(int row, int slot) {
     return row * 128 + ((slot ^ ((row >> 1) & 7)) << 4);
 }
 
-template <int BM, int BN, int MODE, int SPLIT, int ET, bool GLDS, int STAGES, int WMT = 64, int FAST = 0, int WPT = 0>
+template <int CMID, int TA_OFF>
+__device__ __forceinline__ unsigned tail_conv3(const ConvKArgs &p, char *smem, int m0) {
+    constexpr int NK3 = CMID / 32;
+    constexpr int W3_BYTES = 128 * 128;
+    constexpr int CT_STRIDE = 128 + 4;
+    static_assert(NK3 * W3_BYTES <= TA_OFF && 64 * CT_STRIDE * 4 <= TA_OFF, "weight buffers and the fp32 group lie in front of the A tile");
+    typedef unsigned u32x4_t __attribute__((ext_vector_type(4)));
+    const int t = threadIdx.x, lane = t & 63;
+    const int wv = __builtin_amdgcn_readfirstlane(t >> 6);
+    const int wm = wv >> 1, wn = wv & 1;
+    const int l31 = lane & 31, kgrp = lane >> 5, slot = t & 7;
+    const int c8 = t & 15, r0 = t >> 4;
+    const unsigned lds0 = (unsigned)(uintptr_t)(__attribute__((address_space(3))) char *)smem;
+    const float sat_lo = p.relu3 ? 0.f : -65504.f;
+    float *ct = reinterpret_cast<float *>(smem);
+    unsigned ovf = 0u;
+    for (int n0 = 0; n0 < p.Cout3; n0 += 128) {
+        __syncthreads();
+#pragma unroll
+        for (int kt = 0; kt < NK3; ++kt)
+#pragma unroll
+            for (int i = 0; i < 4; ++i) {
+                const int r = wv * 32 + i * 8 + (lane >> 3);
+                const int ks = slot ^ ((r >> 1) & 7);
+                __builtin_amdgcn_global_load_lds((const __attribute__((address_space(1))) void *)(p.w3 + (long long)(n0 + r) * p.Kw3 + kt * 64 + ks * 8),
+                                                 (__attribute__((address_space(3))) void *)(smem + kt * W3_BYTES + wv * 4096 + i * 1024), 16, 0, 0);
+            }
+        __builtin_amdgcn_sched_barrier(0);
+        const int c = n0 + c8 * 8;
+        uint4 rres[8], rres_lo[8];
+#pragma unroll
+        for (int i = 0; i < 8; ++i) {
+            const int m = m0 + i * 16 + r0;
+            const int mc = m < p.m_end ? m : p.m_end - 1;
+            rres[i] = *reinterpret_cast<const uint4 *>(p.res3 + ((unsigned)mc * (unsigned)p.Cout3 + (unsigned)c));
+            rres_lo[i] = *reinterpret_cast<const uint4 *>(p.res3_lo + ((unsigned)mc * (unsigned)p.Cout3 + (unsigned)c));
+        }
+        __builtin_amdgcn_sched_barrier(0);
+        asm volatile("s_waitcnt vmcnt(16)" ::: "memory");
+        __builtin_amdgcn_s_barrier();
+        f32x16_t acc[2][2];
+#pragma unroll
+        for (int mi = 0; mi < 2; ++mi)
+#pragma unroll
+            for (int ni = 0; ni < 2; ++ni)
+#pragma unroll
+                for (int r = 0; r < 16; ++r) acc[mi][ni][r] = 0.f;
+        auto mfma = [&](const u32x4_t &a, const u32x4_t &b, f32x16_t &cc) {
+            cc = __builtin_amdgcn_mfma_f32_32x32x16_f16(__builtin_bit_cast(f16x8_t, a), __builtin_bit_cast(f16x8_t, b), cc, 0, 0, 0);
+        };
+#pragma unroll
+        for (int kt = 0; kt < NK3; ++kt) {
+            const unsigned sa = lds0 + TA_OFF + kt * (128 * 128), sb = lds0 + kt * W3_BYTES;
+#pragma unroll
+            for (int sl = 0; sl < 2; ++sl) {
+                u32x4_t fah[2], fal[2], fbh[2], fbl[2];
+#pragma unroll
+                for (int mi = 0; mi < 2; ++mi) {
+                    asm volatile("ds_read_b128 %0, %1" : "=v"(fah[mi]) : "v"(sa + lds_off(wm * 64 + mi * 32 + l31, sl * 2 + kgrp)) : "memory");
+                    asm volatile("ds_read_b128 %0, %1" : "=v"(fal[mi]) : "v"(sa + lds_off(wm * 64 + mi * 32 + l31, (2 + sl) * 2 + kgrp)) : "memory");
+                }
+#pragma unroll
+                for (int ni = 0; ni < 2; ++ni) {
+                    asm volatile("ds_read_b128 %0, %1" : "=v"(fbh[ni]) : "v"(sb + lds_off(wn * 64 + ni * 32 + l31, sl * 2 + kgrp)) : "memory");
+                    asm volatile("ds_read_b128 %0, %1" : "=v"(fbl[ni]) : "v"(sb + lds_off(wn * 64 + ni * 32 + l31, (2 + sl) * 2 + kgrp)) : "memory");
+                }
+                asm volatile("s_waitcnt lgkmcnt(0)" ::: "memory");
+                __builtin_amdgcn_sched_barrier(0);
+#pragma unroll
+                for (int mi = 0; mi < 2; ++mi)
+#pragma unroll
+                    for (int ni = 0; ni < 2; ++ni) mfma(fal[mi], fbh[ni], acc[mi][ni]);
+#pragma unroll
+                for (int mi = 0; mi < 2; ++mi)
+#pragma unroll
+                    for (int ni = 0; ni < 2; ++ni) mfma(fah[mi], fbl[ni], acc[mi][ni]);
+#pragma unroll
+                for (int mi = 0; mi < 2; ++mi)
+#pragma unroll
+                    for (int ni = 0; ni < 2; ++ni) mfma(fah[mi], fbh[ni], acc[mi][ni]);
+                __builtin_amdgcn_sched_barrier(0);
+            }
+        }
+        float s1[8], b1[8];
+        {
+            const f32x4_t sa = *reinterpret_cast<const f32x4_t *>(p.s3 + c), sb = *reinterpret_cast<const f32x4_t *>(p.s3 + c + 4);
+            const f32x4_t ba = *reinterpret_cast<const f32x4_t *>(p.b3 + c), bb = *reinterpret_cast<const f32x4_t *>(p.b3 + c + 4);
+#pragma unroll
+            for (int j = 0; j < 4; ++j) {
+                s1[j] = sa[j];
+                s1[4 + j] = sb[j];
+                b1[j] = ba[j];
+                b1[4 + j] = bb[j];
+            }
+        }
+#pragma unroll
+        for (int g = 0; g < 2; ++g) {
+            __syncthreads();
+            if (wm == g) {
+#pragma unroll
+                for (int mi = 0; mi < 2; ++mi)
+#pragma unroll
+                    for (int ni = 0; ni < 2; ++ni)
+#pragma unroll
+                        for (int r = 0; r < 16; ++r)
+                            ct[(mi * 32 + (r & 3) + 8 * (r >> 2) + 4 * kgrp) * CT_STRIDE + wn * 64 + ni * 32 + l31] = acc[mi][ni][r];
+            }
+            __syncthreads();
+#pragma unroll
+            for (int pp = 0; pp < 4; ++pp) {
+                const int ri = g * 4 + pp;
+                const int lr = pp * 16 + r0;
+                const int m = m0 + g * 64 + lr;
+                float v[8];
+                const f32x4_t q0 = *reinterpret_cast<const f32x4_t *>(ct + lr * CT_STRIDE + c8 * 8);
+                const f32x4_t q1 = *reinterpret_cast<const f32x4_t *>(ct + lr * CT_STRIDE + c8 * 8 + 4);
+#pragma unroll
+                for (int j = 0; j < 4; ++j) {
+                    v[j] = q0[j] * s1[j] + b1[j];
+                    v[4 + j] = q1[j] * s1[4 + j] + b1[4 + j];
+                }
+                const uint32_t rw[4] = {rres[ri].x, rres[ri].y, rres[ri].z, rres[ri].w};
+#pragma unroll
+                for (int j = 0; j < 4; ++j) {
+                    v[2 * j] += f16_to_f32((bf16_t)(rw[j] & 0xffffu));
+                    v[2 * j + 1] += f16_to_f32((bf16_t)(rw[j] >> 16));
+                }
+                const uint32_t lw_[4] = {rres_lo[ri].x, rres_lo[ri].y, rres_lo[ri].z, rres_lo[ri].w};
+#pragma unroll
+                for (int j = 0; j < 4; ++j) {
+                    v[2 * j] += f16_to_f32((bf16_t)(lw_[j] & 0xffffu));
+                    v[2 * j + 1] += f16_to_f32((bf16_t)(lw_[j] >> 16));
+                }
+                uint32_t hw[4], lw[4];
+#pragma unroll
+                for (int j = 0; j < 4; ++j) {
+                    const float c0 = __builtin_amdgcn_fmed3f(v[2 * j], sat_lo, 65504.f), c1 = __builtin_amdgcn_fmed3f(v[2 * j + 1], sat_lo, 65504.f);
+                    const _Float16 h0 = (_Float16)c0;
+                    const _Float16 h1 = (_Float16)c1;
+                    hw[j] = (uint32_t)__builtin_bit_cast(uint16_t, h0) | ((uint32_t)__builtin_bit_cast(uint16_t, h1) << 16);
+                    const _Float16 l0 = (_Float16)(c0 - (float)h0), l1 = (_Float16)(c1 - (float)h1);
+                    lw[j] = (uint32_t)__builtin_bit_cast(uint16_t, l0) | ((uint32_t)__builtin_bit_cast(uint16_t, l1) << 16);
+                }
+                if (m < p.m_end) {
+                    ovf |= half2_at_ceiling(hw[0]) | half2_at_ceiling(hw[1]) | half2_at_ceiling(hw[2]) | half2_at_ceiling(hw[3]);
+                    *reinterpret_cast<uint4 *>(p.y3 + ((unsigned)m * (unsigned)p.Cout3 + (unsigned)c)) = make_uint4(hw[0], hw[1], hw[2], hw[3]);
+                    *reinterpret_cast<uint4 *>(p.y3_lo + ((unsigned)m * (unsigned)p.Cout3 + (unsigned)c)) = make_uint4(lw[0], lw[1], lw[2], lw[3]);
+                }
+            }
+        }
+    }
+    return ovf;
+}
+
+template <int BM, int BN, int MODE, int SPLIT, int ET, bool GLDS, int STAGES, int WMT = 64, int FAST = 0, int WPT = 0, int TAIL = 0>
 __global__ __launch_bounds__(BM * 2, (STAGES == 1 && FAST != 0) ? 4 : 2) void conv_igemm_kernel(ConvKArgs p) {
     constexpr bool FEPI = (FAST & 1) != 0, PW = (FAST & 2) != 0;
     constexpr bool WIN = WPT > 0;
+    static_assert(!TAIL || (WIN && BN == 64), "bottleneck tail: a window layer with 64 output channels");
     static_assert(!WIN || (SPLIT == 2 && BM == 128 && WMT == 64 && STAGES == 2 && FAST == 1), "LDS window: single-staged split, 128-row tile");
     static_assert(FAST == 0 || (SPLIT != 1 && ET == 1 && ((GLDS && MODE == 0) || FAST == 1)),
                   "FAST paths: f16, one plane or the single-staged split; the pointwise prologue belongs to the LDS-DMA layers");
@@ -766,6 +926,7 @@
     }
 
     float *ct = reinterpret_cast<float *>(smem);
+    constexpr int TA_OFF = BM * CT_STRIDE * 4;
     constexpr int NHALF = STAGES == 1 ? BM / 64 : (WMT == 128 ? BM / 128 : 1);
     constexpr int GR = BM / NHALF;
     constexpr int PPH = NPASS / NHALF;
@@ -842,6 +1003,13 @@
                         const _Float16 l0 = (_Float16)(c0 - (float)h0), l1 = (_Float16)(c1 - (float)h1);
                         lw[j] = (uint32_t)__builtin_bit_cast(uint16_t, l0) | ((uint32_t)__builtin_bit_cast(uint16_t, l1) << 16);
                     }
+                }
+                if constexpr (TAIL != 0) {
+                    char *ta = smem + TA_OFF + (c >> 5) * (BM * 128);
+                    *reinterpret_cast<uint4 *>(ta + lds_off(lrow_e, (c >> 3) & 3)) = make_uint4(hw[0], hw[1], hw[2], hw[3]);
+                    *reinterpret_cast<uint4 *>(ta + lds_off(lrow_e, 4 + ((c >> 3) & 3))) = make_uint4(lw[0], lw[1], lw[2], lw[3]);
+                    if (m < p.m_end) ovf |= half2_at_ceiling(hw[0]) | half2_at_ceiling(hw[1]) | half2_at_ceiling(hw[2]) | half2_at_ceiling(hw[3]);
+                    continue;
                 }
                 if (m < p.m_end) {
                     ovf |= half2_at_ceiling(hw[0]) | half2_at_ceiling(hw[1]) | half2_at_ceiling(hw[2]) | half2_at_ceiling(hw[3]);
@@ -918,19 +1086,26 @@
             }
         }
     }
+    if constexpr (TAIL != 0) {
+        const unsigned ovf3 = tail_conv3<BN, TA_OFF>(p, smem, m0);
+        if (ovf & 0x80008000u) *p.range = (unsigned)p.Cout;
+        if (ovf3 & 0x80008000u) *p.range = (unsigned)p.Cout3;
+        return;
+    }
     if (ET && (ovf & 0x80008000u)) *p.range = (unsigned)p.Cout;
 }
 
-template <int BM, int BN, int MODE, int SPLIT, int ET, int STAGES, int WMT = 64, int FAST = 0, int WPT = 0>
+template <int BM, int BN, int MODE, int SPLIT, int ET, int STAGES, int WMT = 64, int FAST = 0, int WPT = 0, int TAIL = 0>
 int launch_stages(wsc_ctx *ctx, const ConvKArgs &a) {
     constexpr bool GLDS = MODE == 0;
     constexpr int A_BYTES = BM * BK * 2, B_BYTES = BN * BK * 2;
     constexpr int PIPE = WPT > 0 ? WPT * 4096 + STAGES * B_BYTES : STAGES * (A_BYTES + B_BYTES);
     constexpr int EPI = (STAGES == 1 ? 64 : (WMT == 128 ? 128 : BM)) * (BN + 4) * 4;
-    constexpr int LDS = PIPE > EPI ? PIPE : EPI;
+    constexpr int EPI_T = TAIL ? EPI + (BN / 32) * BM * 128 : EPI;
+    constexpr int LDS = PIPE > EPI_T ? PIPE : EPI_T;
     static_assert(LDS <= 160 * 1024, "LDS budget of a CU");
     static bool attr_set[64] = {};
-    auto kern = conv_igemm_kernel<BM, BN, MODE, SPLIT, ET, GLDS, STAGES, WMT, FAST, WPT>;
+    auto kern = conv_igemm_kernel<BM, BN, MODE, SPLIT, ET, GLDS, STAGES, WMT, FAST, WPT, TAIL>;
     const int dev = ctx->device >= 0 && ctx->device < 64 ? ctx->device : 0;
     int lds_req = LDS;
 #ifdef WSC_AB_KNOBS
@@ -943,8 +1118,9 @@
         attr_set[dev] = true;
     }
     const double flops = 2.0 * (a.m_end - a.m_base) * a.Cout *
-                         ((MODE == 0 && !a.stem_rows) ? (double)a.kh * a.kw * a.Cin : (double)a.kh * (a.stem_rows ? a.kw_real : a.kw) * 3);
-    WscKernelTimer timer(ctx, (MODE != 0 || a.stem_rows) ? WSC_K_CONV_SMALLCIN : (BM == 256 ? WSC_K_CONV256 : (BN == 128 ? WSC_K_CONV128 : WSC_K_CONV64)), flops);
+                         ((MODE == 0 && !a.stem_rows) ? (double)a.kh * a.kw * a.Cin : (double)a.kh * (a.stem_rows ? a.kw_real : a.kw) * 3) +
+                         (TAIL ? 2.0 * (a.m_end - a.m_base) * a.Cout3 * a.Cout : 0.0);
+    WscKernelTimer timer(ctx, TAIL ? WSC_K_CONV_TAIL : (MODE != 0 || a.stem_rows) ? WSC_K_CONV_SMALLCIN : (BM == 256 ? WSC_K_CONV256 : (BN == 128 ? WSC_K_CONV128 : WSC_K_CONV64)), flops);
     hipLaunchKernelGGL(kern, dim3(a.nblocks), dim3(BM * 2), lds_req, ctx->stream, a);
     WSC_HIP(hipGetLastError());
     return WSC_OK;
@@ -1018,10 +1194,8 @@
     return launch_variant<256, 256, 0, false, 0>(ctx, a);
 }
 
-}
-
-int conv_igemm_launch(wsc_ctx *ctx, const ConvLaunch &p) {
-    ConvKArgs a;
+int conv_args(wsc_ctx *ctx, const ConvLaunch &p, ConvKArgs &a, int *small_cin_eff_out) {
+    memset(&a, 0, sizeof(a));
     a.x = p.x; a.x_lo = p.x_lo; a.w = p.w;
     a.s1 = p.s1; a.b1 = p.b1; a.s2 = p.s2; a.b2 = p.b2;
     a.res = p.res; a.res_lo = p.res_lo;
@@ -1104,6 +1278,31 @@
         a.fast = 1;
         if (small_cin_eff == 0 && p.kh == 1 && p.kw == 1 && p.pad == 0 && p.stride == 1) a.fast = 3;
     }
+    *small_cin_eff_out = small_cin_eff;
+    return WSC_OK;
+}
+
+int window_wpt(wsc_ctx *ctx, const ConvLaunch &p, ConvKArgs &a) {
+    const bool single_staged = p.split == 2 && (p.small_cin == 0 || p.small_cin == 3);
+    if (single_staged && a.fast == 1 && p.kh == 3 && p.kw == 3 && p.stride == 1 && p.pad == 1 && p.x2 == nullptr &&
+        p.Ho == p.H && p.Wo == p.W && ctx->opt[WSC_OPT_CONV_WINDOW] != 0) {
+        const long long need = 127 + 2ll * p.W + 3 + 1;
+        const long long npix = (long long)p.N * p.H * p.W;
+        if (need <= 320 && npix < (1ll << 30) && a.lo_delta >= 0 && npix * p.Cin + a.lo_delta < (1ll << 33) && (a.lo_delta & 7) == 0) {
+            a.win_npix = (int)npix;
+            return need <= 256 ? 8 : 10;
+        }
+    }
+    return 0;
+}
+
+}
+
+int conv_igemm_launch(wsc_ctx *ctx, const ConvLaunch &p) {
+    ConvKArgs a;
+    int small_cin_eff = 0;
+    WSC_TRY(conv_args(ctx, p, a, &small_cin_eff));
+    const int BN = p.CoutPad % 128 == 0 ? 128 : 64;
     if (a.M == 0) return WSC_OK;
 #ifdef WSC_AB_KNOBS
     static const int force = [] { const char *e = getenv("WSC_CONV_TILE"); return e ? atoi(e) : 0; }();
@@ -1147,17 +1346,41 @@
     }
     const int BMsel = big ? 256 : 128;
     a.nblocks = ((a.M + BMsel - 1) / BMsel) * a.ntiles_n;
-    if (!big && single_staged && a.fast == 1 && p.kh == 3 && p.kw == 3 && p.stride == 1 && p.pad == 1 && p.x2 == nullptr &&
-        p.Ho == p.H && p.Wo == p.W && ctx->opt[WSC_OPT_CONV_WINDOW] != 0) {
-        const long long need = 127 + 2ll * p.W + 3 + 1;
-        const long long npix = (long long)p.N * p.H * p.W;
-        if (need <= 320 && npix < (1ll << 30) && a.lo_delta >= 0 && npix * p.Cin + a.lo_delta < (1ll << 33) && (a.lo_delta & 7) == 0) {
-            a.win_npix = (int)npix;
-            if (BN == 128) return need <= 256 ? launch_window<8>(ctx, a) : launch_window<10>(ctx, a);
-            return need <= 256 ? launch_window<8, 64>(ctx, a) : launch_window<10, 64>(ctx, a);
+    if (!big) {
+        const int wpt = window_wpt(ctx, p, a);
+        if (wpt != 0) {
+            if (BN == 128) return wpt == 8 ? launch_window<8>(ctx, a) : launch_window<10>(ctx, a);
+            return wpt == 8 ? launch_window<8, 64>(ctx, a) : launch_window<10, 64>(ctx, a);
         }
     }
     if (big) return launch_big(ctx, a, p.split, p.fmt);
     if (BN == 128) return launch_bn<128>(ctx, a, small_cin_eff, p.split, p.fmt);
     return launch_bn<64>(ctx, a, small_cin_eff, p.split, p.fmt);
 }
+
+int conv_block_tail_launch(wsc_ctx *ctx, const ConvLaunch &c2, const ConvLaunch &c3) {
+    if (ctx->opt[WSC_OPT_CONV_BLOCK_TAIL] == 0) return 1;
+    const bool pair = c2.split == 2 && c3.split == 2 && c2.fmt && c3.fmt && !c2.generic && !c3.generic && c2.small_cin == 0 &&
+                      c3.small_cin == 0 && c2.Cout == 64 && c2.CoutPad == 64 && c2.s2 == nullptr && c2.res == nullptr &&
+                      c2.y_f32 == nullptr && c2.ldy == 0 && c3.kh == 1 && c3.kw == 1 && c3.stride == 1 && c3.pad == 0 &&
+                      c3.x2 == nullptr && c3.N == c2.N && c3.H == c2.Ho && c3.W == c2.Wo && c3.Cin == c2.Cout && c3.x == c2.y &&
+                      c3.x_lo == c2.y_lo && c3.Cout == 4 * c2.Cout && c3.CoutPad == c3.Cout && c3.s2 == nullptr &&
+                      c3.res != nullptr && c3.res_lo != nullptr && c3.y != nullptr && c3.y_lo != nullptr && c3.y_f32 == nullptr &&
+                      (c3.ldy == 0 || c3.ldy == c3.Cout) && (long long)c3.N * c3.H * c3.W * c3.Cout < (1ll << 31);
+    if (!pair) return 1;
+    ConvKArgs a, b;
+    int sce = 0;
+    WSC_TRY(conv_args(ctx, c2, a, &sce));
+    WSC_TRY(conv_args(ctx, c3, b, &sce));
+    if (a.fast != 1 || b.fast != 3) return 1;
+    const int wpt = window_wpt(ctx, c2, a);
+    if (wpt == 0) return 1;
+    if (a.M == 0) return WSC_OK;
+    a.nblocks = (a.M + 127) / 128;
+    a.w3 = c3.w; a.s3 = c3.s1; a.b3 = c3.b1;
+    a.res3 = c3.res; a.res3_lo = c3.res_lo;
+    a.y3 = c3.y; a.y3_lo = c3.y_lo;
+    a.Cout3 = c3.Cout; a.Kw3 = b.Kw; a.relu3 = c3.relu;
+    if (wpt == 8) return launch_stages<128, 64, 0, 2, 1, 2, 64, 1, 8, 1>(ctx, a);
+    return launch_stages<128, 64, 0, 2, 1, 2, 64, 1, 10, 1>(ctx, a);
+}
diff --git a/wsss-analysis_amd/csrc/net.hip b/wsss-analysis_amd/csrc/net.hip
--- a/wsss-analysis_amd/csrc/net.hip
+++ b/wsss-analysis_amd/csrc/net.hip
@@ -288,13 +288,14 @@
                 continue;
             }
             WSC_TRY(resnet_conv(net, d, pre + ".conv2", pre + ".bn2", s, 1, 1, 0, f[0], f[1], -1));
-            int res = cur;
+            int res = cur, out = f[2];
             if (has(d, pre + ".downsample.0.weight")) {
                 WSC_TRY(resnet_conv(net, d, pre + ".downsample.0", pre + ".downsample.1", s, 0, 0, 0, cur, f[2], -1));
                 res = f[2];
+                out = f[0];
             }
-            WSC_TRY(resnet_conv(net, d, pre + ".conv3", pre + ".bn3", 1, 0, 1, 0, f[1], f[0], res));
-            cur = f[0];
+            WSC_TRY(resnet_conv(net, d, pre + ".conv3", pre + ".bn3", 1, 0, 1, 0, f[1], out, res));
+            cur = out;
         }
         net->taps.push_back((int)net->ops.size() - 1);
     }
@@ -647,41 +648,67 @@
     if (in_pad > 0) WSC_TRY(launch_nchw_to_nhwc4_pad(ctx, x_dev, N, S, SW, in_h, in_w, in_pad, xin, xin_lo, net->fmt));
     else WSC_TRY(launch_nchw_to_nhwc4(ctx, x_dev, N, S, SW, xin, xin_lo, net->fmt));
     int bh[4] = {0, 0, 0, 0}, bw[4] = {0, 0, 0, 0}, bc[4] = {0, 0, 0, 0};
+    auto conv_launch = [&](size_t j, int H, int W) {
+        const Op &op = net->ops[j];
+        const ConvW &c = net->convs[op.conv];
+        ConvLaunch L;
+        memset(&L, 0, sizeof(L));
+        L.x = op.in < 0 ? xin : buf[op.in]; L.x_lo = op.in < 0 ? xin_lo : buf_lo[op.in]; L.w = c.w;
+        L.s1 = c.s1; L.b1 = c.b1; L.s2 = c.s2; L.b2 = c.b2;
+        L.res = op.res >= 0 ? buf[op.res] : nullptr;
+        L.res_lo = op.res >= 0 ? buf_lo[op.res] : nullptr;
+        L.y = buf[op.out]; L.y_lo = buf_lo[op.out]; L.y_f32 = nullptr;
+        if (op.in2 >= 0) {
+            L.x2 = buf[op.in2]; L.x2_lo = buf_lo[op.in2];
+            L.H2 = bh[op.in2]; L.W2 = bw[op.in2]; L.C2 = bc[op.in2]; L.stride2 = op.ps;
+        }
+        L.ldy = op.pitch;
+        if (op.pitch) {
+            L.y += op.coff;
+            if (L.y_lo) L.y_lo += op.coff;
+        }
+        L.N = N; L.H = H; L.W = W; L.Cin = c.Cin; L.Ho = pl.H[j]; L.Wo = pl.W[j];
+        L.Cout = c.Cout; L.CoutPad = c.CoutPad;
+        L.kh = c.kh; L.kw = c.kw; L.stride = c.stride; L.pad = c.pad; L.relu = c.relu;
+        L.small_cin = c.small_cin; L.split = net->split; L.fmt = net->fmt;
+        if (c.small_cin == 3 && op.in < 0) {
+            L.H = in_h; L.W = in_w; L.pad = 0;
+        }
+        return L;
+    };
+    auto tail_pair = [&](size_t j) {
+        if (j + 1 >= net->ops.size()) return false;
+        const Op &a = net->ops[j], &b = net->ops[j + 1];
+        if (a.type != OP_CONV || b.type != OP_CONV || a.in < 0 || a.pitch != 0 || b.pitch != 0 || b.in != a.out || b.in2 >= 0 ||
+            b.res == a.out || b.out == a.in || b.out == a.out)
+            return false;
+        for (int tp : net->taps)
+            if (tp == (int)j) return false;
+        for (size_t k = j + 2; k < net->ops.size(); ++k) {
+            const Op &o = net->ops[k];
+            if (o.in == a.out || o.in2 == a.out || o.res == a.out) return false;
+            if (o.out == a.out) break;
+        }
+        return true;
+    };
     for (size_t i = 0; i < net->ops.size(); ++i) {
         const Op &op = net->ops[i];
         const int H = op.in < 0 ? S : bh[op.in], W = op.in < 0 ? SW : bw[op.in], C = op.in < 0 ? 4 : bc[op.in];
         const bf16_t *src = op.in < 0 ? xin : buf[op.in];
         const bf16_t *src_lo = op.in < 0 ? xin_lo : buf_lo[op.in];
         if (fused_stem && i == 0) continue;
+        bool pair_done = false;
         if (fused_stem && i == 1) {
             const ConvW &c0 = net->convs[net->ops[0].conv];
             WSC_TRY(launch_stem_pool(ctx, xin, xin_lo, N, S, SW, c0.w, c0.kh * 64, c0.s1, c0.b1, c0.relu, buf[op.out], buf_lo[op.out]));
+        } else if (op.type == OP_CONV && tail_pair(i)) {
+            const ConvLaunch L2 = conv_launch(i, H, W), L3 = conv_launch(i + 1, pl.H[i], pl.W[i]);
+            const int st = conv_block_tail_launch(ctx, L2, L3);
+            if (st < 0) return st;
+            pair_done = st == WSC_OK;
+            if (!pair_done) WSC_TRY(conv_igemm_launch(ctx, L2));
         } else if (op.type == OP_CONV) {
-            const ConvW &c = net->convs[op.conv];
-            ConvLaunch L;
-            memset(&L, 0, sizeof(L));
-            L.x = src; L.x_lo = src_lo; L.w = c.w;
-            L.s1 = c.s1; L.b1 = c.b1; L.s2 = c.s2; L.b2 = c.b2;
-            L.res = op.res >= 0 ? buf[op.res] : nullptr;
-            L.res_lo = op.res >= 0 ? buf_lo[op.res] : nullptr;
-            L.y = buf[op.out]; L.y_lo = buf_lo[op.out]; L.y_f32 = nullptr;
-            if (op.in2 >= 0) {
-                L.x2 = buf[op.in2]; L.x2_lo = buf_lo[op.in2];
-                L.H2 = bh[op.in2]; L.W2 = bw[op.in2]; L.C2 = bc[op.in2]; L.stride2 = op.ps;
-            }
-            L.ldy = op.pitch;
-            if (op.pitch) {
-                L.y += op.coff;
-                if (L.y_lo) L.y_lo += op.coff;
-            }
-            L.N = N; L.H = H; L.W = W; L.Cin = c.Cin; L.Ho = pl.H[i]; L.Wo = pl.W[i];
-            L.Cout = c.Cout; L.CoutPad = c.CoutPad;
-            L.kh = c.kh; L.kw = c.kw; L.stride = c.stride; L.pad = c.pad; L.relu = c.relu;
-            L.small_cin = c.small_cin; L.split = net->split; L.fmt = net->fmt;
-            if (c.small_cin == 3 && op.in < 0) {
-                L.H = in_h; L.W = in_w; L.pad = 0;
-            }
-            WSC_TRY(conv_igemm_launch(ctx, L));
+            WSC_TRY(conv_igemm_launch(ctx, conv_launch(i, H, W)));
         } else if (op.type == OP_GATHER) {
             WSC_TRY(launch_gather_strided(ctx, src, src_lo, N, H, W, C, op.ps, pl.H[i], pl.W[i], buf[op.out] + op.coff,
                                           buf_lo[op.out] ? buf_lo[op.out] + op.coff : nullptr, op.pitch));
@@ -689,18 +716,22 @@
             WSC_TRY(launch_maxpool(ctx, src, src_lo, N, H, W, C, op.pk, op.ps, op.pp, pl.H[i], pl.W[i], buf[op.out],
                                    buf_lo[op.out], net->fmt));
         }
-        bh[op.out] = pl.H[i]; bw[op.out] = pl.W[i]; bc[op.out] = pl.C[i];
-        if (copy_taps)
-            for (size_t k = 0; k < net->taps.size(); ++k)
-                if (net->taps[k] == (int)i) {
-                    char *dst = (char *)*extra;
-                    for (size_t j = 0; j < k; ++j) dst += tap_plane_bytes(net, pl, N, (int)j) * planes;
-                    const size_t nb = (size_t)N * pl.H[i] * pl.W[i] * pl.C[i] * sizeof(bf16_t);
-                    WSC_HIP(hipMemcpyAsync(dst, buf[op.out], nb, hipMemcpyDeviceToDevice, ctx->stream));
-                    if (net->split)
-                        WSC_HIP(hipMemcpyAsync(dst + tap_plane_bytes(net, pl, N, (int)k), buf_lo[op.out], nb,
-                                               hipMemcpyDeviceToDevice, ctx->stream));
-                }
+        for (size_t d = i; d <= i + (pair_done ? 1 : 0); ++d) {
+            const Op &od = net->ops[d];
+            bh[od.out] = pl.H[d]; bw[od.out] = pl.W[d]; bc[od.out] = pl.C[d];
+            if (copy_taps)
+                for (size_t k = 0; k < net->taps.size(); ++k)
+                    if (net->taps[k] == (int)d) {
+                        char *dst = (char *)*extra;
+                        for (size_t j = 0; j < k; ++j) dst += tap_plane_bytes(net, pl, N, (int)j) * planes;
+                        const size_t nb = (size_t)N * pl.H[d] * pl.W[d] * pl.C[d] * sizeof(bf16_t);
+                        WSC_HIP(hipMemcpyAsync(dst, buf[od.out], nb, hipMemcpyDeviceToDevice, ctx->stream));
+                        if (net->split)
+                            WSC_HIP(hipMemcpyAsync(dst + tap_plane_bytes(net, pl, N, (int)k), buf_lo[od.out], nb,
+                                                   hipMemcpyDeviceToDevice, ctx->stream));
+                    }
+        }
+        if (pair_done) ++i;
     }
     *feat = buf[net->final_buf];
     *feat_lo = buf_lo[net->final_buf];
diff --git a/wsss-analysis_amd/wsscam/_lib.py b/wsss-analysis_amd/wsscam/_lib.py
--- a/wsss-analysis_amd/wsscam/_lib.py
+++ b/wsss-analysis_amd/wsscam/_lib.py
@@ -32,10 +32,10 @@
 PREC_F16 = 2
 PREC_F16X3 = 3
 OPT_CRF_GAUSS_ON_CHIP, OPT_CRF_FUSED_BLUR, OPT_CRF_BLUR_ON_CHIP, OPT_CRF_RANK_BALLOT, OPT_CRF_EMBED_FULL, OPT_RW_TILED, \
-    OPT_STEM_POOL_FUSED, OPT_CONV_WINDOW, OPT_CAM_HEAD_STREAM, OPT_CRF_MSG_IN_UPDATE = range(10)
+    OPT_STEM_POOL_FUSED, OPT_CONV_WINDOW, OPT_CAM_HEAD_STREAM, OPT_CRF_MSG_IN_UPDATE, OPT_CONV_BLOCK_TAIL = range(11)
 OPT_DEFAULTS = {OPT_CRF_GAUSS_ON_CHIP: 1, OPT_CRF_FUSED_BLUR: 1, OPT_CRF_BLUR_ON_CHIP: 1, OPT_CRF_RANK_BALLOT: 0,
                 OPT_CRF_EMBED_FULL: 0, OPT_RW_TILED: -1, OPT_STEM_POOL_FUSED: 1, OPT_CONV_WINDOW: 1, OPT_CAM_HEAD_STREAM: 1,
-                OPT_CRF_MSG_IN_UPDATE: 1}
+                OPT_CRF_MSG_IN_UPDATE: 1, OPT_CONV_BLOCK_TAIL: 1}
 CONV_GENERIC = 0x100
 
 
```

New measurement: 2664 images/s, median of 6. About the same (+0.4%).
